# mprib/caliscope

Measured on AMD Instinct MI355X. Metric: observations/sec per LM iteration, higher is better.
Workload: dtype f64; 1 GPU; cfg4: 64 cams / 2000000 obs in total (200000 points / 2000000 obs on rank 0), extrinsics-only BA, linear loss; n_obs_total=2000000, params_per_camera=6, tolerances=ftol=xtol=gtol=1e-8 (reference defaults), sums=FP64 atomics (default)

## Files before the change

caliscope_amd/_lib.py:

```python

from __future__ import annotations

import ctypes as C
import os
from pathlib import Path

from caliscope_amd.exceptions import BackendError

LIB_NAME = "libcaliscope_ba.so"
LIB_PATH = Path(__file__).resolve().parent / LIB_NAME

c_double_p = C.POINTER(C.c_double)
c_int32_p = C.POINTER(C.c_int32)
c_int64_p = C.POINTER(C.c_int64)


class ProblemDesc(C.Structure):
    _fields_ = [
        ("n_cams", C.c_int32),
        ("n_points", C.c_int32),
        ("n_obs", C.c_int64),
        ("cam_n_params", c_int32_p),
        ("cam_model", c_int32_p),
        ("cam_const", c_double_p),
        ("obs_cam", c_int32_p),
        ("obs_pt", c_int32_p),
        ("obs_uv", c_double_p),
        ("loss", C.c_int32),
        ("f_scale", C.c_double),
    ]


class Options(C.Structure):
    _fields_ = [("device_id", C.c_int32), ("max_blocks", C.c_int32), ("deterministic", C.c_int32), ("evaluation_only", C.c_int32)]


class Linearization(C.Structure):
    _fields_ = [(n, C.c_double) for n in ("g_norm_inf", "gh_sq", "jg_sq", "x_scaled_norm", "x_norm", "cost")]


class NewtonInfo(C.Structure):
    _fields_ = [("ok", C.c_int32), ("reserved", C.c_int32), ("p_sq", C.c_double), ("gh_dot_p", C.c_double), ("w_sq", C.c_double)]


class TrialInfo(C.Structure):
    _fields_ = [("cost", C.c_double), ("step_norm", C.c_double), ("finite", C.c_int32), ("reserved", C.c_int32)]


class StepInfo(C.Structure):
    _fields_ = [
        ("lin", Linearization), ("newton", NewtonInfo), ("trial", TrialInfo), ("lam", C.c_double), ("radius", C.c_double),
        ("p_s", C.c_double * 2), ("predicted", C.c_double), ("alpha", C.c_double), ("beta", C.c_double),
        ("need_host", C.c_int32), ("reserved", C.c_int32),
    ]


class Info(C.Structure):
    _fields_ = [
        ("n_cams", C.c_int32), ("n_points", C.c_int32), ("n_cam_params", C.c_int32), ("n_params", C.c_int32),
        ("n_obs", C.c_int64), ("n_chunks", C.c_int32), ("grid_blocks", C.c_int32), ("plan_state", C.c_int32),
        ("max_obs_per_point", C.c_int32), ("device_bytes", C.c_int64),
        ("schur_groups", C.c_int32), ("schur_tiles", C.c_int32), ("schur_grid", C.c_int32), ("n_heavy_points", C.c_int32),
        ("schur_stream_len", C.c_int64), ("schur_pairs", C.c_int64), ("plan_error", C.c_int32), ("build_camg", C.c_int32),
    ]


class SolveOptions(C.Structure):
    _fields_ = [
        ("ftol", C.c_double), ("xtol", C.c_double), ("gtol", C.c_double), ("max_nfev", C.c_int64),
        ("lb", c_double_p), ("ub", c_double_p), ("verbose", C.c_int32), ("max_damping_retries", C.c_int32),
    ]


class Result(C.Structure):
    _fields_ = [
        ("status", C.c_int32), ("reserved", C.c_int32), ("nfev", C.c_int64), ("njev", C.c_int64), ("n_iterations", C.c_int64),
        ("cost", C.c_double), ("optimality", C.c_double), ("t_total_s", C.c_double),
        ("t_rejected_s", C.c_double), ("n_rejected_timed", C.c_int64),
    ]


class TriangulateDesc(C.Structure):
    _fields_ = [
        ("n_cams", C.c_int32),
        ("cam_model", c_int32_p),
        ("cam_intr", c_double_p),
        ("cam_P", c_double_p),
        ("n_points", C.c_int64),
        ("pt_start", c_int64_p),
        ("obs_cam", c_int32_p),
        ("obs_xy", c_double_p),
        ("float32_io", C.c_int32),
    ]


class ScaleDesc(C.Structure):
    _fields_ = [
        ("n_world", C.c_int64),
        ("world_xyz", c_double_p),
        ("n_groups", C.c_int64),
        ("group_start", c_int64_p),
        ("ent_world", c_int64_p),
        ("ent_obj", c_double_p),
    ]


SIGNATURES = {
    "cba_create": (C.c_int, [C.POINTER(ProblemDesc), C.POINTER(Options), C.POINTER(C.c_void_p)]),
    "cba_destroy": (None, [C.c_void_p]),
    "cba_comm_unique_id": (C.c_int, [C.c_char_p]),
    "cba_comm_init": (C.c_int, [C.c_void_p, C.c_char_p, C.c_int32, C.c_int32]),
    "cba_comm_abort": (C.c_int, [C.c_void_p]),
    "cba_group_create": (C.c_int, [C.c_int32, C.POINTER(C.c_void_p)]),
    "cba_group_join": (C.c_int, [C.c_void_p, C.c_void_p, C.c_int32]),
    "cba_group_abort": (None, [C.c_void_p]),
    "cba_group_destroy": (None, [C.c_void_p]),
    "cba_set_constraints": (C.c_int, [C.c_void_p, C.c_int32, c_int32_p, c_int32_p, c_double_p, c_double_p]),
    "cba_begin": (C.c_int, [C.c_void_p, c_double_p, c_double_p]),
    "cba_restart": (C.c_int, [C.c_void_p, c_double_p]),
    "cba_begin_deferred": (C.c_int, [C.c_void_p, c_double_p]),
    "cba_linearize": (C.c_int, [C.c_void_p, C.POINTER(Linearization)]),
    "cba_newton_step": (C.c_int, [C.c_void_p, C.c_double, C.POINTER(NewtonInfo)]),
    "cba_subspace_gram": (C.c_int, [C.c_void_p, C.c_double, C.c_double, C.c_double, C.c_double, c_double_p]),
    "cba_trial": (C.c_int, [C.c_void_p, C.c_double, C.c_double, C.POINTER(TrialInfo)]),
    "cba_accept": (C.c_int, [C.c_void_p]),
    "cba_linearize_build": (C.c_int, [C.c_void_p]),
    "cba_step": (C.c_int, [C.c_void_p, C.c_double, C.POINTER(StepInfo)]),
    "cba_refresh_step_scalars": (C.c_int, [C.c_void_p, C.POINTER(NewtonInfo)]),
    "cba_step_supported": (C.c_int, [C.c_void_p]),
    "cba_set_camera_scaling": (C.c_int, [C.c_void_p, c_double_p, c_double_p, C.POINTER(Linearization)]),
    "cba_set_bounds": (C.c_int, [C.c_void_p, c_double_p, c_double_p]),
    "cba_step_camera_state": (C.c_int, [C.c_void_p, c_double_p, c_double_p, c_double_p, c_double_p]),
    "cba_subspace_gram_ex": (C.c_int, [C.c_void_p, C.c_double, C.c_double, c_double_p, C.c_double, C.c_double, c_double_p, c_double_p]),
    "cba_trial_ex": (C.c_int, [C.c_void_p, C.c_double, C.c_double, c_double_p, C.POINTER(TrialInfo)]),
    "cba_solve": (C.c_int, [C.c_void_p, c_double_p, C.POINTER(SolveOptions), c_double_p, C.POINTER(Result)]),
    "cba_get_vector": (C.c_int, [C.c_void_p, C.c_int32, c_double_p]),
    "cba_get_camera_params": (C.c_int, [C.c_void_p, C.c_int32, c_double_p]),
    "cba_get_camera_state": (C.c_int, [C.c_void_p, c_double_p, c_double_p, c_double_p]),
    "cba_residuals": (C.c_int, [C.c_void_p, c_double_p, c_double_p, c_double_p]),
    "cba_normal_blocks": (C.c_int, [C.c_void_p, c_double_p, c_double_p, c_double_p, c_double_p, c_double_p]),
    "cba_reduced_system": (C.c_int, [C.c_void_p, c_double_p, c_double_p]),
    "cba_set_loss": (C.c_int, [C.c_void_p, C.c_int32, C.c_double]),
    "cba_plan_wait": (C.c_int, [C.c_void_p]),
    "cba_get_info": (C.c_int, [C.c_void_p, C.POINTER(Info)]),
    "cba_timer_count": (C.c_int, []),
    "cba_timer_name": (C.c_char_p, [C.c_int32]),
    "cba_get_timers": (C.c_int, [C.c_void_p, c_double_p, c_int64_p]),
    "cba_reset_timers": (C.c_int, [C.c_void_p]),
    "cba_enable_timers": (C.c_int, [C.c_void_p, C.c_int32]),
    "cba_host_plan": (C.c_int64, [C.c_int32, C.c_int64, c_int32_p, c_int32_p, C.c_int32, C.c_int32, c_int64_p, c_int64_p, c_int64_p]),
    "cba_triangulate": (C.c_int, [C.POINTER(TriangulateDesc), C.c_int32, c_double_p, c_double_p]),
    "cba_scale_errors": (C.c_int, [C.POINTER(ScaleDesc), C.c_int32, c_double_p]),
    "cba_trim": (C.c_int64, []),
    "cba_last_error": (C.c_char_p, []),
    "cba_set_error": (C.c_int, [C.c_int32, C.c_char_p]),
    "cba_version": (C.c_int, []),
    "cba_device_count": (C.c_int, []),
}

_lib = None


def load() -> C.CDLL:
    global _lib
    if _lib is not None:
        return _lib
    path = Path(os.environ.get("CALISCOPE_BA_LIB", LIB_PATH))
    if not path.exists():
        raise BackendError(
            f"{path} not found: build the MI355X engine first (python -c 'import __graft_entry__ as g; g.build()' "
            f"or python -m caliscope_amd.build).  There is no CPU fallback."
        )
    try:
        lib = C.CDLL(str(path))
    except OSError as exc:
        raise BackendError(f"could not load {path}: {exc}") from exc
    for name, (res, args) in SIGNATURES.items():
        try:
            fn = getattr(lib, name)
        except AttributeError as exc:
            raise BackendError(f"{path} does not export {name} (stale build?)") from exc
        fn.restype = res
        fn.argtypes = args
    _lib = lib
    return lib


def last_error(lib) -> str:
    msg = lib.cba_last_error()
    return msg.decode("utf-8", "replace") if msg else ""


def check(lib, rc: int, what: str) -> None:
    if rc != 0:
        raise BackendError(f"{what} failed (code {rc}): {last_error(lib)}")
```

caliscope_amd/csrc/cba_kernels.h:

```cpp
#pragma once
#include <hip/hip_runtime.h>

#include "ba_math.h"
#include "trf_math.h"
#include "wg_binding.h"

namespace cba {

constexpr int BLOCK = 256;
constexpr int CHUNK = 256;
constexpr int WAVE = 64;

struct VecLayout {
  int ncp;
  int ncp_pad;
  int P;
  int Ppad;
  __host__ __device__ long total() const { return (long)ncp_pad + 3L * Ppad; }
};

__device__ __forceinline__ double wave_sum(double v) {
#pragma unroll
  for (int o = WAVE / 2; o > 0; o >>= 1) v += __shfl_down(v, o, WAVE);
  return v;
// ... 51 lines not shown
  return r;
}

__device__ __forceinline__ void lds_add(double* addr, double v) { unsafeAtomicAdd(addr, v); }

constexpr int CAMTAB_LIVE = 36;
constexpr int CAMTAB_LDS = CAMTAB_LIVE + 1;
struct ObsRec { double u, v; int cam, pt; };
__device__ __forceinline__ ObsRec load_obs(const double* __restrict__ obs_u, const double* __restrict__ obs_v,
                                           const int* __restrict__ obs_cam, const int* __restrict__ obs_pt, int i) {
  ObsRec r;
  r.u = obs_u[i]; r.v = obs_v[i]; r.cam = obs_cam[i]; r.pt = obs_pt[i];
  return r;
}

__device__ __forceinline__ void stage_camtab(double* sh_tab, const double* tab, int n_cams) {
  for (int i = threadIdx.x; i < n_cams * CAMTAB_LIVE; i += BLOCK)
    sh_tab[(i / CAMTAB_LIVE) * CAMTAB_LDS + (i % CAMTAB_LIVE)] = tab[(i / CAMTAB_LIVE) * CAMTAB_DOUBLES + (i % CAMTAB_LIVE)];
}
__device__ __forceinline__ const CamTab& cam_at(const double* sh_tab, int cam) {
  return *reinterpret_cast<const CamTab*>(sh_tab + cam * CAMTAB_LDS);
}
template <bool CAMG>
__device__ __forceinline__ const CamTab& cam_of(const double* sh_tab, const double* __restrict__ tab, int cam) {
  if constexpr (CAMG) return *reinterpret_cast<const CamTab*>(tab + (long)cam * CAMTAB_DOUBLES);
  else return cam_at(sh_tab, cam);
}

__global__ void k_cam_prep(const double* __restrict__ xvec, const double* __restrict__ cam_const,
                           const int* __restrict__ cam_model, const int* __restrict__ cam_np,
                           const int* __restrict__ cam_off, int n_cams, double* __restrict__ tab) {
  const int c = blockIdx.x * blockDim.x + threadIdx.x;
  if (c >= n_cams) return;
  double xc[MAX_NC];
  const int np = cam_np[c];
  for (int i = 0; i < MAX_NC; ++i) xc[i] = (i < np) ? xvec[cam_off[c] + i] : 0.0;
  CamTab t;
  cam_prepare(xc, cam_const + c * CAM_CONST_STRIDE, cam_model[c], np, &t, cam_off[c]);
  const double* src = reinterpret_cast<const double*>(&t);
  for (int i = 0; i < CAMTAB_DOUBLES; ++i) tab[c * CAMTAB_DOUBLES + i] = src[i];
}

__global__ void __launch_bounds__(BLOCK)
k_begin(const double* __restrict__ x0, double* __restrict__ x, double* __restrict__ x_new, double* __restrict__ sinv, double* __restrict__ cam_diag,
        int* __restrict__ flags, long total, int ncp_pad, const double* __restrict__ cam_const, const int* __restrict__ cam_model,
        const int* __restrict__ cam_np, const int* __restrict__ cam_off, int n_cams, double* __restrict__ tab) {
  const long t0 = (long)blockIdx.x * blockDim.x + threadIdx.x;
  for (long i = t0; i < total; i += (long)gridDim.x * blockDim.x) {
    const double v = x0[i];
    x[i] = v;
    if (x_new) x_new[i] = v;
    sinv[i] = 1.0;
    if (i < ncp_pad) cam_diag[i] = 0.0;
    if (i < 4) flags[i] = 0;
  }
  if (t0 < n_cams) {
    const int c = (int)t0;
    double xc[MAX_NC];
    const int np = cam_np[c];
    for (int i = 0; i < MAX_NC; ++i) xc[i] = (i < np) ? x0[cam_off[c] + i] : 0.0;
    CamTab t;
    cam_prepare(xc, cam_const + c * CAM_CONST_STRIDE, cam_model[c], np, &t, cam_off[c]);
    const double* src = reinterpret_cast<const double*>(&t);
    for (int i = 0; i < CAMTAB_DOUBLES; ++i) tab[c * CAMTAB_DOUBLES + i] = src[i];
  }
}

template <bool WRITE_R, bool CAMG = false>
__global__ void __launch_bounds__(BLOCK)
k_cost(const double* __restrict__ obs_u, const double* __restrict__ obs_v, const int* __restrict__ obs_cam,
       const int* __restrict__ obs_pt, long n_obs, const double* __restrict__ xvec, VecLayout lay,
       const double* __restrict__ tab, int n_cams, int loss, double f_scale, double* __restrict__ partial,
       int* __restrict__ flags, double* __restrict__ r_out, const int* __restrict__ order) {
  extern __shared__ __attribute__((aligned(16))) double sh[];
  double* sh_tab = sh;
  double* sh_red = sh + (CAMG ? 0 : n_cams * CAMTAB_LDS);
  if (!CAMG) stage_camtab(sh_tab, tab, n_cams);
  __syncthreads();
  const double* px = xvec + lay.ncp_pad;
  double acc = 0.0;
  bool bad = false;
  struct Rec { int cam, pt; double u, v; long o; };
  const long stride = (long)gridDim.x * BLOCK, last = n_obs - 1;
  auto load_rec = [&](long i) {
    Rec r; const long k = min(i, last);
    r.cam = obs_cam[k]; r.pt = obs_pt[k]; r.u = obs_u[k]; r.v = obs_v[k]; r.o = WRITE_R ? (long)order[k] : 0;
    return r;
  };
  long i = (long)blockIdx.x * BLOCK + threadIdx.x;
  Rec rc = load_rec(i), rn = load_rec(i + stride);
  double X = px[rc.pt], Y = px[lay.Ppad + rc.pt], Z = px[2 * lay.Ppad + rc.pt];
  for (; i < n_obs; i += stride) {
    asm volatile("s_waitcnt vmcnt(0)" ::: "memory");
    asm volatile("" : "+v"(rc.cam), "+v"(rc.pt), "+v"(rc.u), "+v"(rc.v), "+v"(rc.o));
    asm volatile("" : "+v"(rn.cam), "+v"(rn.pt), "+v"(rn.u), "+v"(rn.v), "+v"(rn.o));
    asm volatile("" : "+v"(X), "+v"(Y), "+v"(Z));
    const double Xn = px[rn.pt], Yn = px[lay.Ppad + rn.pt], Zn = px[2 * lay.Ppad + rn.pt];
    const Rec rnn = load_rec(i + 2 * stride);
    __builtin_amdgcn_sched_barrier(0);
    double e[2];
    project_residual(cam_of<CAMG>(sh_tab, tab, rc.cam), X, Y, Z, rc.u, rc.v, e);
    if (!(isfinite(e[0]) && isfinite(e[1]))) bad = true;
    acc += robust_cost_one(loss, f_scale, e[0]) + robust_cost_one(loss, f_scale, e[1]);
    if (WRITE_R) {
      r_out[2 * rc.o] = e[0];
      r_out[2 * rc.o + 1] = e[1];
    }
    rc = rn; rn = rnn; X = Xn; Y = Yn; Z = Zn;
  }
  asm volatile("s_waitcnt vmcnt(0)" ::: "memory");
  if (bad) flags[0] = 1;
  const double tot = block_sum(acc, sh_red);
  if (threadIdx.x == 0) partial[blockIdx.x] = tot;
}

constexpr int REDUCE_RY = 16;
__device__ __forceinline__ void reduce_rows_block(const double* __restrict__ partial, int nrow, int width, double* __restrict__ out,
                                                  double* __restrict__ grad_out, const int* __restrict__ cam_off, const int* __restrict__ cam_np,
                                                  int stride, int tri) {
  __shared__ double sh[REDUCE_RY][64];
  const int j = blockIdx.x * 64 + threadIdx.x;
  double acc[8] = {0.0, 0.0, 0.0, 0.0, 0.0, 0.0, 0.0, 0.0};
  if (j < width) {
    int b = threadIdx.y;
    for (; b + 7 * REDUCE_RY < nrow; b += 8 * REDUCE_RY) {
#pragma unroll
      for (int q = 0; q < 8; ++q) acc[q] += partial[(long)(b + q * REDUCE_RY) * width + j];
    }
    for (; b < nrow; b += REDUCE_RY) acc[0] += partial[(long)b * width + j];
  }
  sh[threadIdx.y][threadIdx.x] = ((acc[0] + acc[1]) + (acc[2] + acc[3])) + ((acc[4] + acc[5]) + (acc[6] + acc[7]));
  __syncthreads();
  if (threadIdx.y == 0 && j < width) {
    double tot = 0.0;
#pragma unroll
    for (int y = 0; y < REDUCE_RY; ++y) tot += sh[y][threadIdx.x];
    out[j] = tot;
    if (grad_out) {
      const int c = j / stride, r = j % stride - tri;
      if (r >= 0 && r < cam_np[c]) grad_out[cam_off[c] + r] = tot;
    }
  }
}
__global__ void __launch_bounds__(64 * REDUCE_RY)
k_reduce_rows(const double* __restrict__ partial, int nrow, int width, double* __restrict__ out,
              double* __restrict__ grad_out = nullptr, const int* __restrict__ cam_off = nullptr, const int* __restrict__ cam_np = nullptr,
              int stride = 1, int tri = 0) {
  reduce_rows_block(partial, nrow, width, out, grad_out, cam_off, cam_np, stride, tri);
}
struct PubArgs {
  double* scal; int n_scal; int* flags; double* host_scal; int* host_flags; unsigned long long seq;
  const double* part_a; int rows_a, slot_a; const double* part_b; int rows_b, slot_b;
  const double* cam_src[4]; double* cam_dst; int ncp;
};
__global__ void __launch_bounds__(64 * REDUCE_RY)
k_reduce_rows_pub(const double* __restrict__ partial, int nrow, int width, double* __restrict__ out, double* __restrict__ grad_out,
                  const int* __restrict__ cam_off, const int* __restrict__ cam_np, int stride, int tri, PubArgs pub) {
  CBA_STAMP(ST_REDUCE_PUB);
  if (blockIdx.x + 1 < gridDim.x) { reduce_rows_block(partial, nrow, width, out, grad_out, cam_off, cam_np, stride, tri); return; }
  __shared__ double sh_w[2][REDUCE_RY];
  const int t = threadIdx.y * 64 + threadIdx.x;
  const double own = (t < pub.n_scal) ? pub.scal[t] : 0.0;
  double a = 0.0, b = 0.0;
  for (int r = t; r < pub.rows_a; r += 64 * REDUCE_RY) a += pub.part_a[r];
  for (int r = t; r < pub.rows_b; r += 64 * REDUCE_RY) b += pub.part_b[r];
  a = wave_sum(a); b = wave_sum(b);
  if (threadIdx.x == 0) { sh_w[0][threadIdx.y] = a; sh_w[1][threadIdx.y] = b; }
  __syncthreads();
  __shared__ double sh_tot[2];
  if (t == 0) {
    double ta = 0.0, tb = 0.0;
    for (int i = 0; i < REDUCE_RY; ++i) { ta += sh_w[0][i]; tb += sh_w[1][i]; }
    pub.scal[pub.slot_a] = ta; pub.scal[pub.slot_b] = tb;
    sh_tot[0] = ta; sh_tot[1] = tb;
  }
  __syncthreads();
  if (t < pub.n_scal) pub.host_scal[t] = (t == pub.slot_a) ? sh_tot[0] : (t == pub.slot_b) ? sh_tot[1] : own;
  if (t < 4) { pub.host_flags[t] = pub.flags[t]; pub.flags[t] = 0; }
  if (pub.cam_dst)
    for (int e = t; e < 4 * pub.ncp; e += 64 * REDUCE_RY) pub.cam_dst[e] = pub.cam_src[e / pub.ncp][e % pub.ncp];
  __threadfence_system();
  __syncthreads();
  if (t == 0) reinterpret_cast<volatile unsigned long long*>(pub.host_scal)[63] = pub.seq;
}
__global__ void k_xpack(const double* __restrict__ scal, const int* __restrict__ flags, unsigned long long mask, int with_max,
                        int rank, int world, double* __restrict__ xbuf) {
  if (threadIdx.x != 0 || blockIdx.x != 0) return;
  int n = 0;
  for (int s2 = 0; s2 < 32; ++s2)
    if ((mask >> s2) & 1ull) xbuf[n++] = scal[s2];
  for (int k = 0; k < 4; ++k) xbuf[n++] = flags[k] ? 1.0 : 0.0;
  if (with_max)
    for (int r = 0; r < world; ++r) xbuf[n++] = (r == rank) ? scal[4] : 0.0;
}
__global__ void k_xunpack(const double* __restrict__ xbuf, unsigned long long mask, int with_max, int world,
                          double* __restrict__ scal, int* __restrict__ flags) {
  if (threadIdx.x != 0 || blockIdx.x != 0) return;
  int n = 0;
  for (int s2 = 0; s2 < 32; ++s2)
    if ((mask >> s2) & 1ull) scal[s2] = xbuf[n++];
  for (int k = 0; k < 4; ++k) flags[k] = xbuf[n++] > 0.5 ? 1 : 0;
  if (with_max) {
    double m = 0.0;
    for (int r = 0; r < world; ++r) m = fmax(m, xbuf[n++]);
    scal[4] = m;
  }
}

template <bool MAX>
__global__ void __launch_bounds__(BLOCK)
k_reduce_narrow(const double* __restrict__ partial, int nrow, int width, double* __restrict__ out) {
  __shared__ double sh_red[BLOCK / WAVE];
  for (int j = 0; j < width; ++j) {
    double s = 0.0;
    for (int b = threadIdx.x; b < nrow; b += BLOCK) {
      const double v = partial[(long)b * width + j];
      s = MAX ? fmax(s, v) : s + v;
    }
    const double r = MAX ? block_max(s, sh_red) : block_sum(s, sh_red);
    if (threadIdx.x == 0) out[j] = r;
  }
}

template <int NC>
__device__ __forceinline__ double obs_linearize(const CamTab& c_lds, double X, double Y, double Z, double u, double v,
                                                int loss, double f_scale, double* e, double (*A)[MAX_NC],
                                                double (*B)[3]) {
  const CamTab c = c_lds;
  __builtin_amdgcn_sched_barrier(0);
  project_full(c, X, Y, Z, u, v, e, A, B);
  double rho = 0.0;
#pragma unroll
  for (int r = 0; r < 2; ++r) {
    double rs, er;
    rho += robust_one(loss, f_scale, e[r], &rs, &er);
    e[r] = er;
    if (loss != LOSS_LINEAR) {
#pragma unroll
      for (int k = 0; k < NC; ++k) A[r][k] *= rs;
      B[r][0] *= rs; B[r][1] *= rs; B[r][2] *= rs;
    }
  }
  return rho;
}

__device__ __forceinline__ double obs_factors(const CamTab& c_lds, double X, double Y, double Z, double u, double v, int loss, double f_scale, double* e,
                                              double (*G)[3], double* Yr, double (*Aint)[3], double (*B)[3]) {
  CamTab c;
  {
    const double* src = reinterpret_cast<const double*>(&c_lds);
    double* dst = reinterpret_cast<double*>(&c);
#pragma unroll
    for (int i = 0; i < 12; ++i) dst[i] = src[i];
#pragma unroll
    for (int i = 21; i < 35; ++i) dst[i] = src[i];
  }
  __builtin_amdgcn_sched_barrier(0);
  project_factors(c, X, Y, Z, u, v, e, G, Yr, Aint, B);
  double rho = 0.0;
#pragma unroll
  for (int r = 0; r < 2; ++r) {
    double rs, er;
    rho += robust_one(loss, f_scale, e[r], &rs, &er);
    e[r] = er;
    if (loss != LOSS_LINEAR) {
#pragma unroll
      for (int k = 0; k < 3; ++k) { G[r][k] *= rs; B[r][k] *= rs; Aint[r][k] *= rs; }
    }
  }
  return rho;
}

template <int NC> struct UPack {
  static constexpr int TRI = NC * (NC + 1) / 2;
  static constexpr int STRIDE = TRI + NC;
  __host__ __device__ static constexpr int idx(int r, int c) { return r * NC - r * (r - 1) / 2 + (c - r); }
};

constexpr int DET_ROUND = 9;
constexpr int DET_LD = CHUNK + 1;
struct DetPlan {
  const unsigned char* perm;
  const unsigned short* cstart;
};
template <int M>
__device__ __forceinline__ void det_round(const double* val, double* sh_cv, const int* sh_perm, const int* sh_cs, int n_cams, double* acc) {
#pragma unroll
  for (int q = 0; q < DET_ROUND; ++q) sh_cv[q * DET_LD + threadIdx.x] = val[q];
  __syncthreads();
#pragma unroll
  for (int m = 0; m < M; ++m) {
    const int task = (int)threadIdx.x + BLOCK * m;
    if (task < n_cams * DET_ROUND) {
      const int c = task / DET_ROUND, q = task % DET_ROUND;
      double s = 0.0;
      for (int j = sh_cs[c]; j < sh_cs[c + 1]; ++j) s += sh_cv[q * DET_LD + sh_perm[j]];
      acc[m] += s;
    }
  }
  __syncthreads();
}

template <int NC>
__device__ __forceinline__ double cam_block_value(int v, const double (*A)[MAX_NC], const double* e, int np) {
  using UP = UPack<NC>;
  int idx = 0;
#pragma unroll
  for (int r = 0; r < NC; ++r)
#pragma unroll
    for (int c = r; c < NC; ++c, ++idx)
      if (idx == v) return (r < np && c < np) ? A[0][r] * A[0][c] + A[1][r] * A[1][c] : 0.0;
#pragma unroll
  for (int r = 0; r < NC; ++r)
    if (UP::TRI + r == v) return (r < np) ? A[0][r] * e[0] + A[1][r] * e[1] : 0.0;
  return 0.0;
}

template <int NC, int DETM = 0, bool CAMG = false>
__global__ void __launch_bounds__(BLOCK)
k_build(const double* __restrict__ obs_u, const double* __restrict__ obs_v, const int* __restrict__ obs_cam,
        const int* __restrict__ obs_pt, const int* __restrict__ pt_start, const int* __restrict__ chunk_start,
        const int* __restrict__ chunk_pts, int n_chunks, const double* __restrict__ xvec, VecLayout lay, const double* __restrict__ tab, int n_cams,
        int loss, double f_scale, double* __restrict__ Vblk, double* __restrict__ gvec,
        double* __restrict__ partialU, double* __restrict__ partial_cost, int* __restrict__ flags, const double* __restrict__ skip,
        DetPlan det = DetPlan{nullptr, nullptr}) {
  using UP = UPack<NC>;
  constexpr bool DET = DETM > 0;
  if (skip && *skip != 0.0) return;
  extern __shared__ __attribute__((aligned(16))) double sh[];
  double* sh_tab = sh;
// ... 266 lines not shown
      lds_add(&sh_vg[4 * PM + pl], B[0][1] * B[0][2] + B[1][1] * B[1][2]);
      lds_add(&sh_vg[5 * PM + pl], B[0][2] * B[0][2] + B[1][2] * B[1][2]);
      lds_add(&sh_vg[6 * PM + pl], B[0][0] * e[0] + B[1][0] * e[1]);
      lds_add(&sh_vg[7 * PM + pl], B[0][1] * e[0] + B[1][1] * e[1]);
      lds_add(&sh_vg[8 * PM + pl], B[0][2] * e[0] + B[1][2] * e[1]);
    }
    flush();
    __syncthreads();
    for (int i = threadIdx.x; i < npts; i += BLOCK) {
#pragma unroll
      for (int q = 0; q < 6; ++q) Vblk[(long)q * lay.Ppad + p0 + i] = sh_vg[q * PM + i];
      gp[p0 + i] = sh_vg[6 * PM + i];
      gp[lay.Ppad + p0 + i] = sh_vg[7 * PM + i];
      gp[2 * lay.Ppad + p0 + i] = sh_vg[8 * PM + i];
    }
  }
  __syncthreads();
  if (!UGLOB) {
    for (int c = threadIdx.x; c < n_cams; c += BLOCK) {
      const double* Jl = tab + (long)c * CAMTAB_DOUBLES + 12;
      double* Uc = sh_U + (long)c * UP::STRIDE;
      double M[3][3], T[3][3];
#pragma unroll
      for (int r = 0; r < 3; ++r)
#pragma unroll
        for (int q = 0; q < 3; ++q) M[r][q] = Uc[UP::idx(min(r, q), max(r, q))];
#pragma unroll
      for (int r = 0; r < 3; ++r)
#pragma unroll
        for (int q = 0; q < 3; ++q) T[r][q] = Jl[r] * M[0][q] + Jl[3 + r] * M[1][q] + Jl[6 + r] * M[2][q];
#pragma unroll
      for (int r = 0; r < 3; ++r)
#pragma unroll
        for (int q = r; q < 3; ++q) Uc[UP::idx(r, q)] = T[r][0] * Jl[q] + T[r][1] * Jl[3 + q] + T[r][2] * Jl[6 + q];
#pragma unroll
      for (int q = 3; q <= NC; ++q) {
        double* v0 = (q < NC) ? &Uc[UP::idx(0, q)] : &Uc[UP::TRI + 0];
        double* v1 = (q < NC) ? &Uc[UP::idx(1, q)] : &Uc[UP::TRI + 1];
        double* v2 = (q < NC) ? &Uc[UP::idx(2, q)] : &Uc[UP::TRI + 2];
        const double a0 = *v0, a1 = *v1, a2 = *v2;
        *v0 = Jl[0] * a0 + Jl[3] * a1 + Jl[6] * a2;
        *v1 = Jl[1] * a0 + Jl[4] * a1 + Jl[7] * a2;
        *v2 = Jl[2] * a0 + Jl[5] * a1 + Jl[8] * a2;
      }
    }
    __syncthreads();
    double* dst = partialU + (long)blockIdx.x * n_cams * UP::STRIDE;
    for (int i = threadIdx.x; i < n_cams * UP::STRIDE; i += BLOCK) dst[i] = sh_U[i];
  }
  const double tot = block_sum(cost, sh_red);
  if (threadIdx.x == 0) partial_cost[blockIdx.x] = tot;
  if (TRIAL) {
    const double st = block_sum(step_sq, sh_red);
    if (threadIdx.x == 0) trial.step_partial[blockIdx.x] = st;
  }
  if (bad) flags[0] = 1;
}

__global__ void __launch_bounds__(256)
k_gather_uv(const double* __restrict__ uv_raw, const int* __restrict__ order, long n, double* __restrict__ u, double* __restrict__ v) {
  for (long i = (long)blockIdx.x * 256 + threadIdx.x; i < n; i += (long)gridDim.x * 256) {
    const double2 w = reinterpret_cast<const double2*>(uv_raw)[order[i]];
    u[i] = w.x; v[i] = w.y;
  }
}
__global__ void __launch_bounds__(256)
k_cs_fill(const int* __restrict__ perm, const int* __restrict__ sc_obs, const int* __restrict__ sc_p0, const double* __restrict__ u,
          const double* __restrict__ v, const int* __restrict__ cam, const int* __restrict__ pt, double* __restrict__ cu, double* __restrict__ cv,
          int* __restrict__ ccam, int* __restrict__ cptl) {
  const int s = blockIdx.x, o0 = sc_obs[s], o1 = sc_obs[s + 1], p0 = sc_p0[s];
  for (int j = o0 + threadIdx.x; j < o1; j += 256) {
    const int i = perm[j];
    cu[j] = u[i]; cv[j] = v[i]; ccam[j] = cam[i]; cptl[j] = pt[i] - p0;
  }
}

template <int NC>
__global__ void k_unpack_camera_grad(const double* __restrict__ Upacked, const int* __restrict__ cam_off,
                                     const int* __restrict__ cam_np, int n_cams, double* __restrict__ gvec) {
  using UP = UPack<NC>;
  const int t = blockIdx.x * blockDim.x + threadIdx.x;
  const int c = t / NC, r = t % NC;
  if (c >= n_cams || r >= cam_np[c]) return;
  gvec[cam_off[c] + r] = Upacked[c * UP::STRIDE + UP::TRI + r];
}

template <int NC>
__global__ void k_scale_update(const double* __restrict__ Upacked, const double* __restrict__ Vblk,
                               const int* __restrict__ param_cam, const int* __restrict__ param_loc, VecLayout lay,
                               int first, double* __restrict__ sinv, const double* __restrict__ cdiag) {
  using UP = UPack<NC>;
  const long total = lay.total();
  for (long i = (long)blockIdx.x * blockDim.x + threadIdx.x; i < total; i += (long)gridDim.x * blockDim.x) {
    double v;
    if (i < lay.ncp_pad) {
      if (i >= lay.ncp) continue;
      const int r = param_loc[i];
      v = Upacked[param_cam[i] * UP::STRIDE + UP::idx(r, r)];
    } else {
      const long k = (i - lay.ncp_pad) / lay.Ppad, p = (i - lay.ncp_pad) % lay.Ppad;
      if (p >= lay.P) continue;
      const int q = (k == 0) ? 0 : (k == 1 ? 3 : 5);
      v = Vblk[(long)q * lay.Ppad + p];
      if (cdiag) v += cdiag[k * lay.Ppad + p];
    }
    v = sqrt(v);
    if (first) { if (v == 0.0) v = 1.0; }
    else v = fmax(v, sinv[i]);
    sinv[i] = v;
  }
}

__global__ void k_cam_rescale(const double* __restrict__ state, const double* __restrict__ mult, const double* __restrict__ diag_h,
                              int ncp, double* __restrict__ sinv, double* __restrict__ cam_diag) {
  const int i = blockIdx.x * blockDim.x + threadIdx.x;
  if (i >= ncp) return;
  const double si = state[i] * mult[i];
  sinv[i] = si;
  cam_diag[i] = diag_h[i] * si * si;
}

__global__ void __launch_bounds__(BLOCK)
k_lin_scalars(const double* __restrict__ x, const double* __restrict__ g, const double* __restrict__ sinv,
              long total, int cam_end, int count_cams, int max_from, double* __restrict__ v1, double* __restrict__ partial,
              double* __restrict__ partial_max) {
  __shared__ double sh_red[BLOCK / WAVE];
  double s0 = 0, s1 = 0, s2 = 0, m = 0;
  for (long i = (long)blockIdx.x * BLOCK + threadIdx.x; i < total; i += (long)gridDim.x * BLOCK) {
    const double gi = g[i], si = sinv[i], xi = x[i];
    const double gh = gi / si;
    v1[i] = gh / si;
    if (i >= max_from) m = fmax(m, fabs(gi));
    if (i < cam_end && !count_cams) continue;
    s0 += gh * gh;
    s1 += (xi * si) * (xi * si);
    s2 += xi * xi;
  }
  double r;
  r = block_sum(s0, sh_red); if (threadIdx.x == 0) partial[blockIdx.x * 4 + 0] = r;
  r = block_sum(s1, sh_red); if (threadIdx.x == 0) partial[blockIdx.x * 4 + 1] = r;
  r = block_sum(s2, sh_red); if (threadIdx.x == 0) partial[blockIdx.x * 4 + 2] = r;
  if (threadIdx.x == 0) partial[blockIdx.x * 4 + 3] = 0.0;
  r = block_max(m, sh_red); if (threadIdx.x == 0) partial_max[blockIdx.x] = r;
}

__global__ void k_combine(const double* __restrict__ g, const double* __restrict__ sinv, const double* __restrict__ s,
                          double a, double b, long total, const double* __restrict__ over, int n_over, double* __restrict__ out) {
  for (long i = (long)blockIdx.x * blockDim.x + threadIdx.x; i < total; i += (long)gridDim.x * blockDim.x) {
    const double si = sinv[i];
    out[i] = (i < n_over) ? over[i] : a * g[i] / (si * si) + b * s[i];
  }
}

template <int NC, int NV, bool CAMG = false>
__global__ void __launch_bounds__(BLOCK)
k_jv(const double* __restrict__ obs_u, const double* __restrict__ obs_v, const int* __restrict__ obs_cam,
     const int* __restrict__ obs_pt, long n_obs, const double* __restrict__ xvec, VecLayout lay,
     const double* __restrict__ tab, const int* __restrict__ cam_off, int n_cams, int loss, double f_scale,
     const double* __restrict__ v1, const double* __restrict__ v2, double* __restrict__ partial) {
  CBA_STAMP(ST_JV);
  extern __shared__ __attribute__((aligned(16))) double sh[];
  double* sh_tab = sh;
  double* sh_v = sh_tab + (CAMG ? 0 : n_cams * CAMTAB_LDS);
  double* sh_red = sh_v + NV * lay.ncp_pad;
  if (!CAMG) stage_camtab(sh_tab, tab, n_cams);
  for (int i = threadIdx.x; i < lay.ncp_pad; i += BLOCK) {
    sh_v[i] = v1[i];
    if (NV == 2) sh_v[lay.ncp_pad + i] = v2[i];
  }
  __syncthreads();
  for (int c = threadIdx.x; c < n_cams; c += BLOCK) {
    const double* row = tab + (long)c * CAMTAB_DOUBLES;
    const int off = (int)row[35];
#pragma unroll
    for (int q = 0; q < NV; ++q) {
      double* vq = sh_v + q * lay.ncp_pad + off;
      const double r0 = vq[0], r1 = vq[1], r2 = vq[2];
      vq[0] = row[12] * r0 + row[13] * r1 + row[14] * r2;
      vq[1] = row[15] * r0 + row[16] * r1 + row[17] * r2;
      vq[2] = row[18] * r0 + row[19] * r1 + row[20] * r2;
    }
  }
  __syncthreads();
  const double* px = xvec + lay.ncp_pad;
  const double* p1 = v1 + lay.ncp_pad;
  const double* p2 = (NV == 2) ? v2 + lay.ncp_pad : nullptr;
  double s11 = 0, s12 = 0, s22 = 0;
  struct Rec { int cam, pt; double u, v; };
  struct Gat { double X, Y, Z, a, b, c, d, e, f; };
  constexpr int LOADS = 4 + (NV == 2 ? 9 : 6);
  const long stride = (long)gridDim.x * BLOCK, last = n_obs - 1;
  auto load_rec = [&](long i) { Rec r; const long k = min(i, last); r.cam = obs_cam[k]; r.pt = obs_pt[k]; r.u = obs_u[k]; r.v = obs_v[k]; return r; };
  auto load_gat = [&](int pt) {
    Gat g;
    g.X = px[pt]; g.Y = px[lay.Ppad + pt]; g.Z = px[2 * lay.Ppad + pt];
    g.a = p1[pt]; g.b = p1[lay.Ppad + pt]; g.c = p1[2 * lay.Ppad + pt];
    if (NV == 2) { g.d = p2[pt]; g.e = p2[lay.Ppad + pt]; g.f = p2[2 * lay.Ppad + pt]; } else { g.d = g.e = g.f = 0.0; }
    return g;
  };
  auto launder_rec = [](Rec& r) { asm volatile("" : "+v"(r.cam), "+v"(r.pt), "+v"(r.u), "+v"(r.v)); };
  auto launder_gat = [](Gat& g) {
    asm volatile("" : "+v"(g.X), "+v"(g.Y), "+v"(g.Z), "+v"(g.a), "+v"(g.b), "+v"(g.c));
    if (NV == 2) asm volatile("" : "+v"(g.d), "+v"(g.e), "+v"(g.f));
  };
  long i = (long)blockIdx.x * BLOCK + threadIdx.x;
  Rec rc = load_rec(i), r1 = load_rec(i + stride), r2 = load_rec(i + 2 * stride), r3 = load_rec(i + 3 * stride);
  Gat gc = load_gat(rc.pt), g1 = load_gat(r1.pt);
  asm volatile("s_waitcnt vmcnt(0)" ::: "memory");
  launder_rec(rc); launder_rec(r1); launder_rec(r2); launder_rec(r3); launder_gat(gc); launder_gat(g1);
  for (; i < n_obs; i += stride) {
    asm volatile("s_waitcnt vmcnt(%0)" ::"n"(LOADS) : "memory");
    launder_gat(gc); launder_rec(r2);
    const Gat g2 = load_gat(r2.pt);
    const Rec r4 = load_rec(i + 4 * stride);
    __builtin_amdgcn_sched_barrier(0);
    const int cam = rc.cam;
    double e[2], G[2][3], Yr[3], Aint[2][3], B[2][3];
    const CamTab& ctj = cam_of<CAMG>(sh_tab, tab, cam);
    obs_factors(ctj, gc.X, gc.Y, gc.Z, rc.u, rc.v, loss, f_scale, e, G, Yr, Aint, B);
    const double* vc = sh_v + (int)ctj.pad[0];
    auto jv = [&](const double* q, double px0, double px1, double px2, double* o0, double* o1) {
      const double m0 = fma(q[1], Yr[2], fma(-q[2], Yr[1], q[3]));
      const double m1 = fma(q[2], Yr[0], fma(-q[0], Yr[2], q[4]));
      const double m2 = fma(q[0], Yr[1], fma(-q[1], Yr[0], q[5]));
      double a0 = B[0][0] * px0 + B[0][1] * px1 + B[0][2] * px2, a1 = B[1][0] * px0 + B[1][1] * px1 + B[1][2] * px2;
      a0 = fma(G[0][2], m2, fma(G[0][1], m1, fma(G[0][0], m0, a0)));
      a1 = fma(G[1][2], m2, fma(G[1][1], m1, fma(G[1][0], m0, a1)));
      if (NC == 9 && ctj.nparams == 9.0) {
        a0 = fma(Aint[0][2], q[8], fma(Aint[0][1], q[7], fma(Aint[0][0], q[6], a0)));
        a1 = fma(Aint[1][2], q[8], fma(Aint[1][1], q[7], fma(Aint[1][0], q[6], a1)));
      }
      *o0 = a0; *o1 = a1;
    };
    double a0, a1;
    jv(vc, gc.a, gc.b, gc.c, &a0, &a1);
    s11 += a0 * a0 + a1 * a1;
    if (NV == 2) {
      double b0, b1;
      jv(vc + lay.ncp_pad, gc.d, gc.e, gc.f, &b0, &b1);
      s12 += a0 * b0 + a1 * b1;
      s22 += b0 * b0 + b1 * b1;
    }
    rc = r1; r1 = r2; r2 = r3; r3 = r4; gc = g1; g1 = g2;
  }
  asm volatile("s_waitcnt vmcnt(0)" ::: "memory");
  double r;
  r = block_sum(s11, sh_red); if (threadIdx.x == 0) partial[blockIdx.x * 4 + 0] = r;
  r = block_sum(s12, sh_red); if (threadIdx.x == 0) partial[blockIdx.x * 4 + 1] = r;
  r = block_sum(s22, sh_red); if (threadIdx.x == 0) partial[blockIdx.x * 4 + 2] = r;
  if (threadIdx.x == 0) partial[blockIdx.x * 4 + 3] = 0.0;
}

struct TilePlan {
  const int* chunk_start;
  const int* wg_first;
  const int* wg_end;
  const int* wg_tile;
  const int* wg_stride;
  const int* tile_a;
  const int* tile_b;
  const int* group_cam_begin;
  const int* group_par_begin;
  int g;
  int tile_elems;
  const int* obs;
  int rep;
  const unsigned* codes;
  const int* code_start;
  const unsigned* nit;
  int prio_shift;
};

template <int NC> struct SchurRec {
  static constexpr int NVAL = (NC == 9) ? 21 : 12;
  static constexpr int NPH = (NVAL + 1) / 2;
  static constexpr int LST = (NPH & 1) ? NPH : NPH + 1;
  static constexpr int REC = 2 * LST;
  static constexpr int HREC = 2 * NPH;
  static constexpr int STAGE = (HREC / 2) | 1;
  static constexpr int STAGE_WAVES = (NC == 9) ? 2 : 4;
};
static_assert(SchurRec<6>::REC == 14 && SchurRec<6>::LST == 7 && SchurRec<9>::REC == 22 && SchurRec<9>::LST == 11, "record sizes");

template <int NC>
__device__ __forceinline__ void expand_record(const double* __restrict__ rec, const double* __restrict__ Jl, double* __restrict__ T) {
  const double Y0 = rec[0], Y1 = rec[1], Y2 = rec[2];
  const double* Q = rec + 3;
#pragma unroll
  for (int m = 0; m < 3; ++m) {
    const double q0 = Q[m], q1 = Q[3 + m], q2 = Q[6 + m];
    const double c0 = Y1 * q2 - Y2 * q1, c1 = Y2 * q0 - Y0 * q2, c2 = Y0 * q1 - Y1 * q0;
#pragma unroll
    for (int r = 0; r < 3; ++r) T[3 * r + m] = Jl[r] * c0 + Jl[3 + r] * c1 + Jl[6 + r] * c2;
    T[9 + m] = q0; T[12 + m] = q1; T[15 + m] = q2;
  }
  if (NC == 9) {
#pragma unroll
    for (int k = 0; k < 9; ++k) T[18 + k] = rec[12 + k];
  }
}

struct LinFin {
  const double* partial_lin;
  const double* partial_max;
  const double* partial_jv;
  int rows_lin, rows_jv;
  double radius;
  double* scal;
  double* fz;
};
__device__ __forceinline__ double lin_finish_block(const LinFin& lf, double (*sh_red)[BLOCK / WAVE], double* sh_out) {
  double v[10];
#pragma unroll
// ... 2817 lines not shown
```

caliscope_amd/csrc/cba_lib.hip:

```cpp
#include <hip/hip_runtime.h>

#include <algorithm>
#include <atomic>
#include <chrono>
#include <cmath>
#include <condition_variable>
#include <cstdarg>
#include <cstdio>
#include <cstdlib>
#include <cstring>
#include <map>
#include <mutex>
#include <shared_mutex>
#include <memory>
#include <string>
#include <type_traits>
#include <thread>
#include <utility>
#include <vector>

#include <rccl/rccl.h>
#include <rocprofiler-sdk-roctx/roctx.h>

#include "../../include/caliscope_ba.h"
#include "cba_kernels.h"
#include "schur_plan.h"
#include "host_plan.h"
#include "wg_binding.h"

using namespace cba;

#ifndef CBA_SOURCE_DIGEST
#define CBA_SOURCE_DIGEST "unknown"
#endif
extern "C" __attribute__((used, visibility("hidden"))) const char cba_source_digest_marker[] = "CBA_SOURCE_DIGEST=" CBA_SOURCE_DIGEST;

static thread_local std::string g_last_error;

static int fail(int code, const char* fmt, ...) {
  char buf[1024];
  va_list ap;
  va_start(ap, fmt);
  vsnprintf(buf, sizeof(buf), fmt, ap);
  va_end(ap);
  g_last_error = buf;
  return code;
}

#define HIPCHK(expr)                                                                                   \
  do {                                                                                                 \
    hipError_t _e = (expr);                                                                            \
    if (_e != hipSuccess)                                                                              \
      return fail(CBA_ERR_HIP, "%s failed: %s (%s:%d)", #expr, hipGetErrorString(_e), __FILE__, __LINE__); \
  } while (0)

enum TimerId {
  T_CAM_PREP = 0, T_COST, T_BUILD, T_BUILD_REDUCE, T_SCALE_SCALARS, T_JV, T_SCHUR, T_SCHUR_REDUCE, T_CHOLESKY,
  T_BACKSUB, T_VECTOR, T_SCHUR_PAIRS, T_EXCHANGE, T_COUNT
};
static const char* kTimerNames[T_COUNT] = {
    "cam_prep", "cost", "build", "build_reduce", "scale_scalars", "jv", "schur", "schur_reduce_finalize",
    "cholesky_solve", "backsub", "vector_ops", "schur_pairs", "exchange"};

struct EventPair { hipEvent_t a, b; };
struct cba_group;

constexpr int JV_ROWS = 2048, CON_ROWS = 1024, PARTIAL4_ROWS = JV_ROWS + CON_ROWS;

struct cba_problem {
  int device = 0;
  hipStream_t stream = nullptr;
  int C = 0, P = 0, ncp = 0, nct = 6;
  long N = 0;
  VecLayout lay{};
  int n_chunks = 0, grid = 0, max_obs_per_point = 0;
  int G = 1, gsz = 1, n_tiles = 1, n_tile_chunks = 0, tile_grid = 0;
  int cus = 256;
  double plan_lane_util = 0.0;
  long tile_stream_len = 0, n_pairs = 0;
  TilePlan tp{};
  int* tile_wg_begin = nullptr;
  int loss = 0;
  double f_scale = 1.0;
  long device_bytes = 0;
  double *obs_u = nullptr, *obs_v = nullptr;
  int *obs_cam = nullptr, *obs_pt = nullptr, *pt_start = nullptr, *chunk_start = nullptr, *order = nullptr;
  int* chunk_pts = nullptr;
  double* cam_const = nullptr;
  int *cam_model = nullptr, *cam_np = nullptr, *cam_off = nullptr, *param_cam = nullptr, *param_loc = nullptr;
  double *tab = nullptr, *tab_new = nullptr;
  double *x0 = nullptr, *x = nullptr, *x_new = nullptr, *g = nullptr, *s = nullptr, *sinv = nullptr, *v1 = nullptr, *v2 = nullptr;
  double *V = nullptr, *Upacked = nullptr;
  double *partial = nullptr, *partial4 = nullptr, *partial1 = nullptr;
  long partial_width = 0;
  bool want_chol_trace = false;
  long long* chol_trace = nullptr;
  int ldw = 0;
  double *Sacc = nullptr, *S = nullptr, *Lbuf = nullptr, *rhs = nullptr, *red = nullptr, *Trec = nullptr, *partial_b = nullptr;
  CsPlan cs{};
  bool tab_global = false;
  int det_m = 0;
  DetPlan det{nullptr, nullptr};
  double* tri = nullptr;
  double* Xinv = nullptr;
  double* Tinv = nullptr;
  bool fuse_reg_finalize = true;
  double* scal = nullptr;
  double* xbuf = nullptr;
  double *sinv_state_c = nullptr, *cam_diag = nullptr, *cam_over1 = nullptr, *cam_over2 = nullptr;
  bool cam_scaled = false, cam_state_saved = false;
  double *fz = nullptr, *V2 = nullptr, *g2 = nullptr, *U2 = nullptr, *partial4b = nullptr;
  bool eval_only = false;
  bool peer_needs_primitives = false;
  bool have_build = false;
  bool trial_built = false;
  bool cost_pending = false;
  double cost_x = 0.0;
  double trial_cost = 0.0;
  int grid_backsub = 1;
  int jv_grid = 0;
  bool has_fragments = false;
  bool backsub_rec = false;
  int n_heavy = 0; int* heavy_pts = nullptr; int* heavy_frag = nullptr; double* heavy_W = nullptr;
  std::vector<int> h_heavy_pts;
  ConPlan con{};
  int con_grid = 0;
  int n_con_orphan = 0; int* con_orphan = nullptr;
  int* flags = nullptr;
  double* h_scal = nullptr;
  int* h_flags = nullptr;
  double* d_hscal = nullptr;
  double *h_cam = nullptr, *d_hcam = nullptr;
  double *h_bcam = nullptr, *d_hbcam = nullptr;
  double *lb_dev = nullptr, *ub_dev = nullptr, *sinv_state_c2 = nullptr, *cam_diag2 = nullptr;
  bool bounds_on = false;
  unsigned long long publish_seq = 0;
  bool spin_wait = true;
  int* d_hflags = nullptr;
  bool first_scale = true;
  double* sinv2 = nullptr;
  bool spec_enqueued = false, spec_valid = false;
  int spec_rows_jv = 0;
  bool lf_pending = false;
  LinFin lf{};
  bool have_x0 = false;
  std::vector<int> h_tile_wg_begin;
  struct PlanTask* plan_task = nullptr;
  int reg_reduce_y = 4;
  int plan_max_blocks = 0;
  size_t partial_capacity = 0;
  bool plan_is_cheap = false;
  int plan_error = 0;
  bool schur_clock = false;
  long long* stamps = nullptr;
  bool begun = false, linearized = false, stepped = false, have_trial = false;
  double gh_sq = 0.0;
  std::vector<int> h_cam_off, h_cam_np;
  double* h_vec = nullptr;
  size_t h_vec_doubles = 0;
  hipEvent_t h_vec_sent = nullptr;
  bool h_vec_in_flight = false;
  bool timers_on = false;
  std::vector<EventPair> pending[T_COUNT];
  std::vector<EventPair> free_events;
  double t_ms[T_COUNT] = {0};
  long t_calls[T_COUNT] = {0};
  std::vector<void*> allocs;
  std::vector<size_t> alloc_bytes;
  size_t mail_doubles = 0;
  char* arena_cur = nullptr; size_t arena_left = 0, arena_next = (size_t)4 << 20;
  char* up_stage = nullptr; size_t up_cap = 0, up_used = 0;
  std::atomic<ncclComm_t> comm{nullptr};
  std::atomic<bool> comm_aborted{false};
  cba_group* group = nullptr;
  int rank = 0, world = 1;
  unsigned long long group_generation = 0;
  bool sharded() const { return comm.load() != nullptr || group != nullptr || comm_aborted.load(); }
};

constexpr size_t kPoolChunk = (size_t)4 << 20;
constexpr size_t kPoolKeep = 4;
constexpr size_t kPoolStagingMax = (size_t)8 << 20;
struct DevicePool {
  std::vector<void*> chunks;
  std::vector<hipStream_t> streams;
  std::vector<std::pair<double*, size_t>> mail;
  std::vector<std::pair<double*, size_t>> staging;
  std::vector<char*> upstage;
};
constexpr size_t kUpStage = (size_t)256 << 10, kUpStageMax = (size_t)64 << 10;
static std::mutex g_pool_mu;
static std::map<int, DevicePool> g_pool;

template <typename T>
static int dev_alloc(cba_problem* p, T** out, size_t count) {
  const size_t bytes = (std::max<size_t>(count, 1) * sizeof(T) + 255) & ~(size_t)255;
  if (bytes > p->arena_left) {
    const size_t chunk = std::max(bytes, p->arena_next);
    void* ptr = nullptr;
    if (chunk == kPoolChunk) {
      std::lock_guard<std::mutex> lock(g_pool_mu);
      DevicePool& pool = g_pool[p->device];
      if (!pool.chunks.empty()) { ptr = pool.chunks.back(); pool.chunks.pop_back(); }
    }
    if (!ptr) HIPCHK(hipMalloc(&ptr, chunk));
    p->allocs.push_back(ptr);
    p->alloc_bytes.push_back(chunk);
    if (bytes >= p->arena_next) {
      p->device_bytes += (long)bytes;
      *out = static_cast<T*>(ptr);
      return CBA_OK;
    }
    p->arena_cur = static_cast<char*>(ptr);
    p->arena_left = chunk;
    p->arena_next = std::min<size_t>(p->arena_next * 2, (size_t)256 << 20);
  }
  *out = reinterpret_cast<T*>(p->arena_cur);
  p->arena_cur += bytes;
  p->arena_left -= bytes;
  p->device_bytes += (long)bytes;
  return CBA_OK;
}
template <typename T>
static int dev_upload(cba_problem* p, T** out, const T* h, size_t count) {
  int rc = dev_alloc(p, out, count);
  if (rc) return rc;
  const size_t bytes = count * sizeof(T);
  if (bytes && p->up_stage && p->stream && bytes <= kUpStageMax && p->up_used + bytes <= p->up_cap) {
    std::memcpy(p->up_stage + p->up_used, h, bytes);
    HIPCHK(hipMemcpyAsync(*out, p->up_stage + p->up_used, bytes, hipMemcpyHostToDevice, p->stream));
    p->up_used += (bytes + 63) & ~(size_t)63;
  } else if (bytes) {
    HIPCHK(hipMemcpy(*out, h, bytes, hipMemcpyHostToDevice));
  }
  return CBA_OK;
}
template <typename T, typename V>
static int dev_upload(cba_problem* p, T** out, const V& h) {
  static_assert(std::is_same<typename std::remove_cv<typename std::remove_pointer<decltype(h.data())>::type>::type, T>::value, "element type");
  return dev_upload(p, out, h.data(), h.size());
}
template <typename T>
static int dev_zeros(cba_problem* p, T** out, size_t count) {
  int rc = dev_alloc(p, out, count);
  if (rc) return rc;
  HIPCHK(hipMemsetAsync(*out, 0, count * sizeof(T), p->stream));
  return CBA_OK;
}
static void upload_stage_acquire(cba_problem* p) {
  if (p->up_stage) return;
  {
    std::lock_guard<std::mutex> lock(g_pool_mu);
    DevicePool& pool = g_pool[p->device];
    if (!pool.upstage.empty()) { p->up_stage = pool.upstage.back(); pool.upstage.pop_back(); }
  }
  if (!p->up_stage && hipHostMalloc((void**)&p->up_stage, kUpStage, hipHostMallocDefault) != hipSuccess) { (void)hipGetLastError(); p->up_stage = nullptr; }
  p->up_cap = p->up_stage ? kUpStage : 0;
  p->up_used = 0;
}
static void upload_stage_release(cba_problem* p) {
  if (!p->up_stage) return;
  std::lock_guard<std::mutex> lock(g_pool_mu);
  DevicePool& pool = g_pool[p->device];
  if (pool.upstage.size() < kPoolKeep) pool.upstage.push_back(p->up_stage); else (void)hipHostFree(p->up_stage);
  p->up_stage = nullptr; p->up_cap = p->up_used = 0;
}

static int stage_wait(cba_problem* p) {
  if (p->h_vec_in_flight) { HIPCHK(hipEventSynchronize(p->h_vec_sent)); p->h_vec_in_flight = false; }
  return CBA_OK;
}
static int stage_sent(cba_problem* p) {
  HIPCHK(hipEventRecord(p->h_vec_sent, p->stream));
  p->h_vec_in_flight = true;
  return CBA_OK;
}

struct RoctxRange {
  explicit RoctxRange(const char* name) { roctxRangePushA(name); }
  ~RoctxRange() { roctxRangePop(); }
};

struct ScopedTimer {
  cba_problem* p;
  int id;
  EventPair ev{};
  bool on;
  ScopedTimer(cba_problem* p_, int id_) : p(p_), id(id_), on(p_->timers_on) {
    if (!on) return;
    if (!p->free_events.empty()) { ev = p->free_events.back(); p->free_events.pop_back(); }
    else { (void)hipEventCreate(&ev.a); (void)hipEventCreate(&ev.b); }
    (void)hipEventRecord(ev.a, p->stream);
  }
  ~ScopedTimer() {
    if (!on) return;
// ... 670 lines not shown
  {
    int per_cu = p->tab_global ? resident_per_cu(k_jv<NC, 1, true>, lds_jv(p, 1), 2) : resident_per_cu(k_jv<NC, 1>, lds_jv(p, 1), 2);
    if (const char* e = std::getenv("CBA_JV_WGS")) per_cu = std::max(1, std::min(std::atoi(e), 8));
    p->jv_grid = (int)std::max<long>(1, std::min<long>((p->N + BLOCK - 1) / BLOCK, (long)p->cus * per_cu));
    p->jv_grid = std::min(p->jv_grid, JV_ROWS);
  }
  if (p->n_heavy && (rc = allow_lds(k_heavy_schur<NC>, (size_t)p->ncp * 3 * sizeof(double) + (size_t)p->ncp * sizeof(int)))) return rc;
  if ((rc = allow_lds(k_chol_apply, (size_t)p->ncp * 8))) return rc;
  if ((rc = allow_lds(k_step_cam, (size_t)p->lay.ncp_pad * 8))) return rc;
  if (p->ncp <= SMALL_N && (rc = allow_lds(k_small_solve<NC>, kSmallSolveLds))) return rc;
  return CBA_OK;
}


static void start_plan_task(cba_problem* p, const cba_options* opt, int n_cus, const int* hcam, const int* hps) {
  constexpr long kTwoStageObs = 500000;
  const char* plan_env = std::getenv("CBA_PLAN");
  bool plan_two_stage = p->N >= kTwoStageObs;
  if (plan_env && std::strcmp(plan_env, "swap") == 0) plan_two_stage = true;
  if (plan_env && (std::strcmp(plan_env, "full") == 0 || std::strcmp(plan_env, "cheap") == 0)) plan_two_stage = false;
  if ((opt && opt->deterministic) || p->schur_clock) plan_two_stage = false;
  Reg2Params prm = (p->nct == 9) ? reg2_params<9, Reg3Cfg<9>>(p) : reg2_params<6, Reg3Cfg<6>>(p);
  if (plan_env) prm.cheap = std::strcmp(plan_env, "cheap") == 0;
  p->plan_task = new PlanTask();
  {
    const int cus0 = n_cus > 0 ? n_cus : 256;
    const size_t tile_lds = (p->nct == 9) ? Reg3Cfg<9>::LDS_BYTES : Reg3Cfg<6>::LDS_BYTES;
    const int per_cu = std::min(std::max<int>(1, (int)((160 * 1024) / tile_lds)), (p->nct == 9) ? RegCfg<9>::PER_CU : RegCfg<6>::PER_CU);
    const int mb0 = (opt && opt->max_blocks > 0) ? opt->max_blocks : 2 * cus0;
    p->plan_max_blocks = std::min(cus0 * per_cu, std::max(mb0, cus0));
  }
  p->plan_task->start(prm, hcam, hps, plan_two_stage, p);
}

static int open_stream_and_mailbox(cba_problem* p, const MailLayout& mail) {
  {
    std::lock_guard<std::mutex> lock(g_pool_mu);
    DevicePool& pool = g_pool[p->device];
    if (!pool.streams.empty()) { p->stream = pool.streams.back(); pool.streams.pop_back(); }
    for (size_t i = 0; i < pool.mail.size(); ++i)
      if (pool.mail[i].second >= mail.total) {
        p->h_scal = pool.mail[i].first; p->mail_doubles = pool.mail[i].second;
        pool.mail.erase(pool.mail.begin() + (long)i);
        break;
      }
  }
  if (!p->stream) HIPCHK(hipStreamCreateWithFlags(&p->stream, hipStreamNonBlocking));
  if (!p->h_scal) {
    p->mail_doubles = std::max<size_t>(mail.total, MailLayout(96).total);
    HIPCHK(hipHostMalloc((void**)&p->h_scal, p->mail_doubles * sizeof(double), hipHostMallocMapped));
  }
  HIPCHK(hipHostGetDevicePointer((void**)&p->d_hscal, p->h_scal, 0));
  p->h_cam = p->h_scal + mail.cam; p->d_hcam = p->d_hscal + mail.cam;
  p->h_flags = reinterpret_cast<int*>(p->h_scal + mail.flags); p->d_hflags = reinterpret_cast<int*>(p->d_hscal + mail.flags);
  p->h_bcam = p->h_scal + mail.bcam; p->d_hbcam = p->d_hscal + mail.bcam;
  std::memset(p->h_scal, 0, mail.total * sizeof(double));
  return CBA_OK;
}

#define TRYS(e) do { const int rc_ = (e); if (rc_) return rc_; } while (0)

static int upload_observations(cba_problem* p, const double* obs_uv, const SortedObs& obs, const PointTables& tabs) {
  TRYS(dev_upload(p, &p->obs_cam, obs.cam)); TRYS(dev_upload(p, &p->obs_pt, obs.pt));
  TRYS(dev_upload(p, &p->order, obs.order)); TRYS(dev_upload(p, &p->pt_start, tabs.pt_start)); TRYS(dev_upload(p, &p->chunk_start, tabs.chunk_start));
  double* uv_raw = nullptr;
  TRYS(dev_upload(p, &uv_raw, obs_uv, (size_t)2 * p->N)); TRYS(dev_alloc(p, &p->obs_u, (size_t)p->N)); TRYS(dev_alloc(p, &p->obs_v, (size_t)p->N));
  hipLaunchKernelGGL(k_gather_uv, dim3((int)std::min<long>((p->N + 255) / 256, 2048)), dim3(256), 0, p->stream, (const double*)uv_raw, (const int*)p->order, p->N, p->obs_u, p->obs_v);
  return CBA_OK;
}

static int upload_det_plan(cba_problem* p, const HostDetPlan& plan) {
  unsigned char* dperm = nullptr; unsigned short* dcst = nullptr;
  TRYS(dev_upload(p, &dperm, plan.perm)); TRYS(dev_upload(p, &dcst, plan.cst));
  p->det_m = plan.det_m;
  p->det = DetPlan{dperm, dcst};
  return CBA_OK;
}

static int upload_cs_plan(cba_problem* p, const HostCsPlan& plan) {
  double *dcu = nullptr, *dcv = nullptr;
  int *dcc = nullptr, *dcp = nullptr, *dso = nullptr, *dp0 = nullptr, *dnp = nullptr, *dperm = nullptr;
  TRYS(dev_upload(p, &dperm, plan.cperm));
  TRYS(dev_alloc(p, &dcu, (size_t)p->N)); TRYS(dev_alloc(p, &dcv, (size_t)p->N)); TRYS(dev_alloc(p, &dcc, (size_t)p->N)); TRYS(dev_alloc(p, &dcp, (size_t)p->N));
  TRYS(dev_upload(p, &dso, plan.sc_obs)); TRYS(dev_upload(p, &dp0, plan.sc_p0)); TRYS(dev_upload(p, &dnp, plan.sc_np));
  hipLaunchKernelGGL(k_cs_fill, dim3(plan.n_sc), dim3(256), 0, p->stream, (const int*)dperm, (const int*)dso, (const int*)dp0, (const double*)p->obs_u, (const double*)p->obs_v,
                     (const int*)p->obs_cam, (const int*)p->obs_pt, dcu, dcv, dcc, dcp);
  p->cs = CsPlan{dcu, dcv, dcc, dcp, dso, dp0, dnp, plan.n_sc, plan.pmax};
  return CBA_OK;
}

static int upload_cameras(cba_problem* p, const double* cam_const, const CameraLayout& cams, const PointTables& tabs) {
  if (p->n_heavy) {
    TRYS(dev_upload(p, &p->heavy_pts, tabs.heavy)); TRYS(dev_upload(p, &p->heavy_frag, tabs.heavy_frag));
    TRYS(dev_alloc(p, &p->heavy_W, (size_t)p->n_heavy * p->ncp * 3));
  }
  TRYS(dev_upload(p, &p->cam_const, cam_const, (size_t)p->C * 12));
  TRYS(dev_upload(p, &p->cam_model, cams.model)); TRYS(dev_upload(p, &p->cam_np, cams.np)); TRYS(dev_upload(p, &p->cam_off, cams.off));
  TRYS(dev_upload(p, &p->param_cam, cams.param_cam)); TRYS(dev_upload(p, &p->param_loc, cams.param_loc));
  return CBA_OK;
}

static int alloc_vectors(cba_problem* p) {
  TRYS(dev_alloc(p, &p->tab, (size_t)p->C * CAMTAB_DOUBLES)); TRYS(dev_alloc(p, &p->tab_new, (size_t)p->C * CAMTAB_DOUBLES));
  for (double** v : {&p->x0, &p->x, &p->x_new, &p->g, &p->s, &p->sinv, &p->v1, &p->v2, &p->sinv2}) TRYS(dev_zeros(p, v, (size_t)p->lay.total()));
  for (double** v : {&p->sinv_state_c, &p->cam_diag, &p->cam_over1, &p->cam_over2, &p->lb_dev, &p->ub_dev, &p->sinv_state_c2, &p->cam_diag2})
    TRYS(dev_zeros(p, v, (size_t)p->lay.ncp_pad));
  TRYS(dev_zeros(p, &p->V, (size_t)6 * p->lay.Ppad));
  const int ustride = (p->nct == 9) ? UPack<9>::STRIDE : UPack<6>::STRIDE;
  TRYS(dev_alloc(p, &p->Upacked, (size_t)p->C * ustride + 128));
  return CBA_OK;
}

static int install_first_plan(cba_problem* p, bool plan_timing) {
  PlanTask& task = *p->plan_task;
  const auto t_wait = std::chrono::steady_clock::now();
  task.wait_stage(task.two_stage ? 1 : 2);
  if (plan_timing) {
    fprintf(stderr, "  plan: %s took %.3f s on its own threads, started before the uploads; waited %.3f s for it\n", task.two_stage ? "the cheap plan" : "dealt streams and codes",
            task.two_stage ? task.seconds_cheap : task.seconds, std::chrono::duration<double>(std::chrono::steady_clock::now() - t_wait).count());
    const Reg2Plan& made = task.two_stage ? task.cheap : task.plan;
    fprintf(stderr, "  plan: its phases: point runs %.4f s, jobs %.4f s, concatenation %.4f s (%.0f MB)\n", made.seconds_runs, made.seconds_jobs, made.seconds_concat,
            (made.obs.size() + made.codes.size()) * 4e-6);
  }
  if (task.two_stage ? task.rc_cheap : task.rc)
    return fail(CBA_ERR_UNSUPPORTED, "a world point has more observations inside one camera-group tile than a chunk of the pair plan holds (%d records)",
                (p->nct == 9) ? Reg3Cfg<9>::SCHUNK : Reg3Cfg<6>::SCHUNK);
  const int rc = install_reg2_plan(p, task.two_stage ? task.cheap : task.plan, task.prm);
  p->plan_is_cheap = task.two_stage || task.prm.cheap;
  return rc;
}

static int alloc_solver_buffers(cba_problem* p) {
  const int ncp = p->ncp, nct = p->nct;
  const long tot = p->lay.total();
  const int ustride = (nct == 9) ? UPack<9>::STRIDE : UPack<6>::STRIDE;
  const long w_build = (long)p->C * ustride;
  p->partial_width = w_build;
  p->partial_capacity = (size_t)std::max<long>((long)p->grid * w_build, (long)(p->tile_grid + p->tile_grid / 8 + 1) * std::max(p->tp.rep, 1) * p->tp.tile_elems);
  TRYS(dev_alloc(p, &p->partial, p->partial_capacity));
  TRYS(dev_alloc(p, &p->partial4, (size_t)PARTIAL4_ROWS * 4)); TRYS(dev_alloc(p, &p->partial1, (size_t)2048)); TRYS(dev_alloc(p, &p->partial4b, (size_t)2048 * 4));
  TRYS(dev_zeros(p, &p->Sacc, (size_t)ncp * ncp + (size_t)B_SLICES * p->lay.ncp_pad));
  TRYS(dev_alloc(p, &p->tri, (size_t)ncp * (ncp + 1) / 2 + p->lay.ncp_pad));
  if (!p->eval_only) {
    TRYS(dev_alloc(p, &p->red, (size_t)p->G * p->tp.tile_elems));
    TRYS(dev_alloc(p, &p->Trec, (size_t)std::max<long>(p->N, 1) * ((nct == 9) ? SchurRec<9>::HREC : SchurRec<6>::HREC)));
    TRYS(dev_alloc(p, &p->partial_b, (size_t)p->grid * p->lay.ncp_pad));
  }
  TRYS(dev_alloc(p, &p->S, (size_t)ncp * ncp)); p->ldw = (ncp + 3) & ~3;
  if (p->want_chol_trace) TRYS(dev_alloc(p, &p->chol_trace, (size_t)((ncp + NB - 1) / NB + 2) * 8));
  TRYS(dev_alloc(p, &p->Lbuf, (size_t)(ncp + 1) * p->ldw));
  TRYS(dev_alloc(p, &p->Xinv, (size_t)((ncp + NB - 1) / NB + 1) * NB * NB));
  TRYS(dev_zeros(p, &p->Tinv, (size_t)ncp * p->ldw));
  TRYS(dev_alloc(p, &p->rhs, (size_t)p->lay.ncp_pad));
  TRYS(dev_zeros(p, &p->scal, 64)); TRYS(dev_zeros(p, &p->flags, 4)); TRYS(dev_alloc(p, &p->xbuf, 128));
  TRYS(dev_alloc(p, &p->fz, 8)); TRYS(dev_zeros(p, &p->V2, (size_t)6 * p->lay.Ppad)); TRYS(dev_zeros(p, &p->g2, (size_t)tot));
  TRYS(dev_alloc(p, &p->U2, (size_t)p->C * ustride + 128));
  return CBA_OK;
}

static int open_staging(cba_problem* p) {
  const size_t tot = (size_t)p->lay.total();
  {
    std::lock_guard<std::mutex> lock(g_pool_mu);
    DevicePool& pool = g_pool[p->device];
    for (size_t i = 0; i < pool.staging.size(); ++i)
      if (pool.staging[i].second >= tot && pool.staging[i].second <= 4 * tot + 4096) {
        p->h_vec = pool.staging[i].first; p->h_vec_doubles = pool.staging[i].second;
        pool.staging.erase(pool.staging.begin() + (long)i);
        break;
      }
  }
  HIPCHK(hipEventCreateWithFlags(&p->h_vec_sent, hipEventDisableTiming));
  if (!p->h_vec) {
    p->h_vec_doubles = tot;
    HIPCHK(hipHostMalloc((void**)&p->h_vec, p->h_vec_doubles * sizeof(double), hipHostMallocDefault));
  }
  return CBA_OK;
}
static int device_synchronize() { HIPCHK(hipDeviceSynchronize()); return CBA_OK; }
#undef TRYS

extern "C" {

int cba_create(const cba_problem_desc* d, const cba_options* opt, cba_problem** out) {
  if (!d || !out) return fail(CBA_ERR_INVALID, "cba_create: null argument");
  *out = nullptr;
  if (const int rc = validate_problem_desc(fail, d)) return rc;
  const double t_enter = std::chrono::duration<double>(std::chrono::steady_clock::now().time_since_epoch()).count();
  int ndev = 0;
  if (hipGetDeviceCount(&ndev) != hipSuccess || ndev <= 0)
    return fail(CBA_ERR_NO_DEVICE, "no HIP device available: the MI355X engine has no CPU fallback");
  int dev = (opt && opt->device_id >= 0) ? opt->device_id : 0;
  if (!(opt && opt->device_id >= 0)) (void)hipGetDevice(&dev);
  if (dev >= ndev) return fail(CBA_ERR_INVALID, "device %d requested, %d available", dev, ndev);
  HIPCHK(hipSetDevice(dev));
  int n_cus = 0;
  if (hipDeviceGetAttribute(&n_cus, hipDeviceAttributeMultiprocessorCount, dev) != hipSuccess) n_cus = 0;

  cba_problem* p = new cba_problem();
  p->device = dev;
  p->C = d->n_cams; p->P = d->n_points; p->N = d->n_obs;
  p->loss = d->loss; p->f_scale = d->f_scale;
  if (const char* e = std::getenv("CBA_REG_FINALIZE")) p->fuse_reg_finalize = e[0] != '0';
#ifdef CBA_PROFILING
  p->schur_clock = std::getenv("CBA_SCHUR_CLOCK") != nullptr;
  p->want_chol_trace = std::getenv("CBA_CHOL_TRACE") != nullptr;
  if (std::getenv("CBA_STAMPS")) {
    const size_t n = (size_t)STAMP_SLOTS * STAMP_BLOCKS * STAMP_ROW;
    if (hipMalloc((void**)&p->stamps, n * sizeof(long long)) == hipSuccess) {
      (void)hipMemset(p->stamps, 0, n * sizeof(long long));
      (void)hipMemcpyToSymbol(HIP_SYMBOL(g_cba_stamps), &p->stamps, sizeof(p->stamps));
    }
  }
#endif
  int rc = CBA_OK;
#define TRY(e) do { rc = (e); if (rc) { cba_destroy(p); return rc; } } while (0)
  const bool deterministic = opt && opt->deterministic;

  CameraLayout cams;
  TRY(camera_layout(fail, d, cams));
  const int ncp = cams.ncp, nct = cams.nct;
  p->ncp = ncp; p->nct = nct;
  p->h_cam_off = cams.off; p->h_cam_np = cams.np;
  p->lay.ncp = ncp; p->lay.ncp_pad = cams.ncp_pad;
  p->lay.P = p->P; p->lay.Ppad = (p->P + 31) / 32 * 32;

  const bool plan_timing = plan_timing_on();
  auto t_now = []() { return std::chrono::duration<double>(std::chrono::steady_clock::now().time_since_epoch()).count(); };
  double t_mark = t_now();
  auto lap = [&](const char* what) { if (plan_timing) { const double t = t_now(); fprintf(stderr, "cba_create: %-28s %.6f s\n", what, t - t_mark); t_mark = t; } };
  SortedObs obs;
  PointTables tabs;
  {
    HostVec<int64_t> order(p->N), pstart((size_t)p->P + 1), cstart((size_t)p->N + 2);
    const int64_t nch = cba_host_plan(p->P, p->N, d->obs_pt, d->obs_cam, p->C, CHUNK, order.data(), pstart.data(), cstart.data());
    if (nch < 0) TRY((int)nch);
    p->n_chunks = (int)nch;
    lap("sort by point, chunk table");
    gather_sorted(p->N, d->obs_cam, d->obs_pt, order.data(), obs);
    TRY(point_tables(fail, p->P, pstart.data(), nch, cstart.data(), obs.pt.data(), CHUNK, HEAVY_OBS, tabs));
  }
  p->max_obs_per_point = tabs.max_obs_per_point;
  p->n_heavy = (int)tabs.heavy.size();
  p->h_heavy_pts = tabs.heavy;
  p->has_fragments = tabs.has_fragments;
  p->eval_only = opt && opt->evaluation_only != 0;
  choose_schur_groups(p);
  if (!p->eval_only) start_plan_task(p, opt, n_cus, obs.cam.data(), tabs.pt_start.data());

  TRY(open_stream_and_mailbox(p, MailLayout(ncp)));
  const int cus = n_cus > 0 ? n_cus : 256;
  p->cus = cus;
  const int max_blocks = (opt && opt->max_blocks > 0) ? opt->max_blocks : 2 * cus;
  p->grid = std::max(1, std::min(p->n_chunks, max_blocks));
  p->grid_backsub = std::max(1, std::min(p->n_chunks, 2 * cus));
  if (const char* e = std::getenv("CBA_BACKSUB_WGS")) p->grid_backsub = std::max(1, std::min(p->n_chunks, std::min(std::max(std::atoi(e), 1), 8) * cus));

  lap("reorder on host");
  upload_stage_acquire(p);
  TRY(upload_observations(p, d->obs_uv, obs, tabs));
  if (deterministic) {
    HostDetPlan det;
    TRY(det_plan(fail, p->C, nct, p->n_chunks, tabs.chunk_start.data(), obs.cam.data(), CHUNK, DET_ROUND, BLOCK, det));
    TRY(upload_det_plan(p, det));
  }
  TRY(dev_upload(p, &p->chunk_pts, tabs.chunk_pts));
  {
    const char* cs_env = std::getenv("CBA_BUILD_CS");
    HostCsPlan cs;
    cs_plan(!(cs_env && cs_env[0] == '0'), deterministic, p->C, p->N, p->n_chunks, tabs.chunk_start.data(), tabs.chunk_pts.data(), obs.cam.data(), p->grid,
            (nct == 9) ? 4096 : 2048, CHUNK, CS_MAX_PTS, cs);
    if (cs.n_sc) TRY(upload_cs_plan(p, cs));
  }
  TRY(upload_cameras(p, d->cam_const, cams, tabs));
  lap("upload observations");
  TRY(alloc_vectors(p));
  lap("allocate vectors");
  if (nct == 9) TRY(configure_kernels<9>(p)); else TRY(configure_kernels<6>(p));
  lap("reorder, upload, allocate");
  if (!p->eval_only) TRY(install_first_plan(p, plan_timing));
  lap("Schur plan (streams, pairs, upload)");
  TRY(alloc_solver_buffers(p));
  TRY(open_staging(p));
  lap("solver buffers");
  TRY(device_synchronize());
#undef TRY
  upload_stage_release(p);
  lap("device synchronize");
  if (p->plan_task) {
    if (p->plan_task->two_stage) {
      p->plan_task->hcam_keep = std::move(obs.cam);
      p->plan_task->hps_keep = std::move(tabs.pt_start);
    } else {
      drop_plan_task(p);
    }
  }
  if (plan_timing) fprintf(stderr, "cba_create: %.3f s in total\n", t_now() - t_enter);
  *out = p;
  return CBA_OK;
}

static int maybe_swap_plan(cba_problem* p, bool wait);

int cba_plan_wait(cba_problem* p) {
  if (!p) return fail(CBA_ERR_INVALID, "cba_plan_wait: null problem");
  HIPCHK(hipSetDevice(p->device));
  return maybe_swap_plan(p, true);
}

int cba_set_loss(cba_problem* p, int32_t loss, double f_scale) {
  if (!p) return fail(CBA_ERR_INVALID, "cba_set_loss: null problem");
  if (loss < CBA_LOSS_LINEAR || loss > CBA_LOSS_ARCTAN) return fail(CBA_ERR_INVALID, "cba_set_loss: unknown loss %d", loss);
  if (loss != CBA_LOSS_LINEAR && !(f_scale > 0.0)) return fail(CBA_ERR_INVALID, "cba_set_loss: f_scale must be positive");
  p->loss = loss; p->f_scale = f_scale;
  p->have_build = false;
  p->spec_valid = false; p->spec_enqueued = false;
  return CBA_OK;
}

int cba_get_info(cba_problem* p, cba_info* o) {
  if (!p || !o) return fail(CBA_ERR_INVALID, "null argument");
  o->n_cams = p->C; o->n_points = p->P; o->n_cam_params = p->ncp; o->n_params = p->ncp + 3 * p->P; o->n_obs = p->N;
  o->n_chunks = p->n_chunks; o->grid_blocks = p->grid;
  o->plan_state = !p->plan_is_cheap ? 0 : (p->plan_task ? 1 : 2); o->plan_error = p->plan_error;
  o->schur_groups = p->G; o->schur_tiles = p->n_tiles; o->schur_grid = p->tile_grid; o->schur_stream_len = p->tile_stream_len; o->schur_pairs = p->n_pairs;
  o->max_obs_per_point = p->max_obs_per_point; o->device_bytes = p->device_bytes; o->n_heavy_points = p->n_heavy;
  {
    const bool cs = p->cs.n_sc && !p->det_m && !p->n_heavy;
    const bool camg = cs ? (p->nct == 6 ? build_cs_camg<6>(p) : build_cs_camg<9>(p)) : (p->nct == 6 ? build_camg<6>(p) : build_camg<9>(p));
    const bool uglob = cs && (p->nct == 6 ? build_cs_uglob<6>(p) : build_cs_uglob<9>(p));
    o->build_camg = (camg ? 1 : 0) | (p->tab_global ? 2 : 0) | (cs ? 4 : 0) | (uglob ? 8 : 0) | (p->backsub_rec ? 16 : 0) |
                    (p->con.n_con && p->con.small ? 32 : 0);
  }
  return CBA_OK;
}

int cba_enable_timers(cba_problem* p, int32_t on) { if (!p) return fail(CBA_ERR_INVALID, "null"); p->timers_on = on != 0; return CBA_OK; }
int cba_reset_timers(cba_problem* p) {
  if (!p) return fail(CBA_ERR_INVALID, "null");
  (void)hipSetDevice(p->device);
  drain_timers(p);
  for (int t = 0; t < T_COUNT; ++t) { p->t_ms[t] = 0; p->t_calls[t] = 0; }
  return CBA_OK;
}
int cba_get_timers(cba_problem* p, double* ms, int64_t* calls) {
  if (!p) return fail(CBA_ERR_INVALID, "null");
  (void)hipSetDevice(p->device);
  drain_timers(p);
  for (int t = 0; t < T_COUNT; ++t) { if (ms) ms[t] = p->t_ms[t]; if (calls) calls[t] = p->t_calls[t]; }
  return CBA_OK;
}

}

static void pack_host(const cba_problem* p, const double* x_ref, double* v, double pad_value) {
  const VecLayout& L = p->lay;
  std::fill(v, v + L.total(), pad_value);
  for (int i = 0; i < L.ncp; ++i) v[i] = x_ref[i];
  const double* pts = x_ref + L.ncp;
  double* vx = v + L.ncp_pad;
  for (int q = 0; q < L.P; ++q) {
    vx[q] = pts[3 * q]; vx[L.Ppad + q] = pts[3 * q + 1]; vx[2 * L.Ppad + q] = pts[3 * q + 2];
  }
}
static void unpack_host(const cba_problem* p, const double* v, double* x_ref) {
  const VecLayout& L = p->lay;
  for (int i = 0; i < L.ncp; ++i) x_ref[i] = v[i];
  double* pts = x_ref + L.ncp;
  const double* vx = v + L.ncp_pad;
  for (int q = 0; q < L.P; ++q) {
    pts[3 * q] = vx[q]; pts[3 * q + 1] = vx[L.Ppad + q]; pts[3 * q + 2] = vx[2 * L.Ppad + q];
  }
}

static int launch_cam_prep(cba_problem* p, const double* xvec, double* tab) {
  ScopedTimer t(p, T_CAM_PREP);
  hipLaunchKernelGGL(k_cam_prep, dim3((p->C + 63) / 64), dim3(64), 0, p->stream, xvec, p->cam_const, p->cam_model,
                     p->cam_np, p->cam_off, p->C, tab);
  return CBA_OK;
}

static int launch_cost(cba_problem* p, const double* xvec, const double* tab, int slot, double* r_out, int* rows_out = nullptr) {
  const int grid = (int)std::min<long>((p->N + BLOCK - 1) / BLOCK, 1024);
  {
    ScopedTimer t(p, T_COST);
    auto launch = [&](auto kernel, double* r, const int* ord) {
      hipLaunchKernelGGL(kernel, dim3(grid), dim3(BLOCK), lds_cost(p), p->stream, p->obs_u, p->obs_v, p->obs_cam,
                         p->obs_pt, p->N, xvec, p->lay, tab, p->C, p->loss, p->f_scale, p->partial1, p->flags, r, ord);
    };
    if (r_out) { if (p->tab_global) launch(k_cost<true, true>, r_out, (const int*)p->order); else launch(k_cost<true>, r_out, (const int*)p->order); }
    else { if (p->tab_global) launch(k_cost<false, true>, (double*)nullptr, (const int*)nullptr); else launch(k_cost<false>, (double*)nullptr, (const int*)nullptr); }
  }
  ScopedTimer t(p, T_VECTOR);
  int rows = grid;
  if (p->con.n_con) {
    hipLaunchKernelGGL(k_con_eval<false>, dim3(p->con_grid), dim3(BLOCK), 0, p->stream, p->con, xvec, p->lay, p->loss, p->f_scale,
                       (double*)nullptr, p->partial1 + grid, p->flags, r_out ? r_out + 2 * p->N : (double*)nullptr);
    rows += p->con_grid;
  }
  if (rows_out) { *rows_out = rows; return CBA_OK; }
  hipLaunchKernelGGL(k_reduce_narrow<false>, dim3(1), dim3(BLOCK), 0, p->stream, p->partial1, rows, 1, p->scal + slot);
  return CBA_OK;
}

static bool fused_trial(const cba_problem* p, bool compact) { return compact && p->cs.n_sc && !p->det_m && !p->n_heavy && !p->con.n_con; }

template <int NC>
static int run_build_into(cba_problem* p, const double* xvec, const double* tab, double* V, double* g, double* Upacked, int cost_slot,
                          const double* skip = nullptr, bool defer_exchange = false, bool compact = false, int flag_slot = 0,
                          const TrialSrc* trial = nullptr, const PubArgs* pub = nullptr) {
  RoctxRange range("cba:build");
  {
    ScopedTimer t(p, T_BUILD);
    if (p->n_heavy)
      hipLaunchKernelGGL(k_zero_heavy, dim3((p->n_heavy + 63) / 64), dim3(64), 0, p->stream, p->heavy_pts, p->n_heavy, p->lay, V, 6,
                         g + p->lay.ncp_pad, 3);
    auto launch_build = [&](auto kernel) {
      hipLaunchKernelGGL(kernel, dim3(p->grid), dim3(BLOCK), lds_build<NC>(p), p->stream, p->obs_u, p->obs_v, p->obs_cam,
                         p->obs_pt, p->pt_start, p->chunk_start, p->chunk_pts, p->n_chunks, xvec, p->lay, tab, p->C, p->loss, p->f_scale,
                         V, g, p->partial, p->partial1, p->flags + flag_slot, skip, p->det);
    };
    if (p->cs.n_sc && !p->det_m && !p->n_heavy) {
      const TrialSrc tsrc = trial ? *trial : TrialSrc{};
      auto launch_cs = [&](auto kernel, size_t lds) {
        hipLaunchKernelGGL(kernel, dim3(p->grid), dim3(BLOCK), lds, p->stream, p->cs, xvec, p->lay, tab, p->C, p->loss, p->f_scale,
                           V, g, p->partial, p->partial1, p->flags + flag_slot, skip, tsrc);
      };
      if (build_cs_uglob<NC>(p)) {
        (void)hipMemsetAsync(p->partial, 0, (size_t)p->C * UPack<NC>::STRIDE * sizeof(double), p->stream);
        if (trial) launch_cs(k_build_cs<NC, true, true, true>, lds_build_cs<NC>(p, true, true));
        else launch_cs(k_build_cs<NC, true, true>, lds_build_cs<NC>(p, true, true));
      } else if (build_cs_camg<NC>(p)) {
        if (trial) launch_cs(k_build_cs<NC, true, false, true>, lds_build_cs<NC>(p, true));
        else launch_cs(k_build_cs<NC, true>, lds_build_cs<NC>(p, true));
      } else {
        if (trial) launch_cs(k_build_cs<NC, false, false, true>, lds_build_cs<NC>(p, false));
        else launch_cs(k_build_cs<NC, false>, lds_build_cs<NC>(p, false));
      }
    } else
    switch (p->det_m) {
      case 3: launch_build(k_build<NC, 3>); break;
      case 5: launch_build(k_build<NC, 5>); break;
      case 8: launch_build(k_build<NC, 8>); break;
      case 16: { if constexpr (NC == 6) launch_build(k_build<NC, 16>); } break;
      default:
        if (build_camg<NC>(p)) launch_build(k_build<NC, 0, true>); else launch_build(k_build<NC, 0>);
        break;
    }
  }
  {
    ScopedTimer t(p, T_BUILD_REDUCE);
    const int w = p->C * UPack<NC>::STRIDE;
    const int u_rows = (p->cs.n_sc && !p->det_m && !p->n_heavy && build_cs_uglob<NC>(p)) ? 1 : p->grid;
    if (compact) {
      if (pub)
        hipLaunchKernelGGL(k_reduce_rows_pub, dim3((w + 63) / 64 + 1), dim3(64, REDUCE_RY), 0, p->stream, (const double*)p->partial, u_rows, w, Upacked, g,
                           (const int*)p->cam_off, (const int*)p->cam_np, (int)UPack<NC>::STRIDE, (int)UPack<NC>::TRI, *pub);
      else
        hipLaunchKernelGGL(k_reduce_rows, dim3((w + 63) / 64), dim3(64, REDUCE_RY), 0, p->stream, p->partial, u_rows, w, Upacked, g,
                           (const int*)p->cam_off, (const int*)p->cam_np, (int)UPack<NC>::STRIDE, (int)UPack<NC>::TRI);
      return CBA_OK;
    }
    hipLaunchKernelGGL(k_reduce_rows, dim3((w + 63) / 64), dim3(64, REDUCE_RY), 0, p->stream, p->partial, u_rows, w, Upacked,
                       (double*)nullptr, (const int*)nullptr, (const int*)nullptr, 1, 0);
    int rho_rows = p->grid;
    if (p->con.n_con) {
      HIPCHK(hipMemsetAsync(p->con.cdiag, 0, (size_t)3 * p->lay.Ppad * sizeof(double), p->stream));
      if (p->n_con_orphan)
        hipLaunchKernelGGL(k_zero_heavy, dim3((p->n_con_orphan + 63) / 64), dim3(64), 0, p->stream, (const int*)p->con_orphan, p->n_con_orphan, p->lay,
                           g + p->lay.ncp_pad, 3, (double*)nullptr, 0);
      hipLaunchKernelGGL(k_con_eval<true>, dim3(p->con_grid), dim3(BLOCK), 0, p->stream, p->con, xvec, p->lay, p->loss, p->f_scale, g,
                         p->partial1 + p->grid, p->flags, (double*)nullptr);
      rho_rows += p->con_grid;
    }
    hipLaunchKernelGGL(k_reduce_narrow<false>, dim3(1), dim3(BLOCK), 0, p->stream, p->partial1, rho_rows, 1, p->scal + cost_slot);
    if (defer_exchange) return CBA_OK;
    int rc = allreduce_sum(p, Upacked, (size_t)w);
    if (rc) return rc;
    hipLaunchKernelGGL((k_unpack_camera_grad<NC>), dim3((p->C * NC + 255) / 256), dim3(256), 0, p->stream, Upacked,
                       p->cam_off, p->cam_np, p->C, g);
  }
  return CBA_OK;
}

template <int NC>
static int run_build(cba_problem* p) { return run_build_into<NC>(p, p->x, p->tab, p->V, p->g, p->Upacked, 8, nullptr, false, false, 3); }

template <int NC>
static int run_jv(cba_problem* p, int nv, int* rows_out = nullptr, const double* xvec = nullptr, const double* tab = nullptr) {
  ScopedTimer t(p, T_JV);
  if (!xvec) { xvec = p->x; tab = p->tab; }
  const int grid = nv == 1 ? p->jv_grid : (int)std::min<long>((p->N + BLOCK - 1) / BLOCK, 1024);
  const int con_rows = p->con.n_con ? p->con_grid : 0;
  if (grid + con_rows > PARTIAL4_ROWS)
    return fail(CBA_ERR_UNSUPPORTED, "run_jv: %d rows of k_jv and %d of k_con_jv exceed the %d rows of partial4", grid, con_rows, PARTIAL4_ROWS);
  auto launch_jv = [&](auto kernel) {
    hipLaunchKernelGGL(kernel, dim3(grid), dim3(BLOCK), lds_jv(p, nv), p->stream, p->obs_u, p->obs_v, p->obs_cam, p->obs_pt,
                       p->N, xvec, p->lay, tab, p->cam_off, p->C, p->loss, p->f_scale, p->v1, p->v2, p->partial4);
  };
  if (nv == 1) { if (p->tab_global) launch_jv(k_jv<NC, 1, true>); else launch_jv(k_jv<NC, 1>); }
  else { if (p->tab_global) launch_jv(k_jv<NC, 2, true>); else launch_jv(k_jv<NC, 2>); }
  int rows = grid;
  if (con_rows) {
    if (nv == 1) hipLaunchKernelGGL(k_con_jv<1>, dim3(p->con_grid), dim3(BLOCK), 0, p->stream, p->con, p->lay, p->v1, p->v2, p->partial4 + 4 * grid);
    else hipLaunchKernelGGL(k_con_jv<2>, dim3(p->con_grid), dim3(BLOCK), 0, p->stream, p->con, p->lay, p->v1, p->v2, p->partial4 + 4 * grid);
    rows += con_rows;
  }
  if (rows_out) { *rows_out = rows; return CBA_OK; }
  hipLaunchKernelGGL(k_reduce_narrow<false>, dim3(1), dim3(BLOCK), 0, p->stream, p->partial4, rows, 4, p->scal + 12);
  return CBA_OK;
}

template <int NC>
static int run_lin_chain(cba_problem* p, bool scalars = true, bool compact = false, double radius = 0.0, bool defer_finish = false) {
  RoctxRange range("cba:linearize");
  if (!p->have_build) {
    int rcb = run_build<NC>(p);
    if (rcb) return rcb;
    p->cost_pending = true;
    p->have_build = true;
    p->spec_valid = false;
  }
  if (compact && p->spec_valid) {
    p->spec_valid = false;
    if (defer_finish) {
      p->lf = LinFin{p->partial4b, p->partial1, p->partial4, vec_grid(p->lay.total()), p->spec_rows_jv, radius, p->scal, p->fz};
      p->lf_pending = true;
      return CBA_OK;
    }
    ScopedTimer t(p, T_SCALE_SCALARS);
    hipLaunchKernelGGL(k_lin_finish, dim3(1), dim3(BLOCK), 0, p->stream, p->partial4b, p->partial1, vec_grid(p->lay.total()), p->partial4, p->spec_rows_jv, radius,
                       p->scal, p->fz);
    return CBA_OK;
  }
  p->spec_valid = false;
  const long tot = p->lay.total();
  const int vg = vec_grid(tot);
  const bool bnd = defer_finish && p->bounds_on;
  if (bnd && !p->first_scale && !p->cam_scaled)
    HIPCHK(hipMemcpyAsync(p->sinv_state_c, p->sinv, (size_t)p->lay.ncp_pad * sizeof(double), hipMemcpyDeviceToDevice, p->stream));
  if (p->cam_scaled && !bnd)
    HIPCHK(hipMemcpyAsync(p->sinv, p->sinv_state_c, (size_t)p->lay.ncp_pad * sizeof(double), hipMemcpyDeviceToDevice, p->stream));
  p->cam_state_saved = false;
  {
    ScopedTimer t(p, T_SCALE_SCALARS);
    if (compact) {
      const BoundArgs ba = bnd ? BoundArgs{p->lb_dev, p->ub_dev, p->sinv_state_c, p->sinv_state_c, p->cam_diag} : BoundArgs{};
      if (bnd) p->cam_scaled = true;
      auto launch_sl = [&](auto kernel) {
        hipLaunchKernelGGL(kernel, dim3(vg), dim3(BLOCK), 0, p->stream, p->Upacked, p->V, p->param_cam, p->param_loc, p->lay,
                           p->first_scale ? 1 : 0, p->sinv, p->con.n_con ? (const double*)p->con.cdiag : (const double*)nullptr, p->x, p->g, p->v1,
                           p->partial4b, p->partial1, (const double*)nullptr, ba);
      };
      if (bnd) launch_sl(k_scale_lin<NC, true>); else launch_sl(k_scale_lin<NC, false>);
      p->first_scale = false;
      int rows_jv = 0;
      int rcj = run_jv<NC>(p, 1, &rows_jv);
      if (rcj) return rcj;
      if (defer_finish) {
        p->lf = LinFin{p->partial4b, p->partial1, p->partial4, vg, rows_jv, radius, p->scal, p->fz};
        p->lf_pending = true;
        return CBA_OK;
      }
      hipLaunchKernelGGL(k_lin_finish, dim3(1), dim3(BLOCK), 0, p->stream, p->partial4b, p->partial1, vg, p->partial4, rows_jv, radius,
                         p->scal, p->fz);
      return CBA_OK;
    }
    hipLaunchKernelGGL((k_scale_update<NC>), dim3(vg), dim3(BLOCK), 0, p->stream, p->Upacked, p->V, p->param_cam, p->param_loc,
                       p->lay, p->first_scale ? 1 : 0, p->sinv, p->con.n_con ? (const double*)p->con.cdiag : (const double*)nullptr);
    p->first_scale = false;
    if (!scalars) return exchange(p, SLOT(8), false);
    hipLaunchKernelGGL(k_lin_scalars, dim3(vg), dim3(BLOCK), 0, p->stream, p->x, p->g, p->sinv, tot, p->lay.ncp_pad,
                       p->rank == 0 ? 1 : 0, 0, p->v1, p->partial4, p->partial1);
    hipLaunchKernelGGL(k_reduce_narrow<false>, dim3(1), dim3(BLOCK), 0, p->stream, p->partial4, vg, 4, p->scal + 0);
    hipLaunchKernelGGL(k_reduce_narrow<true>, dim3(1), dim3(BLOCK), 0, p->stream, p->partial1, vg, 1, p->scal + 4);
  }
  {
    int rcj = run_jv<NC>(p, 1);
    if (rcj) return rcj;
  }
  return exchange(p, SLOT(0) | SLOT(1) | SLOT(2) | SLOT(3) | SLOT(8) | SLOT(12) | SLOT(13) | SLOT(14) | SLOT(15), true);
}

static void read_linearization(cba_problem* p, cba_linearization* out) {
  if (p->cost_pending) { p->cost_x = p->h_flags[3] ? NAN : 0.5 * p->h_scal[8]; p->cost_pending = false; }
  p->gh_sq = p->h_scal[0];
  out->gh_sq = p->h_scal[0];
  out->x_scaled_norm = std::sqrt(p->h_scal[1]);
  out->x_norm = std::sqrt(p->h_scal[2]);
  out->g_norm_inf = p->h_scal[4];
  out->cost = p->cost_x;
  out->jg_sq = p->h_scal[12];
}

template <int NC>
static int run_linearize(cba_problem* p, cba_linearization* out) {
  int rc = run_lin_chain<NC>(p, true, !p->sharded(), 1.0);
  if (rc) return rc;
  rc = sync_scalars(p, 16);
  if (rc) return rc;
  read_linearization(p, out);
  return CBA_OK;
}

static int enqueue_cholesky(cba_problem* p) {
  const int n = p->ncp, nbk = (n + NB - 1) / NB;
  for (int k = -1; k < nbk; ++k) {
    const int n_panel = k < 0 ? 1 : nbk - k;
    const int x = nbk - k - 1, n_trailing = k < 1 ? 0 : x * (x + 1) / 2;
    const int n_inverse = (k >= 1) ? (nbk - k) * k : 0;
    hipLaunchKernelGGL(k_chol_step, dim3(n_panel + n_trailing + n_inverse), dim3(CHOL_THREADS), 0, p->stream, p->Lbuf, n, p->ldw, k, p->flags, p->chol_trace, p->Xinv, p->Tinv);
  }
  hipLaunchKernelGGL(k_chol_apply, dim3(nbk), dim3(APPLY_THREADS), (size_t)n * 8, p->stream, (const double*)p->Tinv, (const double*)p->Lbuf, n, p->ldw, p->s);
  return CBA_OK;
}

static int run_cholesky(cba_problem* p) {
#ifdef CBA_PROFILING
  if (p->chol_trace) {
    const int nbk = (p->ncp + NB - 1) / NB;
    HIPCHK(hipMemsetAsync(p->chol_trace, 0, (size_t)(nbk + 2) * 8 * sizeof(long long), p->stream));
    int rc = enqueue_cholesky(p);
    if (rc) return rc;
    std::vector<long long> h((size_t)(nbk + 2) * 8);
    HIPCHK(hipMemcpyAsync(h.data(), p->chol_trace, h.size() * sizeof(long long), hipMemcpyDeviceToHost, p->stream));
    HIPCHK(hipStreamSynchronize(p->stream));
    for (int s = 0; s <= nbk; ++s) {
      fprintf(stderr, "chol step %2d:", s - 1);
      for (int ph = 1; ph < 7; ++ph)
        if (h[s * 8 + ph] && h[s * 8 + ph - 1]) fprintf(stderr, " ph%d %6.2f us", ph, (h[s * 8 + ph] - h[s * 8 + ph - 1]) * 0.01); else if (h[s * 8 + ph]) fprintf(stderr, " ph%d (%6.2f)", ph, (h[s * 8 + ph] - h[s * 8]) * 0.01);
      if (s < nbk && h[(s + 1) * 8] && h[s * 8]) fprintf(stderr, "  | to next step start %6.2f us", (h[(s + 1) * 8] - h[s * 8]) * 0.01);
      fprintf(stderr, "\n");
    }
    return CBA_OK;
  }
#endif
  ScopedTimer t(p, T_CHOLESKY);
  return enqueue_cholesky(p);
}

static int run_step_scalars(cba_problem* p, bool formula_w, bool compact = false) {
  ScopedTimer t(p, T_VECTOR);
  const long tot = p->lay.total();
  const int vg = vec_grid(tot);
  const long first = (p->rank == 0) ? 0 : p->lay.ncp_pad;
  if (compact && first == 0 && tot <= STEP_SMALL_MAX) {
    hipLaunchKernelGGL(k_step_small, dim3(1), dim3(STEP_SMALL_THREADS), 0, p->stream, p->g, p->sinv, p->s, tot, p->scal, (const int*)p->flags, p->fz);
    return CBA_OK;
  }
  hipLaunchKernelGGL(k_step_scalars, dim3(vg), dim3(BLOCK), 0, p->stream, p->g, p->sinv, p->s, tot, first, p->partial4);
  if (compact) {
    hipLaunchKernelGGL(k_step_finish, dim3(1), dim3(BLOCK), 0, p->stream, p->partial4, vg, p->scal, (const int*)p->flags, p->fz);
    return CBA_OK;
  }
  hipLaunchKernelGGL(k_reduce_narrow<false>, dim3(1), dim3(BLOCK), 0, p->stream, p->partial4, vg, 4, p->scal + 16);
  if (formula_w) return exchange(p, SLOT(16) | SLOT(17), false);
  int rcv = allreduce_sum(p, p->scal + 16, 2);
  if (rcv) return rcv;
  hipLaunchKernelGGL(k_w_scalar, dim3(vg), dim3(BLOCK), 0, p->stream, p->g, p->sinv, p->s, tot, first, p->scal + 17, p->gh_sq,
                     (const double*)nullptr, p->partial1);
  hipLaunchKernelGGL(k_reduce_narrow<false>, dim3(1), dim3(BLOCK), 0, p->stream, p->partial1, vg, 1, p->scal + 20);
  return exchange(p, SLOT(20), false);
}

static int maybe_swap_plan(cba_problem* p, bool wait) {
  PlanTask* task = p->plan_task;
  if (!task) return CBA_OK;
  if (wait) task->wait_stage(2);
// ... 91 lines not shown
#ifdef CBA_PROFILING
      if (p->schur_clock) {
        int rcc = run_pairs_clocked<NC>(p);
        if (rcc) return rcc;
      } else
#endif
      hipLaunchKernelGGL((k_schur_reg3<NC, SP, MW>), dim3(p->tile_grid), dim3(Reg3Cfg<NC>::LAUNCH_THREADS), Reg3Cfg<NC>::LDS_BYTES, p->stream, p->tp, p->Trec, p->partial, (const double*)p->tab);
    }
  }
  bool small_solve = false;
  const bool fold_in_finalize = !p->n_heavy && !p->con.n_con && !p->sharded();
  {
    ScopedTimer t(p, T_SCHUR_REDUCE);
    const bool fused_finalize = fold_in_finalize && !(ncp <= SMALL_N && !p->chol_trace) && p->fuse_reg_finalize;
    if (fused_finalize) {
      const int per = REG_REDUCE_Y_MAX / p->reg_reduce_y;
      const int tile_x = (p->gsz * p->gsz * NC * NC + 64 * per - 1) / (64 * per), fold_x = (p->gsz * NC * NC + 63) / 64, rhs_x = (p->lay.ncp_pad + 63) / 64;
      hipLaunchKernelGGL((k_reg_finalize<NC>), dim3(p->G * fold_x + rhs_x + p->n_tiles * tile_x), dim3(64, REG_REDUCE_Y_MAX), 0, p->stream, p->tp, p->tile_wg_begin, p->partial,
                         p->cam_off, p->cam_np, ncp, p->n_tiles, p->G, p->reg_reduce_y, fold_x, rhs_x, tile_x, (const double*)p->partial_b, p->grid, p->lay.ncp_pad, p->Upacked, p->g,
                         p->sinv, lam, lam_dev, p->cam_diag, p->S, p->rhs, p->Lbuf, p->ldw);
    } else {
      hipLaunchKernelGGL(k_reg_reduce, dim3(std::max((p->tp.tile_elems + 63) / 64, (p->lay.ncp_pad + 63) / 64), p->n_tiles + B_SLICES), dim3(64, p->reg_reduce_y), 0,
                         p->stream, p->tp, p->tile_wg_begin, p->partial, p->cam_off, p->cam_np, NC, ncp, p->Sacc, p->red, p->n_tiles,
                         (const double*)p->partial_b, p->grid, p->lay.ncp_pad, p->Sacc + (size_t)ncp * ncp);
      if (!fold_in_finalize)
        hipLaunchKernelGGL(k_reg_fold, dim3((p->gsz * NC * NC + 63) / 64, p->G), dim3(64), 0, p->stream, p->tp, p->red,
                           p->cam_off, p->cam_np, NC, ncp, p->Sacc);
      if (p->n_heavy)
        hipLaunchKernelGGL((k_heavy_schur<NC>), dim3(p->n_heavy), dim3(BLOCK), (size_t)ncp * 3 * sizeof(double) + (size_t)ncp * sizeof(int), p->stream,
                           p->heavy_pts, p->pt_start, p->obs_cam, p->cam_off, p->cam_np, ncp, p->Trec, p->tab, p->heavy_W, p->Sacc);
      if (p->con.n_con) {
        if (p->con.small)
          hipLaunchKernelGGL((k_con_schur_small<NC>), dim3(p->con.n_comp), dim3(BLOCK), (size_t)p->con.small_lds, p->stream, p->con, p->lay, lam, p->V, p->g,
                             p->sinv, p->Trec, p->tab, p->pt_start, p->obs_cam, p->cam_off, p->cam_np, ncp, p->Sacc, p->Sacc + (size_t)ncp * ncp, p->flags);
        else
          hipLaunchKernelGGL((k_con_schur<NC>), dim3(p->con.n_comp), dim3(BLOCK), 0, p->stream, p->con, p->lay, lam, p->V, p->g, p->sinv,
                             p->Trec, p->tab, p->pt_start, p->obs_cam, p->cam_off, p->cam_np, ncp, p->Sacc, p->Sacc + (size_t)ncp * ncp, p->flags);
      }
    }
    if (p->sharded()) {
      const size_t ntri = (size_t)ncp * (ncp + 1) / 2 + ncp;
      const int tg = (int)std::min<size_t>(((size_t)ncp * ncp + ncp + 255) / 256, 1024);
      hipLaunchKernelGGL(k_tri_pack, dim3(tg), dim3(256), 0, p->stream, p->Sacc, p->tri, ncp, 0, p->lay.ncp_pad);
      int rcs = allreduce_sum(p, p->tri, ntri);
      if (rcs) return rcs;
      hipLaunchKernelGGL(k_tri_pack, dim3(tg), dim3(256), 0, p->stream, p->Sacc, p->tri, ncp, 1, p->lay.ncp_pad);
    }
    const long nn = (long)ncp * ncp;
    small_solve = ncp <= SMALL_N && !p->sharded() && !p->chol_trace;
    if (!small_solve && !fused_finalize) {
      hipLaunchKernelGGL((k_schur_finalize<NC>), dim3((int)((nn + 255) / 256)), dim3(256), 0, p->stream, p->Sacc,
                         p->Sacc + (size_t)ncp * ncp, p->Upacked, p->g, p->sinv, p->param_cam, p->param_loc, ncp, lam, lam_dev, p->cam_diag, p->S, p->rhs, p->Lbuf, p->ldw,
                         fold_in_finalize ? (const double*)p->red : (const double*)nullptr, p->tp.g, (long)p->tp.tile_elems, (const int*)p->tp.group_cam_begin,
                         p->lay.ncp_pad);
    }
  }
  int rc = CBA_OK;
  if (small_solve) {
    RoctxRange r2("cba:cholesky");
    ScopedTimer t(p, T_CHOLESKY);
    hipLaunchKernelGGL((k_small_solve<NC>), dim3(1), dim3(SMALL_THREADS), kSmallSolveLds, p->stream, p->Sacc, p->Sacc + (size_t)ncp * ncp, p->Upacked, p->g, p->sinv,
                       p->param_cam, p->param_loc, ncp, lam, lam_dev, p->cam_diag, p->S, p->rhs, fold_in_finalize ? (const double*)p->red : (const double*)nullptr,
                       p->tp.g, (long)p->tp.tile_elems, (const int*)p->tp.group_cam_begin, p->flags, p->s, p->lay.ncp_pad);
  } else {
    RoctxRange r2("cba:cholesky");
    rc = run_cholesky(p);
  }
  if (rc) return rc;
  {
    RoctxRange r2("cba:backsub");
    ScopedTimer t(p, T_BACKSUB);
    if (p->n_heavy)
      hipLaunchKernelGGL(k_zero_heavy, dim3((p->n_heavy + 63) / 64), dim3(64), 0, p->stream, p->heavy_pts, p->n_heavy, p->lay,
                         p->s + p->lay.ncp_pad, 3, p->s + p->lay.ncp_pad, 0);
    auto launch_backsub = [&](auto kernel) {
      hipLaunchKernelGGL(kernel, dim3(p->grid_backsub), dim3(BLOCK), lds_backsub(p), p->stream, p->obs_u, p->obs_v, p->obs_cam,
                         p->obs_pt, p->pt_start, p->chunk_start, p->chunk_pts, p->n_chunks, p->x, p->lay, p->tab, p->cam_off, p->C, p->loss,
                         p->f_scale, lam, lam_dev, p->V, p->g, p->sinv, p->s, p->partial4);
    };
    auto launch_backsub_rec = [&](auto kernel) {
      hipLaunchKernelGGL(kernel, dim3(p->grid_backsub), dim3(BLOCK), lds_backsub_rec<NC>(p), p->stream, (const double*)p->Trec, (const int*)p->obs_cam,
                         (const int*)p->pt_start, (const int*)p->chunk_start, (const int*)p->chunk_pts, p->n_chunks, p->lay, (const double*)p->tab,
                         (const int*)p->cam_off, (const int*)p->cam_np, p->C, lam, lam_dev, (const double*)p->V, (const double*)p->g,
                         (const double*)p->sinv, p->s, p->partial4);
    };
    if (p->backsub_rec) { if (fused_trial(p, compact)) launch_backsub_rec(k_backsub_rec<NC, true>); else launch_backsub_rec(k_backsub_rec<NC, false>); }
    else if (fused_trial(p, compact)) { if (p->tab_global) launch_backsub(k_backsub<NC, true, true>); else launch_backsub(k_backsub<NC, false, true>); }
    else if (p->tab_global) launch_backsub(k_backsub<NC, true>); else launch_backsub(k_backsub<NC>);
    if (p->n_heavy)
      hipLaunchKernelGGL(k_heavy_finish, dim3((p->n_heavy + 63) / 64), dim3(64), 0, p->stream, p->heavy_pts, p->heavy_frag, p->n_heavy, p->lay, lam,
                         p->V, p->g, p->sinv, p->s);
    if (p->con.n_con) {
      if (p->n_con_orphan)
        hipLaunchKernelGGL(k_con_orphan_start, dim3((p->n_con_orphan + 63) / 64), dim3(64), 0, p->stream, (const int*)p->con_orphan, p->n_con_orphan, p->lay,
                           lam, (const double*)p->V, (const double*)p->g, (const double*)p->sinv, p->s);
      if (p->con.small)
        hipLaunchKernelGGL(k_con_backsub_small, dim3(p->con.n_comp), dim3(BLOCK), (size_t)(9 * p->con.max_np + 2 * p->con.max_m) * sizeof(double), p->stream,
                           p->con, p->lay, lam, p->V, p->sinv, p->s);
      else
        hipLaunchKernelGGL(k_con_backsub, dim3(p->con.n_comp), dim3(BLOCK), 0, p->stream, p->con, p->lay, lam, p->V, p->sinv, p->s);
    }
  }
  if (fused_trial(p, compact)) {
    ScopedTimer t(p, T_VECTOR);
    hipLaunchKernelGGL(k_step_cam, dim3(1), dim3(BLOCK), (size_t)p->lay.ncp_pad * sizeof(double), p->stream, (const double*)p->partial4, p->grid_backsub,
                       (const double*)p->x, (const double*)p->g, (const double*)p->sinv, (const double*)p->s, p->lay.ncp_pad, p->scal, (const int*)p->flags, p->fz,
                       p->x_new, p->partial4 + p->grid, p->tab_new, (const double*)p->cam_const, (const int*)p->cam_model, (const int*)p->cam_np,
                       (const int*)p->cam_off, p->C, p->bounds_on ? (const double*)p->lb_dev : (const double*)nullptr,
                       p->bounds_on ? (const double*)p->ub_dev : (const double*)nullptr, p->ncp);
    return CBA_OK;
  }
  return run_step_scalars(p, lam_dev != nullptr, compact);
}

static void read_newton(cba_problem* p, cba_newton_info* out) {
  out->ok = (p->h_flags[1] == 0 && p->h_flags[2] == 0) ? 1 : 0;
  out->p_sq = p->h_scal[16];
  out->gh_dot_p = p->h_scal[17];
  out->w_sq = p->h_scal[20];
  if (out->ok && !(std::isfinite(out->p_sq) && std::isfinite(out->gh_dot_p) && std::isfinite(out->w_sq))) out->ok = 0;
}

template <int NC>
static int run_newton(cba_problem* p, double lam, cba_newton_info* out) {
  int rc = run_newton_chain<NC>(p, lam, nullptr);
  if (rc) return rc;
  rc = sync_scalars(p, 24);
  if (rc) return rc;
  read_newton(p, out);
  return CBA_OK;
}

template <int NC>
static int step_enqueue(cba_problem* p, double radius, bool compact, unsigned long long* seq_out) {
  int rc = run_lin_chain<NC>(p, true, compact, radius, compact && !p->det_m);
  if (rc) return rc;
  if (!compact) hipLaunchKernelGGL(k_fused_lam, dim3(1), dim3(1), 0, p->stream, p->scal, radius, p->fz);
  rc = run_newton_chain<NC>(p, 0.0, p->fz, compact);
  if (rc) return rc;
  if (!compact) hipLaunchKernelGGL(k_fused_subspace, dim3(1), dim3(1), 0, p->stream, p->scal, p->flags, p->fz);
  const long tot = p->lay.total();
  const int vg = vec_grid(tot);
  const bool ft = fused_trial(p, compact);
  if (!ft) {
    ScopedTimer t(p, T_VECTOR);
    hipLaunchKernelGGL(k_trial_update, dim3(vg), dim3(BLOCK), 0, p->stream, p->x, p->g, p->sinv, p->s, 0.0, 0.0, tot, p->lay.ncp_pad,
                       p->rank == 0 ? 1 : 0, (const double*)nullptr, 0, (const double*)(p->fz + 2), p->x_new, p->partial4, p->tab_new,
                       (const double*)p->cam_const, (const int*)p->cam_model, (const int*)p->cam_np, (const int*)p->cam_off, p->C);
    if (!compact) hipLaunchKernelGGL(k_reduce_narrow<false>, dim3(1), dim3(BLOCK), 0, p->stream, p->partial4, vg, 1, p->scal + 28);
  }
  const TrialSrc tsrc{p->x, p->g, p->sinv, p->s, p->fz + 2, p->x_new, p->partial4};
  const unsigned long long seq = compact ? ++p->publish_seq : 0;
  const bool bnd = compact && p->bounds_on;
  const PubArgs pub{p->scal, 48, p->flags, p->d_hscal, p->d_hflags, seq, p->partial1, p->grid, 24, p->partial4, ft ? p->grid + 1 : vg, 28,
                    {p->x, p->g, p->sinv_state_c, p->s}, bnd ? p->d_hbcam : (double*)nullptr, p->ncp};
  rc = run_build_into<NC>(p, p->x_new, p->tab_new, p->V2, p->g2, p->U2, 24, p->scal + 42, true, compact, 0, ft ? &tsrc : nullptr,
                          compact ? &pub : nullptr);
  if (rc) return rc;
  if (!compact) return CBA_OK;
  *seq_out = seq;
  p->spec_enqueued = false;
  {
    {
      ScopedTimer t(p, T_SCALE_SCALARS);
      const BoundArgs ba2 = bnd ? BoundArgs{p->lb_dev, p->ub_dev, p->sinv_state_c, p->sinv_state_c2, p->cam_diag2} : BoundArgs{};
      auto launch_sl2 = [&](auto kernel) {
        hipLaunchKernelGGL(kernel, dim3(vg), dim3(BLOCK), 0, p->stream, p->U2, p->V2, p->param_cam, p->param_loc, p->lay, 0, p->sinv2,
                           (const double*)nullptr, p->x_new, p->g2, p->v1, p->partial4b, p->partial1, (const double*)p->sinv, ba2);
      };
      if (bnd) launch_sl2(k_scale_lin<NC, true>); else launch_sl2(k_scale_lin<NC, false>);
      int rows_jv = 0;
      rc = run_jv<NC>(p, 1, &rows_jv, p->x_new, p->tab_new);
      p->spec_rows_jv = rows_jv;
    }
    if (rc) return rc;
    p->spec_enqueued = true;
  }
  return CBA_OK;
}

template <int NC>
static int run_step(cba_problem* p, double radius, cba_step_info* out) {
  RoctxRange range("cba:step");
  const bool compact = !p->sharded();
  int rc;
  if (compact) {
    unsigned long long seq = 0;
    rc = step_enqueue<NC>(p, radius, true, &seq);
    if (rc) return rc;
    rc = publish_wait(p, seq, !p->spec_enqueued);
  } else {
    unsigned long long seq = 0;
    rc = step_enqueue<NC>(p, radius, false, &seq);
    if (rc) return rc;
    rc = exchange_at(p, SLOT(24) | SLOT(28), false, p->U2, (size_t)p->C * UPack<NC>::STRIDE);
    if (rc) return rc;
    hipLaunchKernelGGL((k_unpack_camera_grad<NC>), dim3((p->C * NC + 255) / 256), dim3(256), 0, p->stream, p->U2, p->cam_off, p->cam_np, p->C, p->g2);
    rc = sync_scalars(p, 48);
  }
  if (rc) return rc;
  const int bad_residual = p->h_flags[0];
  read_linearization(p, &out->lin);
  read_newton(p, &out->newton);
  out->lam = p->h_scal[40]; out->radius = p->h_scal[41];
  out->need_host = (int)p->h_scal[42];
  out->p_s[0] = p->h_scal[43]; out->p_s[1] = p->h_scal[44]; out->predicted = p->h_scal[45];
  out->alpha = p->h_scal[46]; out->beta = p->h_scal[47];
  if (const char* e = std::getenv("CBA_TEST_FAIL_FUSED_STEP")) {
    static std::atomic<long> n_fused{0};
    if (++n_fused == std::atol(e)) {
      out->newton.ok = 0; out->need_host = 1;
      if (p->bounds_on) for (int i = 0; i < p->ncp; ++i) p->h_bcam[(size_t)3 * p->ncp + i] = NAN;
    }
  }
  const double c = 0.5 * p->h_scal[24];
  out->trial.finite = (bad_residual == 0 && std::isfinite(c)) ? 1 : 0;
  out->trial.cost = out->trial.finite ? c : NAN;
  out->trial.step_norm = std::sqrt(p->h_scal[28]);
  out->trial.reserved = 0;
  p->trial_cost = c;
  return CBA_OK;
}

#define DISPATCH_NC(p, call6, call9) ((p)->nct == 9 ? (call9) : (call6))

extern "C" {

static int begin_common(cba_problem* p, double* cost_out, bool evaluate = true);

int cba_set_constraints(cba_problem* p, int32_t n_con, const int32_t* groups_a, const int32_t* groups_b, const double* distances,
                        const double* weights) {
  if (!p) return fail(CBA_ERR_INVALID, "cba_set_constraints: null problem");
  if (p->begun) return fail(CBA_ERR_INVALID, "cba_set_constraints: call it before cba_begin");
  if (p->con.n_con) return fail(CBA_ERR_INVALID, "cba_set_constraints: constraints are already set");
  if (n_con <= 0) return CBA_OK;
  if (!groups_a || !groups_b || !distances || !weights) return fail(CBA_ERR_INVALID, "cba_set_constraints: null array");
  HIPCHK(hipSetDevice(p->device));
  const auto t_enter = std::chrono::steady_clock::now();
  auto lap_ms = [&](std::chrono::steady_clock::time_point since) { return std::chrono::duration<double, std::milli>(std::chrono::steady_clock::now() - since).count(); };
  HostConPlan plan;
  int rc = constraint_plan(fail, p->P, p->ncp, n_con, groups_a, groups_b, distances, weights, CON_LDS_POINTS, plan);
  if (rc) return rc;
  const int K = plan.n_comp, max_pts = plan.max_pts;
  const long max_m = plan.max_m;
  std::vector<int> orphan;
  {
    std::vector<int> hps((size_t)p->P + 1);
    HIPCHK(hipStreamSynchronize(p->stream));
    HIPCHK(hipMemcpy(hps.data(), p->pt_start, hps.size() * sizeof(int), hipMemcpyDeviceToHost));
    orphan = constraint_orphans(plan.comp_pts, hps.data());
  }
  const double ms_graph = lap_ms(t_enter);
  const auto t_up = std::chrono::steady_clock::now();
  upload_stage_acquire(p);
  int *dpt = nullptr, *dlp = nullptr, *dorder = nullptr, *dcc = nullptr, *dcp = nullptr, *dcps = nullptr, *dorphan = nullptr;
  long* dcm = nullptr;
  double *ddist = nullptr, *dw = nullptr;
#define TRYC(e) do { rc = (e); if (rc) return rc; } while (0)
  TRYC(dev_upload(p, &dpt, plan.pt)); TRYC(dev_upload(p, &dlp, plan.lp)); TRYC(dev_upload(p, &dorder, plan.order)); TRYC(dev_upload(p, &dcc, plan.comp_con));
  TRYC(dev_upload(p, &dcp, plan.comp_pt)); TRYC(dev_upload(p, &dcps, plan.comp_pts)); TRYC(dev_upload(p, &dcm, plan.comp_m));
  TRYC(dev_upload(p, &ddist, plan.dist)); TRYC(dev_upload(p, &dw, plan.wgt));
  if (!orphan.empty()) TRYC(dev_upload(p, &dorphan, orphan));
  ConPlan cp{};
  cp.n_con = n_con; cp.n_comp = K; cp.pt = dpt; cp.lp = dlp; cp.dist = ddist; cp.weight = dw; cp.order = dorder;
  cp.comp_con = dcc; cp.comp_pt = dcp; cp.comp_pts = dcps; cp.comp_m = dcm;
  cp.heavy_pts = p->heavy_pts; cp.heavy_W = p->heavy_W; cp.n_heavy = p->n_heavy;
  TRYC(dev_alloc(p, &cp.f, (size_t)n_con)); TRYC(dev_alloc(p, &cp.u, (size_t)n_con * 3)); TRYC(dev_alloc(p, &cp.z, (size_t)n_con * 24));
  TRYC(dev_alloc(p, &cp.M, (size_t)std::max<long>(plan.comp_m[K], 1))); TRYC(dev_alloc(p, &cp.G, (size_t)n_con * (p->ncp + 1)));
  TRYC(dev_alloc(p, &cp.cdiag, (size_t)3 * p->lay.Ppad)); TRYC(dev_alloc(p, &cp.w, (size_t)n_con));
  if (plan.big) TRYC(dev_alloc(p, &cp.big, plan.comp_pts.size() * 9));
#undef TRYC
  const double ms_upload = lap_ms(t_up);
  const auto t_attr = std::chrono::steady_clock::now();
  {
    cp.max_m = (int)max_m; cp.max_np = max_pts;
    const ConSmallLayout lo((int)max_m, max_pts, p->ncp);
    cp.small_lds = lo.total * (int)sizeof(double);
    const char* e = std::getenv("CBA_CON_SMALL");
    cp.small = (max_m <= CON_SMALL_M && !p->n_heavy && cp.small_lds <= 120 * 1024 && !(e && e[0] == '0')) ? 1 : 0;
    if (cp.small) {
      int rcl = (p->nct == 9) ? allow_lds(k_con_schur_small<9>, (size_t)cp.small_lds) : allow_lds(k_con_schur_small<6>, (size_t)cp.small_lds);
      if (!rcl) rcl = allow_lds(k_con_backsub_small, (size_t)(9 * max_pts + 2 * max_m) * sizeof(double));
      if (rcl) return rcl;
    }
  }
  const double ms_attr = lap_ms(t_attr);
  const auto t_sync = std::chrono::steady_clock::now();
  HIPCHK(hipMemsetAsync(cp.cdiag, 0, (size_t)3 * p->lay.Ppad * sizeof(double), p->stream));
  HIPCHK(hipStreamSynchronize(p->stream));
  upload_stage_release(p);
  if (plan_timing_on())
    fprintf(stderr, "  cba_set_constraints: %d rows, %d components: graph %.3f ms, uploads + allocations %.3f, kernel attributes %.3f, memset + sync %.3f\n", n_con, K,
            ms_graph, ms_upload, ms_attr, lap_ms(t_sync));
  p->con = cp;
  p->con_orphan = dorphan; p->n_con_orphan = (int)orphan.size();
  p->con_grid = std::max(1, std::min((n_con + BLOCK - 1) / BLOCK, CON_ROWS));
  return CBA_OK;
}

int cba_begin(cba_problem* p, const double* x0, double* cost_out) {
  if (!p || !x0 || !cost_out) return fail(CBA_ERR_INVALID, "cba_begin: null argument");
  HIPCHK(hipSetDevice(p->device));
  { const int rcw = stage_wait(p); if (rcw) return rcw; }
  pack_host(p, x0, p->h_vec, 0.0);
  HIPCHK(hipMemcpyAsync(p->x0, p->h_vec, p->lay.total() * sizeof(double), hipMemcpyHostToDevice, p->stream));
  { const int rcs = stage_sent(p); if (rcs) return rcs; }
  p->have_x0 = true;
  return begin_common(p, cost_out);
}

int cba_restart(cba_problem* p, double* cost_out) {
  if (!p || !cost_out) return fail(CBA_ERR_INVALID, "cba_restart: null argument");
  if (!p->have_x0) return fail(CBA_ERR_INVALID, "cba_restart: call cba_begin first");
  HIPCHK(hipSetDevice(p->device));
  return begin_common(p, cost_out);
}

int cba_begin_deferred(cba_problem* p, const double* x0) {
  if (!p) return fail(CBA_ERR_INVALID, "cba_begin_deferred: null argument");
  if (!x0 && !p->have_x0) return fail(CBA_ERR_INVALID, "cba_begin_deferred: no x0 on the device yet");
  HIPCHK(hipSetDevice(p->device));
  if (x0) {
    { const int rcw = stage_wait(p); if (rcw) return rcw; }
    pack_host(p, x0, p->h_vec, 0.0);
    HIPCHK(hipMemcpyAsync(p->x0, p->h_vec, p->lay.total() * sizeof(double), hipMemcpyHostToDevice, p->stream));
    { const int rcs = stage_sent(p); if (rcs) return rcs; }
    p->have_x0 = true;
  }
  return begin_common(p, nullptr, false);
}

static int begin_common(cba_problem* p, double* cost_out, bool evaluate) {
  p->cam_scaled = false; p->cam_state_saved = false;
  p->have_build = false; p->trial_built = false; p->cost_pending = false; p->lf_pending = false;
  {
    ScopedTimer t(p, T_CAM_PREP);
    double* trial_buf = (!p->eval_only && fused_trial(p, true)) ? p->x_new : nullptr;
    hipLaunchKernelGGL(k_begin, dim3(std::max(vec_grid(p->lay.total()), (p->C + BLOCK - 1) / BLOCK)), dim3(BLOCK), 0, p->stream, (const double*)p->x0, p->x, trial_buf,
                       p->sinv, p->cam_diag, p->flags, p->lay.total(), p->lay.ncp_pad, (const double*)p->cam_const, (const int*)p->cam_model, (const int*)p->cam_np,
                       (const int*)p->cam_off, p->C, p->tab);
  }
  p->first_scale = true;
  p->begun = true; p->linearized = false; p->stepped = false; p->have_trial = false;
  if (!evaluate) {
    p->cost_x = NAN;
    return CBA_OK;
  }
  int rc = launch_cost(p, p->x, p->tab, 24, nullptr);
  if (rc) return rc;
  rc = exchange(p, SLOT(24), false);
  if (rc) return rc;
  rc = sync_scalars(p, 32);
  if (rc) return rc;
  HIPCHK(hipGetLastError());
  *cost_out = p->h_flags[0] ? NAN : 0.5 * p->h_scal[24];
  p->cost_x = *cost_out;
  return CBA_OK;
}

int cba_linearize(cba_problem* p, cba_linearization* out) {
  if (!p || !out) return fail(CBA_ERR_INVALID, "cba_linearize: null argument");
  if (p->eval_only) return fail(CBA_ERR_INVALID, "cba_linearize: the problem was created with evaluation_only");
  if (!p->begun) return fail(CBA_ERR_INVALID, "cba_linearize: call cba_begin first");
  HIPCHK(hipSetDevice(p->device));
  int rc = DISPATCH_NC(p, run_linearize<6>(p, out), run_linearize<9>(p, out));
  if (rc) return rc;
  HIPCHK(hipGetLastError());
  p->linearized = true; p->stepped = false;
  return CBA_OK;
}

int cba_linearize_build(cba_problem* p) {
  if (!p) return fail(CBA_ERR_INVALID, "cba_linearize_build: null argument");
  if (!p->begun) return fail(CBA_ERR_INVALID, "cba_linearize_build: call cba_begin first");
  if (p->eval_only) return fail(CBA_ERR_INVALID, "cba_linearize_build: the problem was created with evaluation_only");
  HIPCHK(hipSetDevice(p->device));
  int rc = DISPATCH_NC(p, run_lin_chain<6>(p, false), run_lin_chain<9>(p, false));
  if (rc) return rc;
  HIPCHK(hipGetLastError());
  p->linearized = true; p->stepped = false;
  return CBA_OK;
}

int cba_newton_step(cba_problem* p, double lam, cba_newton_info* out) {
  if (!p || !out) return fail(CBA_ERR_INVALID, "cba_newton_step: null argument");
  if (!p->linearized) return fail(CBA_ERR_INVALID, "cba_newton_step: call cba_linearize first");
  if (!(lam >= 0.0) || !std::isfinite(lam)) return fail(CBA_ERR_INVALID, "cba_newton_step: lam must be finite and >= 0");
  HIPCHK(hipSetDevice(p->device));
  int rc = DISPATCH_NC(p, run_newton<6>(p, lam, out), run_newton<9>(p, lam, out));
  if (rc) return rc;
  HIPCHK(hipGetLastError());
  p->stepped = true;
  return CBA_OK;
}

int cba_step(cba_problem* p, double radius, cba_step_info* out) {
  if (!p || !out) return fail(CBA_ERR_INVALID, "cba_step: null argument");
  if (!p->begun) return fail(CBA_ERR_INVALID, "cba_step: call cba_begin first");
  if (!cba_step_supported(p)) return fail(CBA_ERR_UNSUPPORTED, "cba_step: not available for this problem (constraint rows, heavy points, or bound scaling without cba_set_bounds): use the primitives");
  HIPCHK(hipSetDevice(p->device));
  int rc = DISPATCH_NC(p, run_step<6>(p, radius, out), run_step<9>(p, radius, out));
  if (rc) return rc;
  HIPCHK(hipGetLastError());
  p->linearized = true; p->stepped = true;
  p->have_trial = out->need_host == 0;
  p->trial_built = p->have_trial;
  return CBA_OK;
}

int cba_set_bounds(cba_problem* p, const double* lb, const double* ub) {
  if (!p) return fail(CBA_ERR_INVALID, "cba_set_bounds: null argument");
  if (!lb || !ub) { p->bounds_on = false; return 0; }
  if (p->eval_only || p->sharded() || !fused_trial(p, true)) { p->bounds_on = false; return 0; }
  HIPCHK(hipSetDevice(p->device));
  HIPCHK(hipMemcpyAsync(p->lb_dev, lb, (size_t)p->ncp * sizeof(double), hipMemcpyHostToDevice, p->stream));
  HIPCHK(hipMemcpyAsync(p->ub_dev, ub, (size_t)p->ncp * sizeof(double), hipMemcpyHostToDevice, p->stream));
  HIPCHK(hipStreamSynchronize(p->stream));
  p->bounds_on = true;
  return 1;
}

int cba_step_camera_state(cba_problem* p, double* x_c, double* g_c, double* scale_inv_c, double* step_c) {
  if (!p || !x_c || !g_c || !scale_inv_c || !step_c) return fail(CBA_ERR_INVALID, "cba_step_camera_state: null argument");
  if (!p->bounds_on || !p->stepped) return fail(CBA_ERR_INVALID, "cba_step_camera_state: no bounded cba_step to report on");
  const size_t n = (size_t)p->ncp;
  std::memcpy(x_c, p->h_bcam, n * sizeof(double)); std::memcpy(g_c, p->h_bcam + n, n * sizeof(double));
  std::memcpy(scale_inv_c, p->h_bcam + 2 * n, n * sizeof(double)); std::memcpy(step_c, p->h_bcam + 3 * n, n * sizeof(double));
  return CBA_OK;
}

int cba_refresh_step_scalars(cba_problem* p, cba_newton_info* out) {
  if (!p || !out) return fail(CBA_ERR_INVALID, "cba_refresh_step_scalars: null argument");
  if (!p->stepped) return fail(CBA_ERR_INVALID, "cba_refresh_step_scalars: no damped step to measure");
  HIPCHK(hipSetDevice(p->device));
  const int f1 = p->h_flags[1], f2 = p->h_flags[2];
  int rc = run_step_scalars(p, false);
  if (!rc) rc = sync_scalars(p, 24);
  if (rc) return rc;
  p->h_flags[1] = f1; p->h_flags[2] = f2;
  read_newton(p, out);
  return CBA_OK;
}

int cba_step_supported(cba_problem* p) {
  return (p && !p->eval_only && !p->con.n_con && !p->n_heavy && (!p->cam_scaled || (p->bounds_on && !p->sharded())) && !p->peer_needs_primitives) ? 1 : 0;
}

static int upload_cam(cba_problem* p, const double* host, double* dev) {
  HIPCHK(hipMemcpyAsync(dev, host, (size_t)p->ncp * sizeof(double), hipMemcpyHostToDevice, p->stream));
  return CBA_OK;
}

int cba_subspace_gram_ex(cba_problem* p, double a1, double b1, const double* cam1, double a2, double b2, const double* cam2,
                         double* gram_out) {
  if (!p || !gram_out) return fail(CBA_ERR_INVALID, "cba_subspace_gram: null argument");
  if (!p->stepped) return fail(CBA_ERR_INVALID, "cba_subspace_gram: call cba_newton_step first");
  HIPCHK(hipSetDevice(p->device));
  const long tot = p->lay.total();
  if (cam1) { int rc = upload_cam(p, cam1, p->cam_over1); if (rc) return rc; }
  if (cam2) { int rc = upload_cam(p, cam2, p->cam_over2); if (rc) return rc; }
  {
    ScopedTimer t(p, T_VECTOR);
    hipLaunchKernelGGL(k_combine, dim3(vec_grid(tot)), dim3(BLOCK), 0, p->stream, p->g, p->sinv, p->s, a1, b1, tot,
                       (const double*)p->cam_over1, cam1 ? p->lay.ncp_pad : 0, p->v1);
    hipLaunchKernelGGL(k_combine, dim3(vec_grid(tot)), dim3(BLOCK), 0, p->stream, p->g, p->sinv, p->s, a2, b2, tot,
                       (const double*)p->cam_over2, cam2 ? p->lay.ncp_pad : 0, p->v2);
  }
  DISPATCH_NC(p, run_jv<6>(p, 2), run_jv<9>(p, 2));
  int rc = exchange(p, SLOT(12) | SLOT(13) | SLOT(14) | SLOT(15), false);
  if (!rc) rc = sync_scalars(p, 16);
  if (rc) return rc;
  HIPCHK(hipGetLastError());
  gram_out[0] = p->h_scal[12]; gram_out[1] = p->h_scal[13]; gram_out[2] = p->h_scal[14];
  return CBA_OK;
}

int cba_subspace_gram(cba_problem* p, double a1, double b1, double a2, double b2, double* gram_out) {
  return cba_subspace_gram_ex(p, a1, b1, nullptr, a2, b2, nullptr, gram_out);
}

int cba_set_camera_scaling(cba_problem* p, const double* mult, const double* diag_h, cba_linearization* out) {
  if (!p || !mult || !diag_h || !out) return fail(CBA_ERR_INVALID, "cba_set_camera_scaling: null argument");
  if (!p->linearized) return fail(CBA_ERR_INVALID, "cba_set_camera_scaling: call cba_linearize first");
  for (int i = 0; i < p->ncp; ++i)
    if (!(mult[i] > 0.0) || !std::isfinite(mult[i]) || !(diag_h[i] >= 0.0) || !std::isfinite(diag_h[i]))
      return fail(CBA_ERR_INVALID, "cba_set_camera_scaling: entry %d: mult must be positive and diag_h non-negative (finite)", i);
  HIPCHK(hipSetDevice(p->device));
  const int npad = p->lay.ncp_pad;
  if (!p->cam_state_saved) {
    HIPCHK(hipMemcpyAsync(p->sinv_state_c, p->sinv, (size_t)npad * sizeof(double), hipMemcpyDeviceToDevice, p->stream));
    p->cam_state_saved = true;
  }
  int rc = upload_cam(p, mult, p->cam_over1);
  if (!rc) rc = upload_cam(p, diag_h, p->cam_over2);
  if (rc) return rc;
  const long tot = p->lay.total();
  const int vg = vec_grid(tot);
  {
    ScopedTimer t(p, T_SCALE_SCALARS);
    hipLaunchKernelGGL(k_cam_rescale, dim3((p->ncp + 255) / 256), dim3(256), 0, p->stream, p->sinv_state_c, p->cam_over1, p->cam_over2, p->ncp,
                       p->sinv, p->cam_diag);
    hipLaunchKernelGGL(k_lin_scalars, dim3(vg), dim3(BLOCK), 0, p->stream, p->x, p->g, p->sinv, tot, npad, p->rank == 0 ? 1 : 0, npad,
                       p->v1, p->partial4, p->partial1);
    hipLaunchKernelGGL(k_reduce_narrow<false>, dim3(1), dim3(BLOCK), 0, p->stream, p->partial4, vg, 4, p->scal + 0);
    hipLaunchKernelGGL(k_reduce_narrow<true>, dim3(1), dim3(BLOCK), 0, p->stream, p->partial1, vg, 1, p->scal + 4);
  }
  rc = DISPATCH_NC(p, run_jv<6>(p, 1), run_jv<9>(p, 1));
  if (rc) return rc;
  rc = exchange(p, SLOT(0) | SLOT(1) | SLOT(2) | SLOT(3) | SLOT(12) | SLOT(13) | SLOT(14) | SLOT(15), true);
  if (!rc) rc = sync_scalars(p, 16);
  if (rc) return rc;
  HIPCHK(hipGetLastError());
  p->cam_scaled = true; p->stepped = false;
  read_linearization(p, out);
  return CBA_OK;
}

int cba_trial(cba_problem* p, double alpha, double beta, cba_trial_info* out) { return cba_trial_ex(p, alpha, beta, nullptr, out); }

int cba_trial_ex(cba_problem* p, double alpha, double beta, const double* cam_x_new, cba_trial_info* out) {
  if (!p || !out) return fail(CBA_ERR_INVALID, "cba_trial: null argument");
  if (!p->stepped) return fail(CBA_ERR_INVALID, "cba_trial: call cba_newton_step first");
  HIPCHK(hipSetDevice(p->device));
  const long tot = p->lay.total();
  const int vg = vec_grid(tot);
  if (cam_x_new) { int rcu = upload_cam(p, cam_x_new, p->cam_over1); if (rcu) return rcu; }
  {
    ScopedTimer t(p, T_VECTOR);
    hipLaunchKernelGGL(k_trial_update, dim3(vg), dim3(BLOCK), 0, p->stream, p->x, p->g, p->sinv, p->s, alpha, beta, tot, p->lay.ncp_pad,
                       p->rank == 0 ? 1 : 0, (const double*)p->cam_over1, cam_x_new ? p->ncp : 0, (const double*)nullptr, p->x_new, p->partial4);
    if (p->sharded()) hipLaunchKernelGGL(k_reduce_narrow<false>, dim3(1), dim3(BLOCK), 0, p->stream, p->partial4, vg, 1, p->scal + 28);
  }
  launch_cam_prep(p, p->x_new, p->tab_new);
  int rc;
  if (p->sharded()) {
    rc = launch_cost(p, p->x_new, p->tab_new, 24, nullptr);
    if (rc) return rc;
    rc = exchange(p, SLOT(24) | SLOT(28), false);
    if (rc) return rc;
    rc = sync_scalars(p, 32);
  } else {
    int cost_rows = 0;
    rc = launch_cost(p, p->x_new, p->tab_new, 24, nullptr, &cost_rows);
    if (rc) return rc;
    rc = sync_scalars(p, 32, p->partial1, cost_rows, 24, p->partial4, vg, 28);
  }
  if (rc) return rc;
  HIPCHK(hipGetLastError());
  const double c = 0.5 * p->h_scal[24];
  out->finite = (p->h_flags[0] == 0 && std::isfinite(c)) ? 1 : 0;
  out->cost = out->finite ? c : NAN;
  out->step_norm = std::sqrt(p->h_scal[28]);
  p->have_trial = true; p->trial_built = false; p->trial_cost = c;
  return CBA_OK;
}

int cba_accept(cba_problem* p) {
  if (!p) return fail(CBA_ERR_INVALID, "cba_accept: null argument");
  if (!p->have_trial) return fail(CBA_ERR_INVALID, "cba_accept: no trial point");
  std::swap(p->x, p->x_new);
  std::swap(p->tab, p->tab_new);
  p->spec_valid = false;
  if (p->trial_built) {
    std::swap(p->V, p->V2); std::swap(p->g, p->g2); std::swap(p->Upacked, p->U2);
    p->cost_x = p->trial_cost;
    if (p->spec_enqueued) {
      std::swap(p->sinv, p->sinv2); p->spec_valid = true;
      if (p->bounds_on) { std::swap(p->sinv_state_c, p->sinv_state_c2); std::swap(p->cam_diag, p->cam_diag2); }
    }
  }
  p->spec_enqueued = false;
  p->have_build = p->trial_built;
  p->trial_built = false;
  p->have_trial = false; p->linearized = false; p->stepped = false;
  return CBA_OK;
}

int cba_comm_unique_id(char* out128) {
  if (!out128) return fail(CBA_ERR_INVALID, "cba_comm_unique_id: null argument");
  static_assert(sizeof(ncclUniqueId) <= 128, "ncclUniqueId larger than 128 bytes");
  ncclUniqueId id;
  NCCLCHK(ncclGetUniqueId(&id));
  std::memset(out128, 0, 128);
  std::memcpy(out128, &id, sizeof(id));
  return CBA_OK;
}

int cba_comm_init(cba_problem* p, const char* id128, int32_t rank, int32_t world) {
  if (!p || !id128) return fail(CBA_ERR_INVALID, "cba_comm_init: null argument");
  if (world < 1 || rank < 0 || rank >= world) return fail(CBA_ERR_INVALID, "cba_comm_init: rank %d of %d", rank, world);
  if (p->comm.load()) return fail(CBA_ERR_INVALID, "cba_comm_init: communicator already initialised");
  if (p->comm_aborted.load()) return fail(CBA_ERR_COMM, "cba_comm_init: a peer rank failed before the communicator was created");
  HIPCHK(hipSetDevice(p->device));
  p->rank = rank; p->world = world;
  const char* force = std::getenv("CBA_FORCE_COMM");
  const bool forced = force && force[0] == '1';
  if (world == 1 && !forced) return CBA_OK;
  ncclUniqueId id;
  std::memcpy(&id, id128, sizeof(id));
  {
    ncclComm_t c = nullptr;
    NCCLCHK(ncclCommInitRank(&c, world, id, rank));
    p->comm.store(c);
  }
  {
    const double mine = cba_step_supported(p) ? 0.0 : 1.0;
    HIPCHK(hipMemcpyAsync(p->xbuf, &mine, sizeof(double), hipMemcpyHostToDevice, p->stream));
    NCCLCHK(ncclAllReduce(p->xbuf, p->xbuf, 1, ncclDouble, ncclSum, p->comm.load(), p->stream));
    double total = 0.0;
    HIPCHK(hipMemcpyAsync(&total, p->xbuf, sizeof(double), hipMemcpyDeviceToHost, p->stream));
    HIPCHK(hipStreamSynchronize(p->stream));
    p->peer_needs_primitives = total > 0.0;
  }
  return CBA_OK;
}

int cba_comm_abort(cba_problem* p) {
  if (!p) return fail(CBA_ERR_INVALID, "cba_comm_abort: null problem");
  p->comm_aborted.store(true, std::memory_order_release);
  if (ncclComm_t c = p->comm.exchange(nullptr)) (void)ncclCommAbort(c);
  return CBA_OK;
}

int cba_group_create(int32_t world, cba_group** out) {
  if (!out) return fail(CBA_ERR_INVALID, "cba_group_create: null argument");
  *out = nullptr;
  if (world < 1 || world > GROUP_MAX) return fail(CBA_ERR_INVALID, "cba_group_create: world %d (1..%d)", world, GROUP_MAX);
  cba_group* g = new cba_group();
  g->world = world;
  if (const char* e = std::getenv("CBA_GROUP_TIMEOUT_S")) g->timeout_s = std::max(1, std::atoi(e));
  g->member.assign(world, nullptr);
  for (int par = 0; par < 2; ++par) {
    g->stage[par].assign(world, nullptr);
    g->ready[par].assign(world, nullptr);
    g->done[par].assign(world, nullptr);
  }
  *out = g;
  return CBA_OK;
}

int cba_group_join(cba_problem* p, cba_group* g, int32_t rank) {
  if (!p || !g) return fail(CBA_ERR_INVALID, "cba_group_join: null argument");
  if (rank < 0 || rank >= g->world) return fail(CBA_ERR_INVALID, "cba_group_join: rank %d of %d", rank, g->world);
  if (p->comm.load() || p->group) return fail(CBA_ERR_INVALID, "cba_group_join: the handle already belongs to a communicator");
  int rc = CBA_OK;
  {
    if (hipSetDevice(p->device) != hipSuccess) rc = fail(CBA_ERR_HIP, "hipSetDevice(%d) failed", p->device);
    const size_t ustride = (p->nct == 9) ? UPack<9>::STRIDE : UPack<6>::STRIDE;
    const size_t cap = std::max<size_t>((size_t)p->ncp * p->ncp + p->lay.ncp_pad, (size_t)p->C * ustride + 128) + 128;
    for (int par = 0; par < 2 && !rc; ++par) {
      if (hipMalloc((void**)&g->stage[par][rank], cap * sizeof(double)) != hipSuccess) { rc = fail(CBA_ERR_HIP, "staging allocation failed"); break; }
      if (hipEventCreateWithFlags(&g->ready[par][rank], hipEventDisableTiming) != hipSuccess ||
          hipEventCreateWithFlags(&g->done[par][rank], hipEventDisableTiming) != hipSuccess) { rc = fail(CBA_ERR_HIP, "hipEventCreate failed"); break; }
      (void)hipEventRecord(g->ready[par][rank], p->stream);
      (void)hipEventRecord(g->done[par][rank], p->stream);
    }
    if (rank == 0) g->capacity = cap;
    g->member[rank] = p;
  }
  if (rc) g->failed.store(1);
  if (!g->barrier()) return fail(CBA_ERR_INVALID, "cba_group_join: the group was aborted (another rank failed before joining)");
  if (g->failed.load()) return rc ? rc : fail(CBA_ERR_HIP, "cba_group_join: another rank failed to join");
  {
    for (int q = 0; q < g->world && !rc; ++q) {
      const int dq = g->member[q]->device;
      if (dq == p->device) continue;
      int can = 0;
      if (hipDeviceCanAccessPeer(&can, p->device, dq) != hipSuccess || !can) { rc = fail(CBA_ERR_HIP, "device %d cannot access device %d", p->device, dq); break; }
      const hipError_t e = hipDeviceEnablePeerAccess(dq, 0);
      if (e != hipSuccess && e != hipErrorPeerAccessAlreadyEnabled) { rc = fail(CBA_ERR_HIP, "hipDeviceEnablePeerAccess(%d) failed: %s", dq, hipGetErrorString(e)); break; }
      (void)hipGetLastError();
    }
  }
  if (rc) g->failed.store(1);
  if (!g->barrier()) return fail(CBA_ERR_INVALID, "cba_group_join: the group was aborted");
  if (g->failed.load()) return rc ? rc : fail(CBA_ERR_HIP, "cba_group_join: another rank failed to join");
  p->group = g; p->rank = rank; p->world = g->world; p->group_generation = 0;
  {
    const double mine = cba_step_supported(p) ? 0.0 : 1.0;
    double total = 0.0;
    HIPCHK(hipMemcpyAsync(p->xbuf, &mine, sizeof(double), hipMemcpyHostToDevice, p->stream));
    int rca = allreduce_sum(p, p->xbuf, 1);
    if (rca) return rca;
    HIPCHK(hipMemcpyAsync(&total, p->xbuf, sizeof(double), hipMemcpyDeviceToHost, p->stream));
    HIPCHK(hipStreamSynchronize(p->stream));
    p->peer_needs_primitives = total > 0.0;
  }
  if (p->world == 1) { p->group = nullptr; }
  return CBA_OK;
}

void cba_group_abort(cba_group* g) { if (g) g->aborted.store(1, std::memory_order_release); }

void cba_group_destroy(cba_group* g) {
  if (!g) return;
  for (int par = 0; par < 2; ++par)
    for (int q = 0; q < g->world; ++q) {
      if (g->stage[par][q]) (void)hipFree(g->stage[par][q]);
      if (g->ready[par][q]) (void)hipEventDestroy(g->ready[par][q]);
      if (g->done[par][q]) (void)hipEventDestroy(g->done[par][q]);
    }
  delete g;
}

static int fetch_camera_blocks(cba_problem* p, const double* const* srcs, double* const* outs) {
  const int ncp = p->ncp;
  unsigned long long* hseq = reinterpret_cast<unsigned long long*>(p->h_cam + (size_t)3 * ncp);
  unsigned long long* dseq = reinterpret_cast<unsigned long long*>(p->d_hcam + (size_t)3 * ncp);
  const unsigned long long seq = ++p->publish_seq;
  hipLaunchKernelGGL(k_publish_cam, dim3(1), dim3(BLOCK), 0, p->stream, srcs[0], srcs[1], srcs[2], ncp, p->d_hcam, dseq, seq);
  if (p->spin_wait) {
    volatile unsigned long long* flag = hseq;
    const auto t0 = std::chrono::steady_clock::now();
    for (unsigned spins = 0; *flag != seq; ++spins)
      if ((spins & 0xfff) == 0xfff && std::chrono::steady_clock::now() - t0 > std::chrono::seconds(2)) {
        HIPCHK(hipStreamSynchronize(p->stream));
        if (*flag != seq) return fail(CBA_ERR_HIP, "k_publish_cam did not complete");
        break;
      }
    std::atomic_thread_fence(std::memory_order_acquire);
  } else {
    HIPCHK(hipStreamSynchronize(p->stream));
  }
  for (int v = 0; v < 3; ++v)
    if (outs[v]) std::memcpy(outs[v], p->h_cam + (size_t)v * ncp, (size_t)ncp * sizeof(double));
  return CBA_OK;
}
// ... 144 lines not shown
```

caliscope_amd/csrc/cba_solve.cpp:

```cpp
#include <algorithm>
#include <chrono>
#include <cmath>
#include <cstdio>
#include <cstdlib>
#include <cstring>
#include <vector>

#include "../../include/caliscope_ba.h"
#include "scale_math.h"
#include "trf_math.h"

namespace {

constexpr double SUBSPACE_EXPLICIT_BELOW = 1e-6;

using trf::solve_subspace_2d;

int termination(double dF, double F, double dx_norm, double x_norm, double ratio, double ftol, double xtol) {
  const bool f_ok = dF < ftol * F && ratio > 0.25;
  const bool x_ok = dx_norm < xtol * (xtol + x_norm);
  if (f_ok && x_ok) return 4;
  if (f_ok) return 2;
  if (x_ok) return 3;
  return -100;
}


struct CamBlock {
  int n = 0;
  const double *lb = nullptr, *ub = nullptr;
  std::vector<double> x, g, sinv, s, mult, diag_h, d, gh, p, ph, r, step, x_new;
  std::vector<char> hit;
  void resize(int ncp) {
    n = ncp;
    for (std::vector<double>* v : {&x, &g, &sinv, &s, &mult, &diag_h, &d, &gh, &p, &ph, &r, &step, &x_new}) v->assign(n, 0.0);
    hit.assign(n, 0);
  }
};

double step_size_to_bound(const CamBlock& cb, const double* x, const double* s, char* hit) {
  double best = INFINITY;
  for (int i = 0; i < cb.n; ++i)
    if (s[i] != 0.0) best = std::min(best, std::max((cb.lb[i] - x[i]) / s[i], (cb.ub[i] - x[i]) / s[i]));
  if (hit)
    for (int i = 0; i < cb.n; ++i) hit[i] = (s[i] != 0.0 && std::max((cb.lb[i] - x[i]) / s[i], (cb.ub[i] - x[i]) / s[i]) == best) ? 1 : 0;
  return best;
}

void minimize_quadratic_1d(double a, double b, double lo, double hi, double c, double* t_best, double* y_best) {
  double t[3] = {lo, hi, 0.0};
  int nt = 2;
  if (a != 0.0) {
    const double ext = -0.5 * b / a;
    if (lo < ext && ext < hi) t[nt++] = ext;
  }
  *y_best = INFINITY;
  for (int i = 0; i < nt; ++i) {
    const double y = t[i] * (a * t[i] + b) + c;
    if (y < *y_best) { *y_best = y; *t_best = t[i]; }
  }
}

struct CallTrace {
  struct Row { const char* name; double s; long n; double longest; };
  bool on = std::getenv("CBA_SOLVE_TRACE") != nullptr;
  Row rows[24];
  int used = 0;
  template <class F> int run(const char* name, F&& f) {
    if (!on) return f();
    const auto t0 = std::chrono::steady_clock::now();
    const int rc = f();
    const double dt = std::chrono::duration<double>(std::chrono::steady_clock::now() - t0).count();
    int i = 0;
    while (i < used && std::strcmp(rows[i].name, name) != 0) ++i;
    if (i == used) { if (used == 24) return rc; rows[used++] = Row{name, 0.0, 0, 0.0}; }
    rows[i].s += dt; ++rows[i].n;
    if (dt > rows[i].longest) rows[i].longest = dt;
    return rc;
  }
  void print(double total_s, long iterations) const {
    if (!on) return;
    double sum = 0.0;
    for (int i = 0; i < used; ++i) sum += rows[i].s;
    std::fprintf(stderr, "cba_solve trace: %ld iterations, %.3f ms, of which %.3f ms inside the primitives\n", iterations, total_s * 1e3, sum * 1e3);
    for (int i = 0; i < used; ++i) std::fprintf(stderr, "  %-22s %5ld calls %9.3f ms  %8.1f us each, longest %8.1f us\n", rows[i].name, rows[i].n, rows[i].s * 1e3, rows[i].s * 1e6 / rows[i].n, rows[i].longest * 1e6);
  }
};

}

extern "C" int cba_solve(cba_problem* p, const double* x0, const cba_solve_options* opt_in, double* x_out, cba_result* out) {
  if (!p || !out) return cba_set_error(CBA_ERR_INVALID, "cba_solve: null argument");
  cba_solve_options opt;
  if (opt_in) opt = *opt_in;
  else { opt.ftol = opt.xtol = opt.gtol = 1e-8; opt.max_nfev = 0; opt.lb = opt.ub = nullptr; opt.verbose = 0; opt.max_damping_retries = 12; }
  const double eps = 2.220446049250313e-16;
  if (opt.ftol < eps && opt.xtol < eps && opt.gtol < eps)
    return cba_set_error(CBA_ERR_INVALID, "cba_solve: at least one of the tolerances must be higher than machine epsilon");
  cba_info info;
  int rc = cba_get_info(p, &info);
  if (rc) return rc;
  const long n_params = info.n_params;
  const int ncp = info.n_cam_params;
  const long max_nfev = opt.max_nfev > 0 ? opt.max_nfev : 100 * n_params;
  const int max_retries = opt.max_damping_retries > 0 ? opt.max_damping_retries : 12;
  bool bounded = false;
  if (opt.lb && opt.ub)
    for (int i = 0; i < ncp; ++i) {
      if (!(opt.lb[i] < opt.ub[i])) return cba_set_error(CBA_ERR_INVALID, "cba_solve: each lower bound must be strictly less than each upper bound");
      bounded = bounded || std::isfinite(opt.lb[i]) || std::isfinite(opt.ub[i]);
    }
  CamBlock cb;
  if (bounded) { cb.resize(ncp); cb.lb = opt.lb; cb.ub = opt.ub; }
  const auto t_begin = std::chrono::steady_clock::now();
  CallTrace calls;

  auto not_finite_at_x0 = [&](double c) {
    out->status = -1; out->reserved = 0; out->nfev = 1; out->njev = 0; out->n_iterations = 0; out->cost = c; out->optimality = NAN;
    out->t_rejected_s = 0.0; out->n_rejected_timed = 0;
    out->t_total_s = std::chrono::duration<double>(std::chrono::steady_clock::now() - t_begin).count();
    return CBA_OK;
  };
  double cost = NAN;
  const bool deferred = !bounded;
  if (deferred) rc = calls.run("begin_deferred", [&] { return cba_begin_deferred(p, x0); });
  else rc = x0 ? calls.run("begin", [&] { return cba_begin(p, x0, &cost); }) : calls.run("restart", [&] { return cba_restart(p, &cost); });
  if (rc) return rc;
  if (!deferred && !std::isfinite(cost)) return not_finite_at_x0(cost);
  if (bounded) {
    if ((rc = calls.run("get_camera_params", [&] { return cba_get_camera_params(p, CBA_VEC_X, cb.x.data()); }))) return rc;
    for (int i = 0; i < ncp; ++i)
      if (!(cb.x[i] > cb.lb[i] && cb.x[i] < cb.ub[i])) return cba_set_error(CBA_ERR_INVALID, "cba_solve: x0 is not strictly inside the bounds");
  }
  long nfev = 1, njev = 1, iteration = 0;
  double t_rejected = 0.0;
  long n_rejected_timed = 0;
  int n_truncated = 0, n_reflected = 0, n_gradient = 0;
  bool bounds_on_device = false;
  if (bounded) {
    const int rb = cba_set_bounds(p, cb.lb, cb.ub);
    if (rb < 0) return rb;
    bounds_on_device = rb == 1;
  } else {
    (void)cba_set_bounds(p, nullptr, nullptr);
  }
  bool fused = (!bounded || bounds_on_device) && cba_step_supported(p);
  bool fuse_next = fused;
  int n_outside = 0;
  cba_linearization lin;
  cba_step_info si;
  bool lin_valid = false;
  double radius = NAN;
  int status = -100;
  double g_norm = NAN, step_norm = NAN, actual = NAN;
  if (opt.verbose == 2) std::printf("%15s%15s%15s%15s%15s%15s\n", "Iteration", "Total nfev", "Cost", "Cost reduction", "Step norm", "Optimality");

  for (;;) {
    double C_gg = 0.0;
    bool have_step = false;
    if (!lin_valid) {
      if (status == -100 && fuse_next && nfev < max_nfev) {
        if ((rc = calls.run("step", [&] { return cba_step(p, std::isnan(radius) ? -1.0 : radius, &si); }))) return rc;
        lin = si.lin; have_step = true;
      } else if (bounded) {
        fuse_next = false;
        if ((rc = calls.run("linearize_build", [&] { return cba_linearize_build(p); }))) return rc;
      } else if ((rc = calls.run("linearize", [&] { return cba_linearize(p, &lin); }))) return rc;
      lin_valid = true;
      if (std::isnan(cost)) {
        cost = lin.cost;
        if (!std::isfinite(cost)) return not_finite_at_x0(cost);
      }
    }
    if (bounded && have_step && si.need_host == 2) {
      lin_valid = false; fuse_next = false;
      if (++n_outside >= 2) fused = false;
      continue;
    }
    if (bounded) {
      if (have_step) {
        if ((rc = cba_step_camera_state(p, cb.x.data(), cb.g.data(), cb.sinv.data(), cb.s.data()))) return rc;
      } else if ((rc = calls.run("get_camera_state", [&] { return cba_get_camera_state(p, cb.x.data(), cb.g.data(), cb.sinv.data()); }))) return rc;
      double gv_max = 0.0;
      for (int i = 0; i < ncp; ++i) {
        double v = 1.0, dv = 0.0;
        if (cb.g[i] < 0 && std::isfinite(cb.ub[i])) { v = cb.ub[i] - cb.x[i]; dv = -1.0; }
        else if (cb.g[i] > 0 && std::isfinite(cb.lb[i])) { v = cb.x[i] - cb.lb[i]; dv = 1.0; }
        gv_max = std::max(gv_max, std::fabs(cb.g[i] * v));
        if (dv != 0.0) v *= cb.sinv[i];
        cb.mult[i] = 1.0 / std::sqrt(v);
        cb.diag_h[i] = cb.g[i] * dv / cb.sinv[i];
        cb.d[i] = 1.0 / (cb.sinv[i] * cb.mult[i]);
        cb.gh[i] = cb.g[i] * cb.d[i];
        C_gg += cb.diag_h[i] * cb.gh[i] * cb.gh[i];
      }
      if (!have_step && (rc = calls.run("set_camera_scaling", [&] { return cba_set_camera_scaling(p, cb.mult.data(), cb.diag_h.data(), &lin); }))) return rc;
      g_norm = std::max(gv_max, lin.g_norm_inf);
    } else {
      g_norm = lin.g_norm_inf;
    }
    if (std::isnan(radius)) radius = lin.x_scaled_norm > 0 ? lin.x_scaled_norm : 1.0;
    if (g_norm < opt.gtol) status = 1;
    if (opt.verbose == 2) {
      std::printf("%15ld%15ld%15.4e", iteration, nfev, cost);
      if (std::isnan(actual)) std::printf("%15s%15s", "", ""); else std::printf("%15.2e%15.2e", actual, step_norm);
      std::printf("%15.2e\n", g_norm);
    }
    if (status != -100 || nfev >= max_nfev) break;
    const double theta = std::max(0.995, 1.0 - g_norm);

    const double gh_sq = lin.gh_sq, gh_norm = std::sqrt(gh_sq);
    const double H_gg = lin.jg_sq + C_gg;
    double lam = trf::damping(H_gg, gh_sq, radius);
    cba_newton_info st;
    if (have_step) {
      lam = si.lam; st = si.newton;
      if (si.need_host && st.ok && (rc = calls.run("refresh_step_scalars", [&] { return cba_refresh_step_scalars(p, &st); }))) return rc;
    } else if ((rc = calls.run("newton_step", [&] { return cba_newton_step(p, lam, &st); }))) return rc;
    bool first_trial_ready = have_step && st.ok && !si.need_host;
    bool refetch_step = !have_step;
    if (calls.on) std::fprintf(stderr, "  iteration %ld: lam %.3e radius %.3e ok %d%s\n", iteration, lam, radius, st.ok, have_step ? " (fused)" : "");
    for (int retries = 0; !st.ok;) {
      if (++retries > max_retries) return cba_set_error(CBA_ERR_NUMERIC, "cba_solve: normal equations could not be factorised even with heavy damping");
      lam = std::max(lam * 10.0, 1e-14 * std::pow(10.0, retries));
      if ((rc = calls.run("newton_step", [&] { return cba_newton_step(p, lam, &st); }))) return rc;
      refetch_step = true;
      if (calls.on) std::fprintf(stderr, "    retry %d: lam %.3e ok %d\n", retries, lam, st.ok);
    }
    if (bounded && refetch_step && (rc = calls.run("get_camera_params", [&] { return cba_get_camera_params(p, CBA_VEC_STEP, cb.s.data()); }))) return rc;
    const double c = st.gh_dot_p / gh_sq, w_sq = st.w_sq;
    const bool two_d = w_sq > 0.0 && w_sq > 1e-30 * st.p_sq;
    const double w_norm = two_d ? std::sqrt(w_sq) : 1.0;
    double b00, b01 = 0.0, b11;
    if (!two_d) {
      b00 = H_gg / gh_sq; b11 = 1.0;
    } else if (w_sq > SUBSPACE_EXPLICIT_BELOW * st.p_sq) {
      trf::subspace_model(H_gg, gh_sq, lam, st.gh_dot_p, st.p_sq, w_sq, &b00, &b01, &b11);
    } else {
      double gram[3];
      if ((rc = calls.run("subspace_gram", [&] { return cba_subspace_gram(p, 1.0 / gh_norm, 0.0, -c / w_norm, 1.0 / w_norm, gram); }))) return rc;
      b00 = gram[0]; b01 = gram[1]; b11 = gram[2];
      for (int i = 0; i < cb.n; ++i) {
        const double q1 = cb.gh[i] / gh_norm, q2 = (cb.s[i] / cb.d[i] - c * cb.gh[i]) / w_norm;
        b00 += cb.diag_h[i] * q1 * q1; b01 += cb.diag_h[i] * q1 * q2; b11 += cb.diag_h[i] * q2 * q2;
      }
    }
    actual = -1.0;
    double cost_new = cost;
    bool first_pass = true;
    while (actual <= 0 && nfev < max_nfev) {
      double pS[2];
      if (first_pass && first_trial_ready) { pS[0] = si.p_s[0]; pS[1] = si.p_s[1]; }
      else {
        solve_subspace_2d(b00, b01, b11, gh_norm, 0.0, radius, pS);
        if (!two_d) pS[1] = 0.0;
      }
      const double quad_p = 0.5 * (pS[0] * (b00 * pS[0] + b01 * pS[1]) + pS[1] * (b01 * pS[0] + b11 * pS[1]));
      const double lin_p = gh_norm * pS[0];
      const double beta = two_d ? pS[1] / w_norm : 0.0;
      const double alpha = pS[0] / gh_norm - beta * c;
      double predicted = -(quad_p + lin_p), step_h_norm = std::hypot(pS[0], pS[1]);
      cba_trial_info tr;
      const auto t_trial = std::chrono::steady_clock::now();
      bool own_call = true;
      if (first_pass && first_trial_ready) {
        own_call = false;
        tr = si.trial; predicted = si.predicted;
      } else if (!bounded) {
        if ((rc = calls.run("trial", [&] { return cba_trial(p, alpha, beta, &tr); }))) return rc;
      } else {
        double pt_alpha = alpha, pt_beta = beta;
        bool inside = true;
        for (int i = 0; i < ncp; ++i) {
          cb.p[i] = alpha * cb.g[i] * cb.d[i] * cb.d[i] + beta * cb.s[i];
          cb.step[i] = cb.p[i];
          const double xn = cb.x[i] + cb.p[i];
          inside = inside && xn >= cb.lb[i] && xn <= cb.ub[i];
        }
        if (!inside) {
          const double p_norm2 = pS[0] * pS[0] + pS[1] * pS[1];
          const double p_stride = step_size_to_bound(cb, cb.x.data(), cb.p.data(), cb.hit.data());
          double hit_ph2 = 0.0, hit_gh_ph = 0.0, C_pp = 0.0, C_hit = 0.0;
          for (int i = 0; i < ncp; ++i) {
            cb.ph[i] = cb.p[i] / cb.d[i];
            cb.r[i] = cb.hit[i] ? -cb.p[i] : cb.p[i];
            C_pp += cb.diag_h[i] * cb.ph[i] * cb.ph[i];
            if (cb.hit[i]) { hit_ph2 += cb.ph[i] * cb.ph[i]; hit_gh_ph += cb.gh[i] * cb.ph[i]; C_hit += cb.diag_h[i] * cb.ph[i] * cb.ph[i]; }
          }
          const double ph_dot_rh = p_norm2 - 2.0 * hit_ph2, C_pr = C_pp - 2.0 * C_hit, C_rr = C_pp;
          double to_tr = 0.0;
          {
            const double a = p_norm2, b = p_stride * ph_dot_rh, cq = p_stride * p_stride * p_norm2 - radius * radius;
            const double disc = std::sqrt(std::max(0.0, b * b - a * cq));
            const double q = -(b + std::copysign(disc, b));
            if (a > 0.0 && q != 0.0) to_tr = std::max(q / a, cq / q);
          }
          for (int i = 0; i < ncp; ++i) cb.x_new[i] = cb.x[i] + p_stride * cb.p[i];
          const double to_bound = step_size_to_bound(cb, cb.x_new.data(), cb.r.data(), nullptr);
          double r_stride = std::min(to_bound, to_tr), r_lo, r_hi, r_value = INFINITY;
          if (r_stride > 0) { r_lo = (1.0 - theta) * p_stride / r_stride; r_hi = (r_stride == to_bound) ? theta * to_bound : to_tr; }
          else { r_lo = 0.0; r_hi = -1.0; }
          if (r_lo <= r_hi) {
            double gram[3];
            if ((rc = calls.run("subspace_gram_ex", [&] { return cba_subspace_gram_ex(p, alpha, beta, nullptr, alpha, beta, cb.r.data(), gram); }))) return rc;
            const double qa = 0.5 * (gram[2] + C_rr);
            const double qb = (lin_p - 2.0 * hit_gh_ph) + p_stride * (gram[1] + C_pr);
            const double qc = 0.5 * p_stride * p_stride * (gram[0] + C_pp) + p_stride * lin_p;
            minimize_quadratic_1d(qa, qb, r_lo, r_hi, qc, &r_stride, &r_value);
          }
          const double kappa = theta * p_stride;
          const double p_value = kappa * kappa * quad_p + kappa * lin_p;
          for (int i = 0; i < ncp; ++i) cb.x_new[i] = -cb.g[i] * cb.d[i] * cb.d[i];
          const double ag_to_tr = radius / gh_norm, ag_to_bound = step_size_to_bound(cb, cb.x.data(), cb.x_new.data(), nullptr);
          double ag_stride, ag_value;
          minimize_quadratic_1d(0.5 * H_gg, -gh_sq, 0.0, ag_to_bound < ag_to_tr ? theta * ag_to_bound : ag_to_tr, 0.0, &ag_stride, &ag_value);
          if (p_value < r_value && p_value < ag_value) {
            ++n_truncated;
            pt_alpha = kappa * alpha; pt_beta = kappa * beta;
            for (int i = 0; i < ncp; ++i) cb.step[i] = kappa * cb.p[i];
            predicted = -p_value; step_h_norm = kappa * std::sqrt(p_norm2);
          } else if (r_value < p_value && r_value < ag_value) {
            ++n_reflected;
            pt_alpha = (p_stride + r_stride) * alpha; pt_beta = (p_stride + r_stride) * beta;
            for (int i = 0; i < ncp; ++i) cb.step[i] = p_stride * cb.p[i] + r_stride * cb.r[i];
            predicted = -r_value;
            step_h_norm = std::sqrt(std::max(0.0, (p_stride * p_stride + r_stride * r_stride) * p_norm2 + 2.0 * p_stride * r_stride * ph_dot_rh));
          } else {
            ++n_gradient;
            pt_alpha = -ag_stride; pt_beta = 0.0;
            for (int i = 0; i < ncp; ++i) cb.step[i] = ag_stride * cb.x_new[i];
            predicted = -ag_value; step_h_norm = ag_stride * gh_norm;
          }
        }
        for (int i = 0; i < ncp; ++i) {
          double xn = cb.x[i] + cb.step[i];
          if (xn <= cb.lb[i]) xn = std::nextafter(cb.lb[i], cb.ub[i]);
          else if (xn >= cb.ub[i]) xn = std::nextafter(cb.ub[i], cb.lb[i]);
          cb.x_new[i] = xn;
        }
        if ((rc = calls.run("trial_ex", [&] { return cba_trial_ex(p, pt_alpha, pt_beta, cb.x_new.data(), &tr); }))) return rc;
      }
      ++nfev;
      const bool was_first = first_pass;
      first_pass = false;
      const double dt_trial = std::chrono::duration<double>(std::chrono::steady_clock::now() - t_trial).count();
      if (!tr.finite) { radius = 0.25 * step_h_norm; if (was_first) fuse_next = false; if (own_call) { t_rejected += dt_trial; ++n_rejected_timed; } continue; }
      cost_new = tr.cost;
      actual = cost - cost_new;
      if (own_call && !(actual > 0)) { t_rejected += dt_trial; ++n_rejected_timed; }
      if (was_first) fuse_next = fused && actual > 0 && w_sq > 1e-2 * st.p_sq;
      double ratio;
      if (predicted > 0) ratio = actual / predicted;
      else if (predicted == 0 && actual == 0) ratio = 1.0;
      else ratio = 0.0;
      double radius_new = radius;
      if (ratio < 0.25) radius_new = 0.25 * step_h_norm;
      else if (ratio > 0.75 && step_h_norm > 0.95 * radius) radius_new = 2.0 * radius;
      step_norm = tr.step_norm;
      status = termination(actual, cost, step_norm, lin.x_norm, ratio, opt.ftol, opt.xtol);
      if (status != -100) break;
      radius = radius_new;
    }
    if (actual > 0) {
      if ((rc = calls.run("accept", [&] { return cba_accept(p); }))) return rc;
      cost = cost_new;
      lin_valid = false;
      ++njev;
    } else {
      step_norm = 0.0; actual = 0.0;
    }
    ++iteration;
  }
  if (status == -100) status = 0;
  if (x_out && (rc = calls.run("get_vector", [&] { return cba_get_vector(p, CBA_VEC_X, x_out); }))) return rc;
  out->status = std::isfinite(cost) ? status : -1;
  out->reserved = std::min(n_truncated, 1023) | (std::min(n_reflected, 1023) << 10) | (std::min(n_gradient, 1023) << 20);
  out->nfev = nfev; out->njev = njev; out->n_iterations = iteration;
  out->cost = cost; out->optimality = g_norm;
  out->t_total_s = std::chrono::duration<double>(std::chrono::steady_clock::now() - t_begin).count();
  out->t_rejected_s = t_rejected; out->n_rejected_timed = n_rejected_timed;
  calls.print(out->t_total_s, iteration);
  return CBA_OK;
}

extern "C" int cba_scale_errors(const cba_scale_desc* d, int32_t device, double* stats_out) {
  if (!d || !stats_out) return cba_set_error(CBA_ERR_INVALID, "cba_scale_errors: null argument");
  if (d->n_groups < 0 || d->n_world < 0 || !d->group_start) return cba_set_error(CBA_ERR_INVALID, "cba_scale_errors: bad descriptor");
  if (d->n_groups == 0) return CBA_OK;
  const int64_t n_groups = d->n_groups, n_ent = d->group_start[n_groups];
  if (n_ent > 0 && (!d->ent_world || !d->ent_obj || !d->world_xyz)) return cba_set_error(CBA_ERR_INVALID, "cba_scale_errors: bad descriptor");
  if (n_groups > ((int64_t)1 << 30)) return cba_set_error(CBA_ERR_UNSUPPORTED, "cba_scale_errors: more than 2^30 groups");
  cba::ScalePlan plan;
  std::string msg;
  const int prc = cba::scale_plan(d->n_world, n_groups, d->group_start, d->ent_world, plan, msg);
  if (prc) return cba_set_error(prc == -4 ? CBA_ERR_UNSUPPORTED : CBA_ERR_INVALID, msg.c_str());
  if (!cba_scale_launch) return cba_set_error(CBA_ERR_UNSUPPORTED, "cba_scale_errors: this build has no device kernels");
  std::vector<int64_t> list;
  list.reserve((size_t)n_groups);
  for (const auto* v : {&plan.small, &plan.lds_small, &plan.lds_large, &plan.direct}) list.insert(list.end(), v->begin(), v->end());
  const int64_t counts[4] = {(int64_t)plan.small.size(), (int64_t)plan.lds_small.size(), (int64_t)plan.lds_large.size(), (int64_t)plan.direct.size()};
  return cba_scale_launch(d, device, list.data(), counts, stats_out);
}
```

caliscope_amd/csrc/trf_math.h:

```cpp
#pragma once
#include <math.h>

#ifdef __HIPCC__
#define TRF_HD __host__ __device__
#else
#define TRF_HD
#endif

namespace trf {

TRF_HD inline double min_quadratic_on_segment(double a, double b, double hi) {
  double best = fmin(0.0, hi * (a * hi + b));
  if (a != 0.0) {
    const double t = -0.5 * b / a;
    if (t > 0.0 && t < hi) best = fmin(best, t * (a * t + b));
  }
  return best;
}

constexpr double DAMPING_FLOOR = 1e-13;
TRF_HD inline double damping(double H_gg, double gh_sq, double radius) {
  const double lam = -min_quadratic_on_segment(0.5 * H_gg, -gh_sq, radius / sqrt(gh_sq)) / (radius * radius);
  return lam > DAMPING_FLOOR ? lam : DAMPING_FLOOR;
}

TRF_HD inline double poly_eval(const double* c, int deg, double t) {
  double p = c[0];
  for (int i = 1; i <= deg; ++i) p = p * t + c[i];
  return p;
}

template <int DEG>
TRF_HD inline int real_roots_of_degree(const double* c, double* out) {
  static_assert(DEG >= 1 && DEG <= 4, "quartics at most");
  if constexpr (DEG == 1) {
    out[0] = -c[1] / c[0];
    return 1;
  } else if constexpr (DEG == 2) {
    const double disc = c[1] * c[1] - 4.0 * c[0] * c[2];
    if (disc < 0.0) return 0;
    const double q = -0.5 * (c[1] + copysign(sqrt(disc), c[1]));
    int n = 0;
    if (q != 0.0) { out[n++] = q / c[0]; out[n++] = c[2] / q; }
    else { out[n++] = 0.0; }
    return n;
  } else {
    double d[DEG], crit[DEG - 1];
    for (int i = 0; i < DEG; ++i) d[i] = c[i] * (DEG - i);
    int nc = real_roots_of_degree<DEG - 1>(d, crit);
    for (int i = 1; i < nc; ++i)
      for (int j = i; j > 0 && crit[j] < crit[j - 1]; --j) { const double t = crit[j]; crit[j] = crit[j - 1]; crit[j - 1] = t; }
    double bound = 0.0;
    for (int i = 1; i <= DEG; ++i) bound = fmax(bound, fabs(c[i] / c[0]));
    bound += 1.0;
    double knots[DEG + 1];
    int nk = 0;
    knots[nk++] = -bound;
    for (int i = 0; i < nc; ++i)
      if (crit[i] > -bound && crit[i] < bound) knots[nk++] = crit[i];
    knots[nk++] = bound;
    int n = 0;
    double scale = 0.0;
    for (int i = 0; i <= DEG; ++i) scale = fmax(scale, fabs(c[i]));
    for (int k = 0; k + 1 < nk; ++k) {
      double a = knots[k], b = knots[k + 1];
      double fa = poly_eval(c, DEG, a), fb = poly_eval(c, DEG, b);
      if (fa == 0.0) { out[n++] = a; continue; }
      if (k + 2 == nk && fb == 0.0) { out[n++] = b; continue; }
      if ((fa < 0.0) == (fb < 0.0)) {
        if (k > 0 && fabs(fa) <= 1e-14 * scale * fmax(1.0, pow(fabs(a), (double)DEG))) out[n++] = a;
        continue;
      }
      for (int it = 0; it < 200 && b - a > 0.0; ++it) {
        const double m = 0.5 * (a + b);
        if (m == a || m == b) break;
        const double fm = poly_eval(c, DEG, m);
        if (fm == 0.0) { a = b = m; break; }
        if ((fm < 0.0) == (fa < 0.0)) { a = m; fa = fm; } else { b = m; }
      }
      out[n++] = 0.5 * (a + b);
      if (n >= DEG) break;
    }
    return n;
  }
}

TRF_HD inline int real_roots(const double* c_in, int n_coef, double* out) {
  int lead = 0;
  while (lead < n_coef && c_in[lead] == 0.0) ++lead;
  switch (n_coef - 1 - lead) {
    case 4: return real_roots_of_degree<4>(c_in + lead, out);
    case 3: return real_roots_of_degree<3>(c_in + lead, out);
    case 2: return real_roots_of_degree<2>(c_in + lead, out);
    case 1: return real_roots_of_degree<1>(c_in + lead, out);
    default: return 0;
  }
}

TRF_HD inline void solve_subspace_2d(double b00, double b01, double b11, double g0, double g1, double radius, double* p) {
  if (b00 > 0.0) {
    const double schur = b11 - b01 * b01 / b00;
    if (schur > 0.0) {
      const double det = b00 * schur;
      const double p0 = -(b11 * g0 - b01 * g1) / det, p1 = -(b00 * g1 - b01 * g0) / det;
      if (p0 * p0 + p1 * p1 <= radius * radius) { p[0] = p0; p[1] = p1; return; }
    }
  }
  const double r2 = radius * radius;
  const double a = b00 * r2, b = b01 * r2, c = b11 * r2, d = g0 * radius, f = g1 * radius;
  const double coef[5] = {-b + d, 2.0 * (a - c + f), 6.0 * b, 2.0 * (-a + c + f), -b - d};
  double t[4];
  const int nt = real_roots(coef, 5, t);
  if (nt == 0) {
    const double n = hypot(g0, g1);
    p[0] = n > 0 ? -radius * g0 / n : 0.0;
    p[1] = n > 0 ? -radius * g1 / n : 0.0;
    return;
  }
  double best = INFINITY;
  for (int i = 0; i <= nt; ++i) {
    double c0, c1;
    if (i < nt) { const double q = 1.0 + t[i] * t[i]; c0 = radius * 2.0 * t[i] / q; c1 = radius * (1.0 - t[i] * t[i]) / q; }
    else { c0 = 0.0; c1 = -radius; }
    const double val = 0.5 * (c0 * (b00 * c0 + b01 * c1) + c1 * (b01 * c0 + b11 * c1)) + g0 * c0 + g1 * c1;
    if (val < best) { best = val; p[0] = c0; p[1] = c1; }
  }
}

TRF_HD inline void subspace_model(double H_gg, double gh_sq, double lam, double gh_dot_p, double p_sq, double w_sq, double* b00,
                                  double* b01, double* b11) {
  const double c = gh_dot_p / gh_sq, gh_norm = sqrt(gh_sq), w_norm = sqrt(w_sq);
  const double H_gp = -gh_sq - lam * gh_dot_p, H_pp = -gh_dot_p - lam * p_sq;
  *b00 = H_gg / gh_sq;
  *b01 = (H_gp - c * H_gg) / (gh_norm * w_norm);
  *b11 = (H_pp - 2.0 * c * H_gp + c * c * H_gg) / w_sq;
}

}
```

include/caliscope_ba.h:

```cpp
#ifndef CALISCOPE_BA_H
#define CALISCOPE_BA_H

#include <stdint.h>

#ifdef __cplusplus
extern "C" {
#endif

#define CBA_VERSION 100

enum {
  CBA_OK = 0,
  CBA_ERR_INVALID = -1,
  CBA_ERR_NO_DEVICE = -2,
  CBA_ERR_HIP = -3,
  CBA_ERR_UNSUPPORTED = -4,
  CBA_ERR_COMM = -5,
  CBA_ERR_NUMERIC = -6
};

enum { CBA_MODEL_PINHOLE_BC5 = 0, CBA_MODEL_FISHEYE4 = 1 };
enum { CBA_LOSS_LINEAR = 0, CBA_LOSS_HUBER = 1, CBA_LOSS_SOFT_L1 = 2, CBA_LOSS_CAUCHY = 3, CBA_LOSS_ARCTAN = 4 };

typedef struct cba_problem cba_problem;

typedef struct {
  int32_t n_cams;
  int32_t n_points;
  int64_t n_obs;
  const int32_t* cam_n_params;
  const int32_t* cam_model;
  const double* cam_const;
  const int32_t* obs_cam;
  const int32_t* obs_pt;
  const double* obs_uv;
  int32_t loss;
  double f_scale;
} cba_problem_desc;

typedef struct {
  int32_t device_id;
  int32_t max_blocks;
  int32_t deterministic;
  int32_t evaluation_only;
} cba_options;

int cba_create(const cba_problem_desc* desc, const cba_options* opt, cba_problem** out);
void cba_destroy(cba_problem* p);

int cba_comm_unique_id(char* out128);
int cba_comm_init(cba_problem* p, const char* id128, int32_t rank, int32_t world);
int cba_comm_abort(cba_problem* p);

typedef struct cba_group cba_group;
int cba_group_create(int32_t world, cba_group** out);
int cba_group_join(cba_problem* p, cba_group* g, int32_t rank);
void cba_group_abort(cba_group* g);
void cba_group_destroy(cba_group* g);


int cba_begin(cba_problem* p, const double* x0, double* cost_out);

int cba_restart(cba_problem* p, double* cost_out);

int cba_begin_deferred(cba_problem* p, const double* x0);

typedef struct {
  double g_norm_inf;
  double gh_sq;
  double jg_sq;
  double x_scaled_norm;
  double x_norm;
  double cost;
} cba_linearization;

int cba_linearize(cba_problem* p, cba_linearization* out);

typedef struct {
  int32_t ok;
  int32_t reserved;
  double p_sq;
  double gh_dot_p;
  double w_sq;
} cba_newton_info;

int cba_newton_step(cba_problem* p, double lam, cba_newton_info* out);

int cba_subspace_gram(cba_problem* p, double a1, double b1, double a2, double b2, double* gram_out);

typedef struct {
  double cost;
  double step_norm;
  int32_t finite;
  int32_t reserved;
} cba_trial_info;

int cba_trial(cba_problem* p, double alpha, double beta, cba_trial_info* out);

int cba_accept(cba_problem* p);

typedef struct {
  cba_linearization lin;
  cba_newton_info newton;
  cba_trial_info trial;
  double lam, radius;
  double p_s[2], predicted;
  double alpha, beta;
  int32_t need_host, reserved;
} cba_step_info;
int cba_step(cba_problem* p, double radius, cba_step_info* out);
int cba_refresh_step_scalars(cba_problem* p, cba_newton_info* out);
int cba_step_supported(cba_problem* p);

int cba_set_camera_scaling(cba_problem* p, const double* mult, const double* diag_h, cba_linearization* out);

int cba_set_bounds(cba_problem* p, const double* lb, const double* ub);
int cba_step_camera_state(cba_problem* p, double* x_c, double* g_c, double* scale_inv_c, double* step_c);

int cba_linearize_build(cba_problem* p);

int cba_subspace_gram_ex(cba_problem* p, double a1, double b1, const double* cam1, double a2, double b2, const double* cam2,
                         double* gram_out);

int cba_trial_ex(cba_problem* p, double alpha, double beta, const double* cam_x_new, cba_trial_info* out);

typedef struct {
  double ftol, xtol, gtol;
  int64_t max_nfev;
  const double* lb;
  const double* ub;
  int32_t verbose;
  int32_t max_damping_retries;
} cba_solve_options;

typedef struct {
  int32_t status;
  int32_t reserved;
  int64_t nfev, njev, n_iterations;
  double cost;
  double optimality;
  double t_total_s;
  double t_rejected_s;
  int64_t n_rejected_timed;
} cba_result;

int cba_solve(cba_problem* p, const double* x0, const cba_solve_options* opt, double* x_out, cba_result* out);

enum { CBA_VEC_X = 0, CBA_VEC_X_NEW = 1, CBA_VEC_GRAD = 2, CBA_VEC_STEP = 3, CBA_VEC_SCALE_INV = 4 };

int cba_get_vector(cba_problem* p, int32_t which, double* out);

int cba_get_camera_params(cba_problem* p, int32_t which, double* out);

int cba_get_camera_state(cba_problem* p, double* x_c, double* g_c, double* scale_inv_c);

int cba_residuals(cba_problem* p, const double* x, double* r_out, double* cost_out);

int cba_normal_blocks(cba_problem* p, const double* x, double* U, double* V, double* gc, double* gp);

int cba_reduced_system(cba_problem* p, double* S, double* rhs);

int cba_set_loss(cba_problem* p, int32_t loss, double f_scale);

int cba_plan_wait(cba_problem* p);

typedef struct {
  int32_t n_cams, n_points, n_cam_params, n_params;
  int64_t n_obs;
  int32_t n_chunks, grid_blocks;
  int32_t plan_state;
  int32_t max_obs_per_point;
  int64_t device_bytes;
  int32_t schur_groups;
  int32_t schur_tiles;
  int32_t schur_grid;
  int32_t n_heavy_points;
  int64_t schur_stream_len;
  int64_t schur_pairs;
  int32_t plan_error;
  int32_t build_camg;
} cba_info;
int cba_get_info(cba_problem* p, cba_info* out);

int cba_timer_count(void);
const char* cba_timer_name(int32_t i);
int cba_get_timers(cba_problem* p, double* ms_out, int64_t* calls_out);
int cba_reset_timers(cba_problem* p);
int cba_enable_timers(cba_problem* p, int32_t on);

int64_t cba_host_plan(int32_t n_points, int64_t n_obs, const int32_t* obs_pt, const int32_t* obs_cam, int32_t n_cams,
                      int32_t chunk_cap, int64_t* order_out, int64_t* pt_start_out, int64_t* chunk_start_out);

int cba_set_constraints(cba_problem* p, int32_t n_con, const int32_t* groups_a, const int32_t* groups_b, const double* distances,
                        const double* weights);

typedef struct {
  int32_t n_cams;
  const int32_t* cam_model;
  const double* cam_intr;
  const double* cam_P;
  int64_t n_points;
  const int64_t* pt_start;
  const int32_t* obs_cam;
  const double* obs_xy;
  int32_t float32_io;
} cba_triangulate_desc;

int cba_triangulate(const cba_triangulate_desc* d, int32_t device, double* xyz_out, double* undistorted_out);

#define CBA_SCALE_NSTAT 8
typedef struct {
  int64_t n_world;   const double* world_xyz;
  int64_t n_groups;  const int64_t* group_start;
  const int64_t* ent_world;
  const double* ent_obj;
} cba_scale_desc;
int cba_scale_errors(const cba_scale_desc* d, int32_t device, double* stats_out);

int64_t cba_trim(void);

const char* cba_last_error(void);
int cba_set_error(int32_t code, const char* message);
int cba_version(void);
int cba_device_count(void);

#ifdef __cplusplus
}
#endif
#endif
```

Before: 3.671 billion obs/s.

## Skip speculative next-iteration J·v when the trial already meets termination

The trial-publish reduction kernel now evaluates the ftol/xtol termination test on the device and writes a flag. The speculative J·v kernel for the next linearization reads that flag and exits early, publishing only the gradient infinity-norm. The solver also hints the final allowed trial so that J·v is not enqueued at all, and it fetches the final gradient norm through a light path instead of a full linearize. This removes speculative work at the end of the solve, at the cost of extra device-side branching and host spin-wait logic.

```diff
diff --git a/caliscope_amd/_lib.py b/caliscope_amd/_lib.py
--- a/caliscope_amd/_lib.py
+++ b/caliscope_amd/_lib.py
@@ -62,6 +62,7 @@
         ("max_obs_per_point", C.c_int32), ("device_bytes", C.c_int64),
         ("schur_groups", C.c_int32), ("schur_tiles", C.c_int32), ("schur_grid", C.c_int32), ("n_heavy_points", C.c_int32),
         ("schur_stream_len", C.c_int64), ("schur_pairs", C.c_int64), ("plan_error", C.c_int32), ("build_camg", C.c_int32),
+        ("spec_jv_skipped", C.c_int64),
     ]
 
 
@@ -128,6 +129,9 @@
     "cba_step": (C.c_int, [C.c_void_p, C.c_double, C.POINTER(StepInfo)]),
     "cba_refresh_step_scalars": (C.c_int, [C.c_void_p, C.POINTER(NewtonInfo)]),
     "cba_step_supported": (C.c_int, [C.c_void_p]),
+    "cba_set_tolerances": (C.c_int, [C.c_void_p, C.c_double, C.c_double]),
+    "cba_hint_last_trial": (C.c_int, [C.c_void_p]),
+    "cba_gradient_norm": (C.c_int, [C.c_void_p, c_double_p]),
     "cba_set_camera_scaling": (C.c_int, [C.c_void_p, c_double_p, c_double_p, C.POINTER(Linearization)]),
     "cba_set_bounds": (C.c_int, [C.c_void_p, c_double_p, c_double_p]),
     "cba_step_camera_state": (C.c_int, [C.c_void_p, c_double_p, c_double_p, c_double_p, c_double_p]),
diff --git a/caliscope_amd/csrc/cba_kernels.h b/caliscope_amd/csrc/cba_kernels.h
--- a/caliscope_amd/csrc/cba_kernels.h
+++ b/caliscope_amd/csrc/cba_kernels.h
@@ -227,7 +227,16 @@
   double* scal; int n_scal; int* flags; double* host_scal; int* host_flags; unsigned long long seq;
   const double* part_a; int rows_a, slot_a; const double* part_b; int rows_b, slot_b;
   const double* cam_src[4]; double* cam_dst; int ncp;
+  int* spec_word; double ftol, xtol, cost_x;
 };
+__device__ __forceinline__ int pub_solve_ends(const PubArgs& pub, double ta, double tb) {
+  const double cost_new = 0.5 * ta;
+  const double cost = isnan(pub.cost_x) ? 0.5 * pub.scal[8] : pub.cost_x;
+  if (pub.scal[42] != 0.0 || (pub.flags[0] | pub.flags[1] | pub.flags[2] | pub.flags[3]) != 0 || !isfinite(cost_new) || !isfinite(cost)) return 0;
+  const double actual = cost - cost_new;
+  const double ratio = trf::reduction_ratio(actual, pub.scal[45]);
+  return trf::termination(actual, cost, sqrt(tb), sqrt(pub.scal[2]), ratio, pub.ftol, pub.xtol) != trf::TERMINATION_NONE ? 1 : 0;
+}
 __global__ void __launch_bounds__(64 * REDUCE_RY)
 k_reduce_rows_pub(const double* __restrict__ partial, int nrow, int width, double* __restrict__ out, double* __restrict__ grad_out,
                   const int* __restrict__ cam_off, const int* __restrict__ cam_np, int stride, int tri, PubArgs pub) {
@@ -242,15 +251,18 @@
   a = wave_sum(a); b = wave_sum(b);
   if (threadIdx.x == 0) { sh_w[0][threadIdx.y] = a; sh_w[1][threadIdx.y] = b; }
   __syncthreads();
-  __shared__ double sh_tot[2];
+  __shared__ double sh_tot[3];
   if (t == 0) {
     double ta = 0.0, tb = 0.0;
     for (int i = 0; i < REDUCE_RY; ++i) { ta += sh_w[0][i]; tb += sh_w[1][i]; }
     pub.scal[pub.slot_a] = ta; pub.scal[pub.slot_b] = tb;
     sh_tot[0] = ta; sh_tot[1] = tb;
-  }
-  __syncthreads();
-  if (t < pub.n_scal) pub.host_scal[t] = (t == pub.slot_a) ? sh_tot[0] : (t == pub.slot_b) ? sh_tot[1] : own;
+    int ends = 0;
+    if (pub.spec_word) { ends = pub_solve_ends(pub, ta, tb); *pub.spec_word = ends; }
+    sh_tot[2] = (double)ends;
+  }
+  __syncthreads();
+  if (t < pub.n_scal) pub.host_scal[t] = (t == pub.slot_a) ? sh_tot[0] : (t == pub.slot_b) ? sh_tot[1] : (t == pub.n_scal - 1) ? sh_tot[2] : own;
   if (t < 4) { pub.host_flags[t] = pub.flags[t]; pub.flags[t] = 0; }
   if (pub.cam_dst)
     for (int e = t; e < 4 * pub.ncp; e += 64 * REDUCE_RY) pub.cam_dst[e] = pub.cam_src[e / pub.ncp][e % pub.ncp];
@@ -823,13 +835,37 @@
   }
 }
 
+constexpr int MAIL_GNORM = 60, MAIL_GNORM_SEQ = 61;
+struct SpecSkip {
+  const int* word;
+  const double* max_rows;
+  int n_rows;
+  double* mail; unsigned long long seq;
+};
+__device__ __forceinline__ void publish_gnorm(const SpecSkip& sk) {
+  __shared__ double sh_gn[BLOCK / WAVE];
+  double m = 0.0;
+  for (int b = threadIdx.x; b < sk.n_rows; b += BLOCK) m = fmax(m, sk.max_rows[b]);
+  m = block_max(m, sh_gn);
+  if (threadIdx.x == 0) {
+    sk.mail[MAIL_GNORM] = m;
+    __threadfence_system();
+    reinterpret_cast<volatile unsigned long long*>(sk.mail)[MAIL_GNORM_SEQ] = sk.seq;
+  }
+}
+__global__ void __launch_bounds__(BLOCK) k_gnorm_pub(SpecSkip sk) { publish_gnorm(sk); }
+
 template <int NC, int NV, bool CAMG = false>
 __global__ void __launch_bounds__(BLOCK)
 k_jv(const double* __restrict__ obs_u, const double* __restrict__ obs_v, const int* __restrict__ obs_cam,
      const int* __restrict__ obs_pt, long n_obs, const double* __restrict__ xvec, VecLayout lay,
      const double* __restrict__ tab, const int* __restrict__ cam_off, int n_cams, int loss, double f_scale,
-     const double* __restrict__ v1, const double* __restrict__ v2, double* __restrict__ partial) {
+     const double* __restrict__ v1, const double* __restrict__ v2, double* __restrict__ partial, SpecSkip skip = SpecSkip{}) {
   CBA_STAMP(ST_JV);
+  if (skip.word && *skip.word) {
+    if (blockIdx.x == 0) publish_gnorm(skip);
+    return;
+  }
   extern __shared__ __attribute__((aligned(16))) double sh[];
   double* sh_tab = sh;
   double* sh_v = sh_tab + (CAMG ? 0 : n_cams * CAMTAB_LDS);
diff --git a/caliscope_amd/csrc/cba_lib.hip b/caliscope_amd/csrc/cba_lib.hip
--- a/caliscope_amd/csrc/cba_lib.hip
+++ b/caliscope_amd/csrc/cba_lib.hip
@@ -141,6 +141,15 @@
   double* sinv2 = nullptr;
   bool spec_enqueued = false, spec_valid = false;
   int spec_rows_jv = 0;
+  bool spec_skip = true, tol_set = false, last_trial_hint = false;
+  double ftol = 0.0, xtol = 0.0;
+  int* spec_word = nullptr;
+  bool spec_jv_enqueued = false;
+  bool spec_jv_dropped = false;
+  bool spec_scale_ready = false;
+  long spec_jv_skipped = 0;
+  unsigned long long gnorm_seq = 0;
+  bool gnorm_mailed = false;
   bool lf_pending = false;
   LinFin lf{};
   bool have_x0 = false;
@@ -1117,7 +1126,8 @@
   TRYS(dev_alloc(p, &p->Xinv, (size_t)((ncp + NB - 1) / NB + 1) * NB * NB));
   TRYS(dev_zeros(p, &p->Tinv, (size_t)ncp * p->ldw));
   TRYS(dev_alloc(p, &p->rhs, (size_t)p->lay.ncp_pad));
-  TRYS(dev_zeros(p, &p->scal, 64)); TRYS(dev_zeros(p, &p->flags, 4)); TRYS(dev_alloc(p, &p->xbuf, 128));
+  TRYS(dev_zeros(p, &p->scal, 64)); TRYS(dev_zeros(p, &p->flags, 8)); TRYS(dev_alloc(p, &p->xbuf, 128));
+  p->spec_word = p->flags + 4;
   TRYS(dev_alloc(p, &p->fz, 8)); TRYS(dev_zeros(p, &p->V2, (size_t)6 * p->lay.Ppad)); TRYS(dev_zeros(p, &p->g2, (size_t)tot));
   TRYS(dev_alloc(p, &p->U2, (size_t)p->C * ustride + 128));
   return CBA_OK;
@@ -1167,6 +1177,7 @@
   p->C = d->n_cams; p->P = d->n_points; p->N = d->n_obs;
   p->loss = d->loss; p->f_scale = d->f_scale;
   if (const char* e = std::getenv("CBA_REG_FINALIZE")) p->fuse_reg_finalize = e[0] != '0';
+  if (const char* e = std::getenv("CBA_SPEC_SKIP")) p->spec_skip = e[0] != '0';
 #ifdef CBA_PROFILING
   p->schur_clock = std::getenv("CBA_SCHUR_CLOCK") != nullptr;
   p->want_chol_trace = std::getenv("CBA_CHOL_TRACE") != nullptr;
@@ -1279,7 +1290,7 @@
   if (loss != CBA_LOSS_LINEAR && !(f_scale > 0.0)) return fail(CBA_ERR_INVALID, "cba_set_loss: f_scale must be positive");
   p->loss = loss; p->f_scale = f_scale;
   p->have_build = false;
-  p->spec_valid = false; p->spec_enqueued = false;
+  p->spec_valid = false; p->spec_enqueued = false; p->spec_scale_ready = false;
   return CBA_OK;
 }
 
@@ -1297,6 +1308,7 @@
     o->build_camg = (camg ? 1 : 0) | (p->tab_global ? 2 : 0) | (cs ? 4 : 0) | (uglob ? 8 : 0) | (p->backsub_rec ? 16 : 0) |
                     (p->con.n_con && p->con.small ? 32 : 0);
   }
+  o->spec_jv_skipped = p->spec_jv_skipped;
   return CBA_OK;
 }
 
@@ -1452,7 +1464,7 @@
 static int run_build(cba_problem* p) { return run_build_into<NC>(p, p->x, p->tab, p->V, p->g, p->Upacked, 8, nullptr, false, false, 3); }
 
 template <int NC>
-static int run_jv(cba_problem* p, int nv, int* rows_out = nullptr, const double* xvec = nullptr, const double* tab = nullptr) {
+static int run_jv(cba_problem* p, int nv, int* rows_out = nullptr, const double* xvec = nullptr, const double* tab = nullptr, const SpecSkip& skip = SpecSkip{}) {
   ScopedTimer t(p, T_JV);
   if (!xvec) { xvec = p->x; tab = p->tab; }
   const int grid = nv == 1 ? p->jv_grid : (int)std::min<long>((p->N + BLOCK - 1) / BLOCK, 1024);
@@ -1461,7 +1473,7 @@
     return fail(CBA_ERR_UNSUPPORTED, "run_jv: %d rows of k_jv and %d of k_con_jv exceed the %d rows of partial4", grid, con_rows, PARTIAL4_ROWS);
   auto launch_jv = [&](auto kernel) {
     hipLaunchKernelGGL(kernel, dim3(grid), dim3(BLOCK), lds_jv(p, nv), p->stream, p->obs_u, p->obs_v, p->obs_cam, p->obs_pt,
-                       p->N, xvec, p->lay, tab, p->cam_off, p->C, p->loss, p->f_scale, p->v1, p->v2, p->partial4);
+                       p->N, xvec, p->lay, tab, p->cam_off, p->C, p->loss, p->f_scale, p->v1, p->v2, p->partial4, skip);
   };
   if (nv == 1) { if (p->tab_global) launch_jv(k_jv<NC, 1, true>); else launch_jv(k_jv<NC, 1>); }
   else { if (p->tab_global) launch_jv(k_jv<NC, 2, true>); else launch_jv(k_jv<NC, 2>); }
@@ -1479,6 +1491,7 @@
 template <int NC>
 static int run_lin_chain(cba_problem* p, bool scalars = true, bool compact = false, double radius = 0.0, bool defer_finish = false) {
   RoctxRange range("cba:linearize");
+  p->spec_scale_ready = false; p->gnorm_mailed = false;
   if (!p->have_build) {
     int rcb = run_build<NC>(p);
     if (rcb) return rcb;
@@ -1876,14 +1889,18 @@
   const TrialSrc tsrc{p->x, p->g, p->sinv, p->s, p->fz + 2, p->x_new, p->partial4};
   const unsigned long long seq = compact ? ++p->publish_seq : 0;
   const bool bnd = compact && p->bounds_on;
-  const PubArgs pub{p->scal, 48, p->flags, p->d_hscal, p->d_hflags, seq, p->partial1, p->grid, 24, p->partial4, ft ? p->grid + 1 : vg, 28,
-                    {p->x, p->g, p->sinv_state_c, p->s}, bnd ? p->d_hbcam : (double*)nullptr, p->ncp};
+  const bool last_trial = p->last_trial_hint;
+  p->last_trial_hint = false;
+  const bool spec_test = compact && p->spec_skip && p->tol_set && !p->bounds_on && !last_trial;
+  const PubArgs pub{p->scal, 49, p->flags, p->d_hscal, p->d_hflags, seq, p->partial1, p->grid, 24, p->partial4, ft ? p->grid + 1 : vg, 28,
+                    {p->x, p->g, p->sinv_state_c, p->s}, bnd ? p->d_hbcam : (double*)nullptr, p->ncp,
+                    spec_test ? p->spec_word : (int*)nullptr, p->ftol, p->xtol, p->cost_pending ? NAN : p->cost_x};
   rc = run_build_into<NC>(p, p->x_new, p->tab_new, p->V2, p->g2, p->U2, 24, p->scal + 42, true, compact, 0, ft ? &tsrc : nullptr,
                           compact ? &pub : nullptr);
   if (rc) return rc;
   if (!compact) return CBA_OK;
   *seq_out = seq;
-  p->spec_enqueued = false;
+  p->spec_enqueued = false; p->spec_jv_enqueued = false;
   {
     {
       ScopedTimer t(p, T_SCALE_SCALARS);
@@ -1893,9 +1910,17 @@
                            (const double*)nullptr, p->x_new, p->g2, p->v1, p->partial4b, p->partial1, (const double*)p->sinv, ba2);
       };
       if (bnd) launch_sl2(k_scale_lin<NC, true>); else launch_sl2(k_scale_lin<NC, false>);
+    }
+    const SpecSkip skip{spec_test ? p->spec_word : (const int*)nullptr, p->partial1, vg, p->d_hscal, seq};
+    p->gnorm_seq = seq;
+    if (!(p->spec_skip && last_trial)) {
       int rows_jv = 0;
-      rc = run_jv<NC>(p, 1, &rows_jv, p->x_new, p->tab_new);
+      rc = run_jv<NC>(p, 1, &rows_jv, p->x_new, p->tab_new, skip);
       p->spec_rows_jv = rows_jv;
+      p->spec_jv_enqueued = true;
+    } else {
+      ScopedTimer t(p, T_SCALE_SCALARS);
+      hipLaunchKernelGGL(k_gnorm_pub, dim3(1), dim3(BLOCK), 0, p->stream, skip);
     }
     if (rc) return rc;
     p->spec_enqueued = true;
@@ -1923,6 +1948,8 @@
     rc = sync_scalars(p, 48);
   }
   if (rc) return rc;
+  p->spec_jv_dropped = compact && p->h_scal[48] != 0.0;
+  if (p->spec_jv_dropped) ++p->spec_jv_skipped;
   const int bad_residual = p->h_flags[0];
   read_linearization(p, &out->lin);
   read_newton(p, &out->newton);
@@ -1943,6 +1970,55 @@
   out->trial.step_norm = std::sqrt(p->h_scal[28]);
   out->trial.reserved = 0;
   p->trial_cost = c;
+  return CBA_OK;
+}
+
+template <int NC>
+static int run_gradient_norm(cba_problem* p, double* out) {
+  if (!p->spec_skip || p->sharded() || p->bounds_on || p->cam_scaled || p->eval_only) {
+    cba_linearization lin;
+    const int rc = run_linearize<NC>(p, &lin);
+    if (rc) return rc;
+    p->linearized = true; p->stepped = false;
+    *out = lin.g_norm_inf;
+    return CBA_OK;
+  }
+  if (p->spec_scale_ready && p->gnorm_mailed) {
+    volatile unsigned long long* word = reinterpret_cast<volatile unsigned long long*>(p->h_scal) + MAIL_GNORM_SEQ;
+    const auto t0 = std::chrono::steady_clock::now();
+    for (unsigned spins = 0; *word != p->gnorm_seq; ++spins) {
+      if ((spins & 0xfff) == 0xfff && std::chrono::steady_clock::now() - t0 > std::chrono::seconds(2)) {
+        HIPCHK(hipStreamSynchronize(p->stream));
+        if (*word != p->gnorm_seq) return fail(CBA_ERR_HIP, "the gradient norm of the accepted trial did not arrive");
+        break;
+      }
+    }
+    std::atomic_thread_fence(std::memory_order_acquire);
+    *out = p->h_scal[MAIL_GNORM];
+    return CBA_OK;
+  }
+  const int vg = vec_grid(p->lay.total());
+  if (!p->spec_scale_ready) {
+    if (!p->have_build) {
+      const int rcb = run_build<NC>(p);
+      if (rcb) return rcb;
+      p->cost_pending = true; p->have_build = true;
+    }
+    p->spec_valid = false;
+    ScopedTimer t(p, T_SCALE_SCALARS);
+    hipLaunchKernelGGL((k_scale_lin<NC, false>), dim3(vg), dim3(BLOCK), 0, p->stream, p->Upacked, p->V, p->param_cam, p->param_loc, p->lay, p->first_scale ? 1 : 0,
+                       p->sinv, p->con.n_con ? (const double*)p->con.cdiag : (const double*)nullptr, p->x, p->g, p->v1, p->partial4b, p->partial1,
+                       (const double*)nullptr, BoundArgs{});
+    p->first_scale = false;
+    p->spec_scale_ready = true;
+  }
+  {
+    ScopedTimer t(p, T_SCALE_SCALARS);
+    hipLaunchKernelGGL(k_reduce_narrow<true>, dim3(1), dim3(BLOCK), 0, p->stream, p->partial1, vg, 1, p->scal + 4);
+  }
+  const int rc = sync_scalars(p, 16);
+  if (rc) return rc;
+  *out = p->h_scal[4];
   return CBA_OK;
 }
 
@@ -2057,6 +2133,7 @@
 static int begin_common(cba_problem* p, double* cost_out, bool evaluate) {
   p->cam_scaled = false; p->cam_state_saved = false;
   p->have_build = false; p->trial_built = false; p->cost_pending = false; p->lf_pending = false;
+  p->spec_scale_ready = false; p->gnorm_mailed = false; p->tol_set = false; p->last_trial_hint = false;
   {
     ScopedTimer t(p, T_CAM_PREP);
     double* trial_buf = (!p->eval_only && fused_trial(p, true)) ? p->x_new : nullptr;
@@ -2284,19 +2361,46 @@
   if (!p->have_trial) return fail(CBA_ERR_INVALID, "cba_accept: no trial point");
   std::swap(p->x, p->x_new);
   std::swap(p->tab, p->tab_new);
-  p->spec_valid = false;
+  p->spec_valid = false; p->spec_scale_ready = false; p->gnorm_mailed = false;
   if (p->trial_built) {
     std::swap(p->V, p->V2); std::swap(p->g, p->g2); std::swap(p->Upacked, p->U2);
     p->cost_x = p->trial_cost;
     if (p->spec_enqueued) {
-      std::swap(p->sinv, p->sinv2); p->spec_valid = true;
+      std::swap(p->sinv, p->sinv2);
       if (p->bounds_on) { std::swap(p->sinv_state_c, p->sinv_state_c2); std::swap(p->cam_diag, p->cam_diag2); }
+      p->spec_valid = p->spec_jv_enqueued && !p->spec_jv_dropped;
+      p->spec_scale_ready = true;
+      p->gnorm_mailed = !p->spec_valid;
     }
   }
   p->spec_enqueued = false;
   p->have_build = p->trial_built;
   p->trial_built = false;
   p->have_trial = false; p->linearized = false; p->stepped = false;
+  return CBA_OK;
+}
+
+int cba_set_tolerances(cba_problem* p, double ftol, double xtol) {
+  if (!p) return fail(CBA_ERR_INVALID, "cba_set_tolerances: null argument");
+  if (!(ftol >= 0.0) || !(xtol >= 0.0)) return fail(CBA_ERR_INVALID, "cba_set_tolerances: the tolerances must be >= 0");
+  p->ftol = ftol; p->xtol = xtol; p->tol_set = true;
+  return CBA_OK;
+}
+
+int cba_hint_last_trial(cba_problem* p) {
+  if (!p) return fail(CBA_ERR_INVALID, "cba_hint_last_trial: null argument");
+  p->last_trial_hint = true;
+  return CBA_OK;
+}
+
+int cba_gradient_norm(cba_problem* p, double* g_norm_inf) {
+  if (!p || !g_norm_inf) return fail(CBA_ERR_INVALID, "cba_gradient_norm: null argument");
+  if (p->eval_only) return fail(CBA_ERR_INVALID, "cba_gradient_norm: the problem was created with evaluation_only");
+  if (!p->begun) return fail(CBA_ERR_INVALID, "cba_gradient_norm: call cba_begin first");
+  HIPCHK(hipSetDevice(p->device));
+  const int rc = DISPATCH_NC(p, run_gradient_norm<6>(p, g_norm_inf), run_gradient_norm<9>(p, g_norm_inf));
+  if (rc) return rc;
+  HIPCHK(hipGetLastError());
   return CBA_OK;
 }
 
diff --git a/caliscope_amd/csrc/cba_solve.cpp b/caliscope_amd/csrc/cba_solve.cpp
--- a/caliscope_amd/csrc/cba_solve.cpp
+++ b/caliscope_amd/csrc/cba_solve.cpp
@@ -15,15 +15,7 @@
 constexpr double SUBSPACE_EXPLICIT_BELOW = 1e-6;
 
 using trf::solve_subspace_2d;
-
-int termination(double dF, double F, double dx_norm, double x_norm, double ratio, double ftol, double xtol) {
-  const bool f_ok = dF < ftol * F && ratio > 0.25;
-  const bool x_ok = dx_norm < xtol * (xtol + x_norm);
-  if (f_ok && x_ok) return 4;
-  if (f_ok) return 2;
-  if (x_ok) return 3;
-  return -100;
-}
+using trf::termination;
 
 
 struct CamBlock {
@@ -87,6 +79,15 @@
   }
 };
 
+}
+
+extern "C" __attribute__((weak)) int cba_set_tolerances(cba_problem*, double, double) { return CBA_OK; }
+extern "C" __attribute__((weak)) int cba_hint_last_trial(cba_problem*) { return CBA_OK; }
+extern "C" __attribute__((weak)) int cba_gradient_norm(cba_problem* p, double* g_norm_inf) {
+  cba_linearization lin;
+  const int rc = cba_linearize(p, &lin);
+  if (!rc && g_norm_inf) *g_norm_inf = lin.g_norm_inf;
+  return rc;
 }
 
 extern "C" int cba_solve(cba_problem* p, const double* x0, const cba_solve_options* opt_in, double* x_out, cba_result* out) {
@@ -144,12 +145,14 @@
   } else {
     (void)cba_set_bounds(p, nullptr, nullptr);
   }
+  if (!bounded && (rc = cba_set_tolerances(p, opt.ftol, opt.xtol))) return rc;
   bool fused = (!bounded || bounds_on_device) && cba_step_supported(p);
   bool fuse_next = fused;
   int n_outside = 0;
   cba_linearization lin;
   cba_step_info si;
   bool lin_valid = false;
+  bool accepted = false;
   double radius = NAN;
   int status = -100;
   double g_norm = NAN, step_norm = NAN, actual = NAN;
@@ -160,8 +163,11 @@
     bool have_step = false;
     if (!lin_valid) {
       if (status == -100 && fuse_next && nfev < max_nfev) {
+        if (nfev + 1 >= max_nfev && (rc = cba_hint_last_trial(p))) return rc;
         if ((rc = calls.run("step", [&] { return cba_step(p, std::isnan(radius) ? -1.0 : radius, &si); }))) return rc;
         lin = si.lin; have_step = true;
+      } else if (!bounded && accepted && (status != -100 || nfev >= max_nfev)) {
+        if ((rc = calls.run("gradient_norm", [&] { return cba_gradient_norm(p, &lin.g_norm_inf); }))) return rc;
       } else if (bounded) {
         fuse_next = false;
         if ((rc = calls.run("linearize_build", [&] { return cba_linearize_build(p); }))) return rc;
@@ -349,10 +355,7 @@
       actual = cost - cost_new;
       if (own_call && !(actual > 0)) { t_rejected += dt_trial; ++n_rejected_timed; }
       if (was_first) fuse_next = fused && actual > 0 && w_sq > 1e-2 * st.p_sq;
-      double ratio;
-      if (predicted > 0) ratio = actual / predicted;
-      else if (predicted == 0 && actual == 0) ratio = 1.0;
-      else ratio = 0.0;
+      const double ratio = trf::reduction_ratio(actual, predicted);
       double radius_new = radius;
       if (ratio < 0.25) radius_new = 0.25 * step_h_norm;
       else if (ratio > 0.75 && step_h_norm > 0.95 * radius) radius_new = 2.0 * radius;
@@ -363,6 +366,7 @@
     }
     if (actual > 0) {
       if ((rc = calls.run("accept", [&] { return cba_accept(p); }))) return rc;
+      accepted = true;
       cost = cost_new;
       lin_valid = false;
       ++njev;
diff --git a/caliscope_amd/csrc/trf_math.h b/caliscope_amd/csrc/trf_math.h
--- a/caliscope_amd/csrc/trf_math.h
+++ b/caliscope_amd/csrc/trf_math.h
@@ -136,4 +136,20 @@
   *b11 = (H_pp - 2.0 * c * H_gp + c * c * H_gg) / w_sq;
 }
 
+TRF_HD inline double reduction_ratio(double actual, double predicted) {
+  if (predicted > 0.0) return actual / predicted;
+  if (predicted == 0.0 && actual == 0.0) return 1.0;
+  return 0.0;
 }
+
+constexpr int TERMINATION_NONE = -100;
+TRF_HD inline int termination(double dF, double F, double dx_norm, double x_norm, double ratio, double ftol, double xtol) {
+  const bool f_ok = dF < ftol * F && ratio > 0.25;
+  const bool x_ok = dx_norm < xtol * (xtol + x_norm);
+  if (f_ok && x_ok) return 4;
+  if (f_ok) return 2;
+  if (x_ok) return 3;
+  return TERMINATION_NONE;
+}
+
+}
diff --git a/include/caliscope_ba.h b/include/caliscope_ba.h
--- a/include/caliscope_ba.h
+++ b/include/caliscope_ba.h
@@ -111,6 +111,10 @@
 int cba_step(cba_problem* p, double radius, cba_step_info* out);
 int cba_refresh_step_scalars(cba_problem* p, cba_newton_info* out);
 int cba_step_supported(cba_problem* p);
+
+int cba_set_tolerances(cba_problem* p, double ftol, double xtol);
+int cba_hint_last_trial(cba_problem* p);
+int cba_gradient_norm(cba_problem* p, double* g_norm_inf);
 
 int cba_set_camera_scaling(cba_problem* p, const double* mult, const double* diag_h, cba_linearization* out);
 
@@ -179,6 +183,7 @@
   int64_t schur_pairs;
   int32_t plan_error;
   int32_t build_camg;
+  int64_t spec_jv_skipped;
 } cba_info;
 int cba_get_info(cba_problem* p, cba_info* out);
 
```

After: 3.729 billion obs/s, median of 6. 1.6% higher.
